# kamwoh/concepthash

Hardware: AMD Instinct MI355X
Metric: images/s encode (ViT+hash) + Hamming top-10 retrieval, CUB-200 64-bit (higher is better)
Workload: dtype bf16; 1 GPU; CUB-200 64-bit concept_hash, vit_b16 bf16 (CLIP-structured, Q=4 concept tokens, adapters b=384), batch=256/GPU, top-10 Hamming vs 5994-row gallery shard/GPU; per_gpu_batch=256, global_batch=256, gallery_rows_per_gpu=5994, hip_streams=2, parallelism=single GPU

## Files before the change

### concepthash_amd/_lib.py

```python
from __future__ import annotations

import ctypes
import os
from ctypes import (POINTER, Structure, c_char_p, c_double, c_float, c_int, c_int32, c_int64, c_size_t, c_uint32,
                    c_uint64, c_ulonglong, c_void_p)

_HERE = os.path.dirname(os.path.abspath(__file__))
LIB_PATH = os.path.join(_HERE, "libconcepthash_hip.so")
ABI_VERSION = 3


class ModelConfig(Structure):
    _fields_ = [(n, c_int32) for n in ("image_size", "patch", "dim", "layers", "heads", "ffn", "adapter_dim", "ncontext",
                                       "nbit", "nclass", "proj_dim", "center_dim", "upt_heads", "act", "max_batch")] + \
               [("ln_eps", c_float), ("bn_eps", c_float)]


class TextConfig(Structure):
    _fields_ = [(n, c_int32) for n in ("vocab", "max_positions", "dim", "layers", "heads", "ffn", "act", "max_batch")] + [("ln_eps", c_float)]


class ImageDesc(Structure):
    _fields_ = [("src_offset", c_int64), ("tmp_offset", c_int64)] + \
               [(n, c_int32) for n in ("h", "w", "nh", "nw", "top", "left", "row0", "nrows", "stride", "flip")]


class AugmentDesc(Structure):
    _fields_ = [("src_offset", c_int64), ("tmp_offset", c_int64), ("img_offset", c_int64)] + \
               [(n, c_int32) for n in ("h", "w", "nh", "nw", "top", "left", "row0", "nrows", "flip", "op", "iparam", "reserved")] + \
               [("fparam", c_double), ("m", c_double * 6)]


class JpegDesc(Structure):
    _fields_ = [("coef_offset", c_int64), ("pix_offset", c_int64), ("plane_offset", c_int64)] + \
               [(n, c_int32) for n in ("width", "height", "ncomp", "hs", "vs", "mcu_w", "mcu_h", "status", "nblocks", "reserved")] + \
               [("quant", (ctypes.c_uint16 * 64) * 3)]


class Tensor(Structure):
    _fields_ = [("name", c_char_p), ("data", POINTER(c_float)), ("numel", c_int64)]


SIGNATURES = {
    "ch_abi_version": (c_int, []),
    "ch_last_error": (c_char_p, []),
    "ch_model_create": (c_int, [POINTER(ModelConfig), POINTER(Tensor), c_int32, POINTER(c_void_p)]),
    "ch_model_destroy": (None, [c_void_p]),
    "ch_model_device_bytes": (c_size_t, [c_void_p]),
    "ch_model_flops_per_image": (c_double, [c_void_p]),
    "ch_model_set_option": (c_int, [c_void_p, c_char_p, c_int64]),
    "ch_model_get_option": (c_int, [c_void_p, c_char_p, POINTER(c_int64)]),
    "ch_model_profile_begin": (c_int, [c_void_p, c_int32]),
    "ch_model_profile_end": (c_int, [c_void_p, c_int32, POINTER(c_double), POINTER(c_int64), POINTER(c_double)]),
    "ch_debug_gemm": (c_int, [c_int32, c_void_p, c_int64, c_void_p, c_void_p, c_int32, c_int32, c_int32, c_int32, c_void_p,
                              c_int32, c_void_p, c_int32, c_void_p, c_void_p, c_void_p]),
    "ch_debug_gemm_ln": (c_int, [c_int32, c_void_p, c_int64, c_void_p, c_void_p, c_int32, c_int32, c_int32, c_int32, c_void_p,
                                 c_int32, c_void_p, c_int32, c_void_p, c_void_p, c_void_p, c_void_p, c_float, c_void_p, c_void_p,
                                 c_void_p]),
    "ch_debug_gemm_train": (c_int, [c_int32, c_void_p, c_int64, c_void_p, c_void_p, c_int32, c_int32, c_int32, c_int32, c_void_p,
                                    c_int32, c_void_p, c_void_p, c_void_p, c_void_p, c_float, c_void_p, c_int32, c_void_p]),
    "ch_debug_gemm_patch": (c_int, [c_int32, c_void_p, c_int64, c_void_p, c_int32, c_int32, c_int32, c_void_p, c_int32, c_void_p,
                                    c_int32, c_int32, c_void_p]),
    "ch_debug_gemm_dispatch_count": (c_int64, [c_int32]),
    "ch_debug_experiments_built": (c_int32, []),
    "ch_debug_set_gemm_splitk": (None, [c_int32]),
    "ch_debug_copy_buffer": (c_int, [c_void_p, c_int32, c_void_p, c_int64, c_void_p]),
    "ch_debug_adapter": (c_int, [c_void_p] * 2 + [c_int32] * 3 + [c_void_p] * 10 + [c_int32, c_void_p]),
    "ch_debug_attention": (c_int, [c_void_p, c_int32, c_int32, c_int32, c_void_p, c_void_p]),
    "ch_debug_attention_ex": (c_int, [c_void_p, c_int32, c_int32, c_int32, c_void_p, c_void_p, c_int32, c_int32, c_int32, c_void_p]),
    "ch_debug_attention_causal": (c_int, [c_void_p, c_int32, c_int32, c_int32, c_void_p, c_void_p]),
    "ch_debug_attention_dispatch_count": (c_int64, [c_int32]),
    "ch_encode": (c_int, [c_void_p, c_void_p, c_int32, c_int32, c_void_p, c_void_p, c_void_p, c_void_p, c_void_p,
                          c_void_p, c_void_p, c_void_p, c_int32, c_void_p]),
    "ch_encode_hidden": (c_int, [c_void_p, c_void_p, c_int32, c_int32, c_int32, c_void_p, c_void_p]),
    "ch_preprocess": (c_int, [c_void_p, c_void_p, c_int32, c_int32, c_int32, c_int32, POINTER(c_float), POINTER(c_float), c_void_p,
                              c_int32, c_void_p, c_void_p]),
    "ch_preprocess_max_taps": (c_int32, []),
    "ch_augment_workspace": (c_int64, [c_int32, c_int64]),
    "ch_preprocess_augment": (c_int, [c_void_p, c_void_p, c_int32, c_int32, c_int32, c_int32, c_int32, POINTER(c_float), POINTER(c_float),
                                      c_void_p, c_int32, c_void_p, c_void_p]),
    "ch_jpeg_plan": (c_int, [c_void_p, c_void_p, c_int32, c_void_p, POINTER(c_int64), POINTER(c_int64), POINTER(c_int64)]),
    "ch_jpeg_entropy_decode": (c_int, [c_void_p, c_void_p, c_int32, c_void_p, c_void_p, c_int32]),
    "ch_jpeg_plan_packed": (c_int, [c_void_p, c_void_p, c_int32, c_void_p, POINTER(c_int64), POINTER(c_int64), POINTER(c_int64)]),
    "ch_jpeg_entropy_decode_packed": (c_int, [c_void_p, c_void_p, c_int32, c_void_p, c_void_p, c_int32]),
    "ch_io_file_sizes": (c_int, [c_void_p, c_int32, c_void_p]),
    "ch_io_read_files": (c_int, [c_void_p, c_int32, c_void_p, c_void_p, c_void_p, c_int32]),
    "ch_jpeg_reconstruct": (c_int, [c_void_p, c_void_p, c_void_p, c_int32, c_void_p, c_void_p, c_void_p]),
    "ch_pack_sign": (c_int, [c_void_p, c_int64, c_int32, c_float, c_void_p, c_void_p]),
    "ch_hamming_dist": (c_int, [c_void_p, c_int64, c_void_p, c_int64, c_int32, c_void_p, c_void_p]),
    "ch_hamming_topk_workspace": (c_size_t, [c_int64, c_int64, c_int32, c_int32]),
    "ch_hamming_topk": (c_int, [c_void_p, c_int64, c_void_p, c_int64, c_int32, c_int32, c_int64, c_void_p, c_void_p,
                                c_void_p, c_size_t, c_void_p]),
    "ch_topk_merge": (c_int, [c_void_p, c_void_p, c_int32, c_int64, c_int32, c_void_p, c_void_p, c_void_p]),
    "ch_hamming_hist": (c_int, [c_void_p, c_int64, c_void_p, c_int64, c_int32, c_void_p, c_void_p, c_int32, c_int32,
                                c_void_p, c_void_p]),
    "ch_hamming_ap": (c_int, [c_void_p, c_int64, c_void_p, c_int64, c_int32, c_void_p, c_void_p, c_int32, c_int32,
                              c_void_p, c_int64, c_void_p, c_void_p, c_void_p, c_void_p]),
    "ch_hamming_ap_multi": (c_int, [c_void_p, c_int64, c_void_p, c_int64, c_int32, c_void_p, c_void_p, c_int32, c_int32,
                                    c_void_p, POINTER(c_int64), c_int32, c_void_p, c_void_p, c_void_p, c_void_p]),
    "ch_hamming_rec_workgroups": (c_size_t, [c_int64, c_int64, c_int32, c_int32]),
    "ch_hamming_rec_block": (c_int32, [c_int32]),
    "ch_hamming_hist_rec": (c_int, [c_void_p, c_int64, c_void_p, c_int64, c_int32, c_void_p, c_void_p, c_int32, c_int32,
                                    c_void_p, c_void_p, c_int32, c_void_p, c_void_p, c_void_p]),
    "ch_hamming_ap_rec": (c_int, [c_void_p, c_int64, c_void_p, c_int64, c_int32, c_void_p, c_void_p, c_int32, c_int32,
                                  c_void_p, c_void_p, c_int32, c_void_p, c_void_p, POINTER(c_int64), c_int32, c_void_p, c_void_p,
                                  c_void_p, c_void_p]),
    "ch_adapter_arena_numel": (c_int64, [c_void_p]),
    "ch_trainer_create": (c_int, [c_void_p, c_int32, c_void_p, c_void_p, POINTER(c_void_p)]),
    "ch_backbone_arena_numel": (c_int64, [POINTER(ModelConfig)]),
    "ch_backbone_arena_offset": (c_int64, [POINTER(ModelConfig), c_char_p, POINTER(c_int64)]),
    "ch_trainer_create_ex": (c_int, [c_void_p, c_int32, c_void_p, c_void_p, c_void_p, c_void_p, POINTER(c_void_p)]),
    "ch_trainer_destroy": (None, [c_void_p]),
    "ch_trainer_bytes": (c_int64, [c_void_p]),
    "ch_trainer_refresh": (c_int, [c_void_p, c_void_p]),
    "ch_train_forward": (c_int, [c_void_p, c_void_p, c_int32, c_int32, c_void_p, c_void_p, c_void_p, c_void_p, c_int32, c_void_p]),
    "ch_train_backward": (c_int, [c_void_p, c_void_p, c_void_p, c_void_p, c_void_p]),
    "ch_sgd_step": (c_int, [c_void_p, c_void_p, c_void_p, c_int64, c_float, c_float, c_float, c_float, c_int32, c_int32, c_void_p]),
    "ch_adam_step": (c_int, [c_void_p, c_void_p, c_void_p, c_void_p, c_int64, c_double, c_double, c_double, c_double, c_double, c_int32, c_int64,
                             c_void_p]),
    "ch_debug_attention_bwd": (c_int, [c_void_p, c_void_p, c_int32, c_int32, c_int32, c_void_p, c_void_p, c_int32, c_void_p]),
    "ch_debug_attention_bwd_ex": (c_int, [c_void_p, c_void_p, c_int32, c_int32, c_int32, c_void_p, c_void_p, c_int32, c_int32, c_void_p]),
    "ch_debug_wgrad": (c_int, [c_void_p, c_int32, c_void_p, c_int32, c_int64, c_int64, c_int32, c_int32, c_void_p, c_void_p]),
    "ch_debug_ln_bwd": (c_int, [c_void_p, c_void_p, c_int64, c_int32, c_float, c_void_p, c_void_p, c_void_p, c_void_p, c_void_p]),
    "ch_debug_act": (c_int, [c_void_p, c_void_p, c_int64, c_int32, c_void_p, c_int32, c_void_p, c_void_p]),
    "ch_hamming_hist_prefix": (c_int, [c_void_p, c_int32, c_int64, c_int32, c_void_p, c_void_p, c_void_p]),
    "ch_debug_set_hamming_scalar_loads": (None, [c_int32]),
    "ch_hamming_tie_bracket": (c_int, [c_void_p, c_int64, c_int32, POINTER(c_int64), c_int32, c_int32, c_void_p, c_void_p, c_void_p,
                                       c_void_p, c_void_p]),
    "ch_text_create": (c_int, [POINTER(TextConfig), POINTER(Tensor), c_int32, POINTER(c_void_p)]),
    "ch_text_destroy": (None, [c_void_p]),
    "ch_text_device_bytes": (c_size_t, [c_void_p]),
    "ch_text_encode": (c_int, [c_void_p, POINTER(c_int32), POINTER(c_int32), c_int32, c_int32, c_void_p, c_void_p, c_void_p]),
}

OPTION_KEYS = ("streams", "chain_auto", "ln_fold", "prune_last", "pp_min_k", "attn_stream", "small_kernel", "serpentine", "pp_sched", "fused_adapter", "resid_nt",
               "nt_out", "group_n", "splitk", "gemm_rows", "wide_kernel", "graph_max_batch", "train_chains", "train_chain_min_rows", "train_prune_last",
               "train_batched_grads")
_ENV_OVERRIDES = {
    "CH_STREAMS": ("streams", int), "CH_LN_FOLD": ("ln_fold", int), "CH_PRUNE_LAST": ("prune_last", int),
    "CH_GEMM_PP_MIN_K": ("pp_min_k", int), "CH_GEMM_SMALL": ("small_kernel", int), "CH_SERPENTINE": ("serpentine", int),
    "CH_GEMM_PP_SCHED": ("pp_sched", int), "CH_FUSED_ADAPTER": ("fused_adapter", int),
    "CH_RESID_NT": ("resid_nt", lambda v: 1 if int(v) else -1), "CH_NT_OUT": ("nt_out", lambda v: 1 if int(v) else -1),
    "CH_GEMM_GROUP_N": ("group_n", int), "CH_GEMM_SPLITK": ("splitk", int), "CH_GEMM_ROWS": ("gemm_rows", int), "CH_GEMM_WIDE": ("wide_kernel", int), "CH_GRAPH_MAX_BATCH": ("graph_max_batch", int),
    "CH_CHAIN_AUTO": ("chain_auto", int), "CH_TRAIN_STREAMS": ("train_chains", int), "CH_TRAIN_CHAIN_MIN_ROWS": ("train_chain_min_rows", int),
    "CH_TRAIN_PRUNE_LAST": ("train_prune_last", int),
}


def env_option_overrides() -> dict:
    out = {}
    for env, (key, conv) in _ENV_OVERRIDES.items():
        if env in os.environ:
            out[key] = conv(os.environ[env])
    return out

CATEGORIES = ("im2col", "gemm_patch", "rowops", "gemm_qkv", "attention", "gemm_out", "gemm_down", "gemm_up", "gemm_fc1",
              "gemm_fc2", "head", "adapter_fused", "attention_pruned", "gemm_out_pruned", "gemm_down_pruned", "gemm_up_pruned",
              "gemm_fc1_pruned", "gemm_fc2_pruned", "end")

_lib = None


def load() -> ctypes.CDLL:
    global _lib
    if _lib is not None:
        return _lib
    if not os.path.exists(LIB_PATH):
        raise RuntimeError(
            f"{LIB_PATH} is missing: the ConceptHash MI355X path needs the HIP extension. "
            "Build it with `python -m concepthash_amd.build` (hipcc, --offload-arch=gfx950). There is no CPU fallback.")
    try:
        lib = ctypes.CDLL(LIB_PATH)
    except OSError as e:
        raise RuntimeError(f"cannot load {LIB_PATH}: {e}") from e
    for name, (res, args) in SIGNATURES.items():
        try:
            fn = getattr(lib, name)
        except AttributeError as e:
            raise RuntimeError(f"{LIB_PATH} does not export {name}; rebuild it") from e
        fn.restype = res
        fn.argtypes = args
    if lib.ch_abi_version() != ABI_VERSION:
        raise RuntimeError(f"ABI mismatch: library {lib.ch_abi_version()} vs binding {ABI_VERSION}; rebuild")
    _lib = lib
    return lib


def check(status: int, what: str) -> None:
    if status != 0:
        msg = load().ch_last_error()
        raise RuntimeError(f"{what} failed (status {status}): {msg.decode() if msg else 'unknown error'}")


def stream_ptr(stream=None) -> c_void_p:
    import torch
    s = stream if stream is not None else torch.cuda.current_stream()
    return c_void_p(s.cuda_stream)


def ptr(t) -> c_void_p:
    return c_void_p(t.data_ptr()) if t is not None else c_void_p(0)
```

### concepthash_amd/csrc/attention.hip

```cpp
#include "ch_common.h"
#include "kernels.h"

namespace {

constexpr int HD = 64;
constexpr int QKV_AUX = 0;
#define LDQ(p) (*(const bf16x8 *)(p))
constexpr int NW = 8;
typedef __attribute__((address_space(3))) void lds_void_t;
typedef __attribute__((address_space(1))) const void gbl_void_t;
typedef short v4s __attribute__((ext_vector_type(4)));
typedef __attribute__((address_space(3))) v4s lds_v4s;

template <int KB, bool TAP, bool COMPACT, bool CAUSAL = false>
__global__ __launch_bounds__(NW * 64, 4) void attention_kernel(const bf16_t *__restrict__ qkv, int ntok, int heads, float scale_log2e,
                                                        bf16_t *__restrict__ out, float *__restrict__ cattn, int ncon, int rev) {
    extern __shared__ __attribute__((aligned(16))) char smem[];
    constexpr int KT = KB * 2;
    constexpr int KP = KB * 32;
    char *Ks = smem;
    char *Vs = smem + KP * 128;

    const int tid = threadIdx.x, lane = tid & 63;
    const int wid = __builtin_amdgcn_readfirstlane(tid >> 6);
    const int bid = rev ? (int)gridDim.x - 1 - (int)blockIdx.x : (int)blockIdx.x;
    const int b = bid / heads, h = bid - b * heads;
    const int D = heads * HD;
    const size_t ld = (size_t)3 * D;
    const bf16_t *base = qkv + (size_t)b * ntok * ld + h * HD;

    {
        const int lrow = lane >> 3;
        const int src_chunk = (lane & 7) ^ lrow;
        for (int i = wid; i < KP / 8; i += NW) {
            int row = i * 8 + lrow;
            row = row < ntok ? row : ntok - 1;
            const bf16_t *src = base + (size_t)row * ld + src_chunk * 8;
            __builtin_amdgcn_global_load_lds((gbl_void_t *)(src + D), (lds_void_t *)(Ks + i * 1024), 16, 0, QKV_AUX);
            __builtin_amdgcn_global_load_lds((gbl_void_t *)(src + 2 * D), (lds_void_t *)(Vs + i * 1024), 16, 0, QKV_AUX);
        }
    }
    const int fr = lane & 15, fq = lane >> 4;
    const int nqc = 1 + ncon;
    const int QT = COMPACT ? (nqc + 15) >> 4 : (ntok + 15) >> 4;
    auto query_of = [&](int j, bool &valid) {
        if constexpr (COMPACT) {
            valid = j < nqc;
            return !valid ? ntok - 1 : (j == 0 ? 0 : ntok - ncon + j - 1);
        } else {
            valid = j < ntok;
            return valid ? j : ntok - 1;
        }
    };
    bool qvalid;
    int qslot = wid * 16 + fr;
    int q = query_of(qslot, qvalid);
    bf16x8 qf0 = LDQ(base + (size_t)q * ld + fq * 8);
    bf16x8 qf1 = LDQ(base + (size_t)q * ld + fq * 8 + 32);
    asm volatile("s_waitcnt vmcnt(0)" ::: "memory");
    __syncthreads();

    const int tq = fr >> 2, tp = fr & 3;
    const int trow7 = ((fq & 1) << 2) | tq;
    int voff[4];
#pragma unroll
    for (int dt = 0; dt < 4; ++dt)
        voff[dt] = (fq * 4 + tq) * 128 + (((dt * 2 + (tp >> 1)) ^ trow7) << 4) + (tp & 1) * 8;
    const int koff0 = fr * 128 + ((fq ^ (fr & 7)) << 4), koff1 = fr * 128 + (((4 + fq) ^ (fr & 7)) << 4);

    for (int qt = wid; qt < QT; qt += NW) {
        f32x4 st[KT];
        bf16x8 kf[2][4];
#pragma unroll
        for (int t = 0; t < 2; ++t) {
            kf[0][2 * t] = *(const bf16x8 *)(Ks + t * 2048 + koff0);
            kf[0][2 * t + 1] = *(const bf16x8 *)(Ks + t * 2048 + koff1);
        }
#pragma unroll
        for (int c = 0; c < KB; ++c) {
            if (c + 1 < KB) {
#pragma unroll
                for (int t = 0; t < 2; ++t) {
                    kf[(c + 1) & 1][2 * t] = *(const bf16x8 *)(Ks + (2 * c + 2 + t) * 2048 + koff0);
                    kf[(c + 1) & 1][2 * t + 1] = *(const bf16x8 *)(Ks + (2 * c + 2 + t) * 2048 + koff1);
                }
            }
#pragma unroll
            for (int t = 0; t < 2; ++t) {
                f32x4 a = {0.f, 0.f, 0.f, 0.f};
                a = __builtin_amdgcn_mfma_f32_16x16x32_bf16(kf[c & 1][2 * t], qf0, a, 0, 0, 0);
                a = __builtin_amdgcn_mfma_f32_16x16x32_bf16(kf[c & 1][2 * t + 1], qf1, a, 0, 0, 0);
                st[2 * c + t] = a;
            }
            __builtin_amdgcn_sched_barrier(0);
        }
        const bool cur_valid = qvalid;
        const int cur_q = q, cur_slot = qslot;
        if (qt + NW < QT) {
            qslot = (qt + NW) * 16 + fr;
            q = query_of(qslot, qvalid);
            qf0 = LDQ(base + (size_t)q * ld + fq * 8);
            qf1 = LDQ(base + (size_t)q * ld + fq * 8 + 32);
        }
#pragma unroll
        for (int kt = KT - 2; kt < KT; ++kt)
            if (kt >= 0 && kt * 16 + 16 > ntok) {
#pragma unroll
                for (int r = 0; r < 4; ++r)
                    if (kt * 16 + fq * 4 + r >= ntok) st[kt][r] = -1e30f;
            }
        if constexpr (CAUSAL) {
            const int lim = cur_q - fq * 4;
#pragma unroll
            for (int kt = 0; kt < KT; ++kt)
#pragma unroll
                for (int r = 0; r < 4; ++r) st[kt][r] = kt * 16 + r > lim ? -1e30f : st[kt][r];
        }
        float mx = -1e30f;
#pragma unroll
        for (int kt = 0; kt < KT; ++kt)
#pragma unroll
            for (int r = 0; r < 4; ++r) mx = fmaxf(mx, st[kt][r]);
        mx = fmaxf(mx, __shfl_xor(mx, 16, 64));
        mx = fmaxf(mx, __shfl_xor(mx, 32, 64));
        const float mxs = mx * scale_log2e;
        float sum = 0.f;
#pragma unroll
        for (int kt = 0; kt < KT; ++kt)
#pragma unroll
            for (int r = 0; r < 4; ++r) {
                const float e = __builtin_amdgcn_exp2f(st[kt][r] * scale_log2e - mxs);
                st[kt][r] = e;
                sum += e;
            }
        sum += __shfl_xor(sum, 16, 64);
        sum += __shfl_xor(sum, 32, 64);
        const float inv = 1.0f / sum;
        if (TAP && cur_valid && cur_q >= ntok - ncon) {
            const int np = ntok - ncon - 1;
            float *dst = cattn + (((size_t)b * heads + h) * ncon + (cur_q - (ntok - ncon))) * np;
#pragma unroll
            for (int kt = 0; kt < KT; ++kt)
#pragma unroll
                for (int r = 0; r < 4; ++r) {
                    const int key = kt * 16 + fq * 4 + r;
                    if (key >= 1 && key <= np) dst[key - 1] = st[kt][r] * inv;
                }
        }

        f32x4 o[4];
#pragma unroll
        for (int dt = 0; dt < 4; ++dt) o[dt] = f32x4{0.f, 0.f, 0.f, 0.f};
        union VF {
            bf16x8 v;
            v4s h[2];
        };
        VF vf[2][4];
#pragma unroll
        for (int dt = 0; dt < 4; ++dt) {
            vf[0][dt].h[0] = __builtin_amdgcn_ds_read_tr16_b64_v4i16((lds_v4s *)(Vs + voff[dt]));
            vf[0][dt].h[1] = __builtin_amdgcn_ds_read_tr16_b64_v4i16((lds_v4s *)(Vs + 2048 + voff[dt]));
        }
#pragma unroll
        for (int kb = 0; kb < KB; ++kb) {
            if (kb + 1 < KB) {
#pragma unroll
                for (int dt = 0; dt < 4; ++dt) {
                    vf[(kb + 1) & 1][dt].h[0] = __builtin_amdgcn_ds_read_tr16_b64_v4i16((lds_v4s *)(Vs + (kb + 1) * 4096 + voff[dt]));
                    vf[(kb + 1) & 1][dt].h[1] =
                        __builtin_amdgcn_ds_read_tr16_b64_v4i16((lds_v4s *)(Vs + (kb + 1) * 4096 + 2048 + voff[dt]));
                }
            }
            union {
                bf16x8 v;
                uint32_t u[4];
            } pf;
            pf.u[0] = pack_bf16x2(st[2 * kb][0], st[2 * kb][1]);
            pf.u[1] = pack_bf16x2(st[2 * kb][2], st[2 * kb][3]);
            pf.u[2] = pack_bf16x2(st[2 * kb + 1][0], st[2 * kb + 1][1]);
            pf.u[3] = pack_bf16x2(st[2 * kb + 1][2], st[2 * kb + 1][3]);
#pragma unroll
            for (int dt = 0; dt < 4; ++dt) o[dt] = __builtin_amdgcn_mfma_f32_16x16x32_bf16(vf[kb & 1][dt].v, pf.v, o[dt], 0, 0, 0);
            __builtin_amdgcn_sched_barrier(0);
        }
        if (cur_valid) {
            bf16_t *op = out + (COMPACT ? (size_t)b * nqc + cur_slot : (size_t)b * ntok + cur_q) * D + h * HD + fq * 4;
#pragma unroll
            for (int dt = 0; dt < 4; ++dt) {
                uint2 w;
                w.x = pack_bf16x2(o[dt][0] * inv, o[dt][1] * inv);
                w.y = pack_bf16x2(o[dt][2] * inv, o[dt][3] * inv);
                *(uint2 *)(op + dt * 16) = w;
            }
        }
    }
}

template <int KB, bool TAP, bool COMPACT, bool CAUSAL = false>
int launch_attn_inst(const bf16_t *qkv, int B, int ntok, int heads, bf16_t *out, float *cattn, int ncon, int rev, hipStream_t s) {
    const int KP = KB * 32;
    const size_t lds = (size_t)KP * 128 * 2;
    CH_REQUIRE(lds <= 160 * 1024, "attention: sequence too long for the LDS-resident K/V kernel");
    static ch_once_per_device lds_once;
    if (int e = ch_func_max_lds((const void *)attention_kernel<KB, TAP, COMPACT, CAUSAL>, (int)lds, lds_once)) return e;
    const float scale_log2e = 0.125f * 1.4426950408889634f;
    CH_LAUNCH((attention_kernel<KB, TAP, COMPACT, CAUSAL>), dim3(B * heads), dim3(NW * 64), lds, s, qkv, ntok, heads, scale_log2e,
                       out, cattn, ncon, rev);
    CH_LAUNCH_CHECK();
    return 0;
}
template <int KB>
int launch_attn(const bf16_t *qkv, int B, int ntok, int heads, bf16_t *out, float *cattn, int ncon, bool compact, int rev, hipStream_t s) {
    if (compact)
        return cattn ? launch_attn_inst<KB, true, true>(qkv, B, ntok, heads, out, cattn, ncon, rev, s)
                     : launch_attn_inst<KB, false, true>(qkv, B, ntok, heads, out, cattn, ncon, rev, s);
    return cattn ? launch_attn_inst<KB, true, false>(qkv, B, ntok, heads, out, cattn, ncon, rev, s)
                 : launch_attn_inst<KB, false, false>(qkv, B, ntok, heads, out, cattn, ncon, rev, s);
}

}

int ch_attention(const bf16_t *qkv, int B, int ntok, int heads, bf16_t *out, hipStream_t s, float *cattn, int ncon, bool compact,
                 bool rev, int kernel) {
    CH_REQUIRE(B > 0 && ntok > 0 && heads > 0, "attention: empty problem");
    CH_REQUIRE(!compact || (ncon >= 1 && ncon < ntok), "attention: compact mode needs 1 <= ncon < ntok");
    CH_REQUIRE(kernel >= 0 && kernel <= 2, "attention: kernel must be 0 (by length), 1 (resident) or 2 (streaming)");
    if (kernel == 2 || (kernel == 0 && ntok > CH_ATTN_RESIDENT_MAX_TOKENS)) {
        ch_attention_count_launch(1);
        return ch_attention_stream(qkv, B, ntok, heads, out, s, cattn, ncon, compact, rev);
    }
    if (ntok <= CH_ATTN_RESIDENT_MAX_TOKENS) ch_attention_count_launch(0);
    const int KB = (ntok + 31) / 32;
    switch (KB) {
        case 1: return launch_attn<1>(qkv, B, ntok, heads, out, cattn, ncon, compact, rev ? 1 : 0, s);
        case 2: return launch_attn<2>(qkv, B, ntok, heads, out, cattn, ncon, compact, rev ? 1 : 0, s);
        case 3: return launch_attn<3>(qkv, B, ntok, heads, out, cattn, ncon, compact, rev ? 1 : 0, s);
        case 4: return launch_attn<4>(qkv, B, ntok, heads, out, cattn, ncon, compact, rev ? 1 : 0, s);
        case 5: return launch_attn<5>(qkv, B, ntok, heads, out, cattn, ncon, compact, rev ? 1 : 0, s);
        case 6: return launch_attn<6>(qkv, B, ntok, heads, out, cattn, ncon, compact, rev ? 1 : 0, s);
        case 7: return launch_attn<7>(qkv, B, ntok, heads, out, cattn, ncon, compact, rev ? 1 : 0, s);
        case 8: return launch_attn<8>(qkv, B, ntok, heads, out, cattn, ncon, compact, rev ? 1 : 0, s);
        case 9: return launch_attn<9>(qkv, B, ntok, heads, out, cattn, ncon, compact, rev ? 1 : 0, s);
    }
    ch_set_error("attention: the LDS-resident kernel holds at most 288 tokens per image");
    return 2;
}

int ch_attention_causal(const bf16_t *qkv, int B, int ntok, int heads, bf16_t *out, hipStream_t s) {
    CH_REQUIRE(B > 0 && ntok > 0 && heads > 0, "causal attention: empty problem");
    CH_REQUIRE(ntok <= CH_ATTN_RESIDENT_MAX_TOKENS, "causal attention: the LDS-resident kernel holds at most 288 tokens per sequence");
    switch ((ntok + 31) / 32) {
        case 1: return launch_attn_inst<1, false, false, true>(qkv, B, ntok, heads, out, nullptr, 0, 0, s);
        case 2: return launch_attn_inst<2, false, false, true>(qkv, B, ntok, heads, out, nullptr, 0, 0, s);
        case 3: return launch_attn_inst<3, false, false, true>(qkv, B, ntok, heads, out, nullptr, 0, 0, s);
        case 4: return launch_attn_inst<4, false, false, true>(qkv, B, ntok, heads, out, nullptr, 0, 0, s);
        case 5: return launch_attn_inst<5, false, false, true>(qkv, B, ntok, heads, out, nullptr, 0, 0, s);
        case 6: return launch_attn_inst<6, false, false, true>(qkv, B, ntok, heads, out, nullptr, 0, 0, s);
        case 7: return launch_attn_inst<7, false, false, true>(qkv, B, ntok, heads, out, nullptr, 0, 0, s);
        case 8: return launch_attn_inst<8, false, false, true>(qkv, B, ntok, heads, out, nullptr, 0, 0, s);
        default: return launch_attn_inst<9, false, false, true>(qkv, B, ntok, heads, out, nullptr, 0, 0, s);
    }
}
```

### concepthash_amd/csrc/debug_taps.hip

```cpp
#include <algorithm>
#include <string>

#include "model_internal.h"
#include "../../include/concepthash_hip_debug.h"

static bool g_debug_splitk = false;
static float *g_debug_ws = nullptr;
static unsigned *g_debug_cnt = nullptr;
static int debug_attach_splitk(GemmParams &p) {
    if (!g_debug_splitk) return 0;
    if (!g_debug_ws) {
        CH_CHECK_HIP(hipMalloc((void **)&g_debug_ws, CH_SPLITK_WS_BYTES));
        CH_CHECK_HIP(hipMalloc((void **)&g_debug_cnt, CH_SPLITK_CNT_BYTES));
        CH_CHECK_HIP(hipMemset(g_debug_cnt, 0, CH_SPLITK_CNT_BYTES));
    }
    p.splitk_ws = g_debug_ws;
    p.splitk_cnt = g_debug_cnt;
    p.force_split = 1;
    return 0;
}
extern "C" void ch_debug_set_gemm_splitk(int32_t on) { g_debug_splitk = on != 0; }

static GemmParams debug_gemm_params(const void *X, int64_t X_rows_alloc, const void *W, const float *bias, int32_t M, int32_t N, int32_t K,
                                    void *out_bf16, int32_t ldo, const float *scale_ptr) {
    GemmParams p{};
    p.X = (const bf16_t *)X; p.W = (const bf16_t *)W; p.M = M; p.N = N; p.K = K; p.X_rows_alloc = X_rows_alloc;
    p.bias = bias; p.out_bf16 = (bf16_t *)out_bf16; p.ldo = ldo; p.scale_ptr = scale_ptr;
    return p;
}
static int debug_gemm_launch(GemmParams &p, int epi, void *stream, int variant, bool direct, bool splitk) {
    if (splitk)
        if (int e = debug_attach_splitk(p)) return e;
    return direct ? ch_gemm_launch_variant(variant, p, epi, (hipStream_t)stream) : ch_gemm_bf16(p, epi, (hipStream_t)stream, variant);
}
extern "C" int ch_debug_gemm(int32_t variant, const void *X, int64_t X_rows_alloc, const void *W, const float *bias,
                             int32_t M, int32_t N, int32_t K, int32_t epi, void *out_bf16, int32_t ldo, float *resid,
                             int32_t ldr, const float *scale_ptr, const void *addend, void *stream) {
    CH_REQUIRE(X && W, "debug_gemm: null operand");
    CH_REQUIRE(epi >= EPI_BIAS && epi <= EPI_SCALE_RESID, "debug_gemm: epilogue must be one of the non-patch modes");
    GemmParams p = debug_gemm_params(X, X_rows_alloc, W, bias, M, N, K, out_bf16, ldo, scale_ptr);
    p.resid = resid; p.ldr = ldr; p.addend = (const bf16_t *)addend; p.ld_addend = N;
    const bool direct = (variant >= 1 && variant <= 10) || (variant >= 21 && variant <= 29) || (variant >= 41 && variant <= 47);
    return debug_gemm_launch(p, epi, stream, direct ? variant : 0, direct, true);
}
extern "C" int ch_debug_gemm_ln(int32_t variant, const void *X, int64_t X_rows_alloc, const void *W, const float *bias,
                                int32_t M, int32_t N, int32_t K, int32_t epi, void *out_bf16, int32_t ldo, float *resid,
                                int32_t ldr, const float *scale_ptr, const void *addend, const float *stats_in,
                                const float *fold_c, float ln_eps, float *stats_out, void *hb_out, void *stream) {
    CH_REQUIRE(X && W, "debug_gemm_ln: null operand");
    CH_REQUIRE(epi >= EPI_BIAS_STATS && epi <= EPI_FOLD_GELU, "debug_gemm_ln: epilogue must be one of the LayerNorm-fold modes");
    GemmParams p = debug_gemm_params(X, X_rows_alloc, W, bias, M, N, K, out_bf16, ldo, scale_ptr);
    p.resid = resid; p.ldr = ldr; p.addend = (const bf16_t *)addend; p.ld_addend = N;
    p.stats_in = stats_in; p.fold_c = fold_c; p.ln_eps = ln_eps; p.stats_out = stats_out; p.hb_out = (bf16_t *)hb_out; p.ld_hb = N;
    const bool direct = variant >= 5 && variant <= 7;
    const bool forced = variant == 1 || variant == 2 || variant == 4 || variant == 8 || variant == 9 || variant == 10;
    return debug_gemm_launch(p, epi, stream, direct || forced ? variant : 0, direct, true);
}
static int debug_gemm_launch_checked(GemmParams &p, int epi, void *stream, int variant, const char *what) {
    if (variant != 0 && variant != 1 && variant != 2 && variant != 4 && variant != 7) {
        ch_set_error(std::string(what) + ": variant must be 0 (dispatcher), 1, 2, 4 or 7");
        return 2;
    }
    return debug_gemm_launch(p, epi, stream, variant, variant != 0, false);
}
extern "C" int ch_debug_gemm_train(int32_t variant, const void *X, int64_t X_rows_alloc, const void *W, const float *bias, int32_t M,
                                   int32_t N, int32_t K, int32_t epi, void *out_bf16, int32_t ldo, const void *aux, const float *scale_ptr,
                                   const float *stats_in, const float *fold_c, float ln_eps, void *hb_out, int32_t ld_hb, void *stream) {
    CH_REQUIRE(X && W && bias && out_bf16, "debug_gemm_train: null operand");
    CH_REQUIRE(epi >= EPI_BIAS_DACT_QUICK && epi <= EPI_FOLD_ACT2_GELU, "debug_gemm_train: epilogue must be one of the training modes (11 .. 14)");
    CH_REQUIRE(M > 0 && N > 0 && K > 0, "debug_gemm_train: empty problem");
    CH_REQUIRE(ldo >= N && ldo % 8 == 0, "debug_gemm_train: ldo must be >= N and a multiple of 8 (16-byte row chunks)");
    const bool dact = epi == EPI_BIAS_DACT_QUICK || epi == EPI_BIAS_DACT_GELU;
    if (dact) {
        CH_REQUIRE(aux != nullptr, "debug_gemm_train: the derivative epilogues need aux");
        const char *a0 = (const char *)aux, *o0 = (const char *)out_bf16;
        const size_t span = ((size_t)(M - 1) * ldo + N) * sizeof(bf16_t);
        CH_REQUIRE(a0 + span <= o0 || o0 + span <= a0, "debug_gemm_train: aux and out_bf16 must not overlap");
    } else {
        CH_REQUIRE(hb_out != nullptr && stats_in && fold_c, "debug_gemm_train: the two-output epilogues need hb_out, stats_in and fold_c");
        CH_REQUIRE(ld_hb >= N && ld_hb % 8 == 0, "debug_gemm_train: ld_hb must be >= N and a multiple of 8 (16-byte row chunks)");
        CH_REQUIRE(K % 128 == 0 && K <= 1280 && ln_eps > 0.f, "debug_gemm_train: LN-folded epilogue needs K % 128 == 0, K <= 1280, ln_eps > 0");
        CH_REQUIRE(hb_out != out_bf16, "debug_gemm_train: hb_out and out_bf16 must be distinct");
    }
    GemmParams p = debug_gemm_params(X, X_rows_alloc, W, bias, M, N, K, out_bf16, ldo, scale_ptr);
    p.aux = (const bf16_t *)aux;
    p.stats_in = stats_in; p.fold_c = fold_c; p.ln_eps = ln_eps; p.hb_out = (bf16_t *)hb_out; p.ld_hb = ld_hb;
    return debug_gemm_launch_checked(p, epi, stream, variant, "debug_gemm_train");
}
extern "C" int ch_debug_gemm_patch(int32_t variant, const void *X, int64_t X_rows_alloc, const void *W, int32_t M, int32_t N, int32_t K,
                                   float *resid, int32_t ldr, const float *pos, int32_t tokens_per_img, int32_t patches_per_img,
                                   void *stream) {
    CH_REQUIRE(X && W && resid && pos, "debug_gemm_patch: null operand");
    CH_REQUIRE(M > 0 && N > 0 && K > 0, "debug_gemm_patch: empty problem");
    CH_REQUIRE(ldr >= N && ldr % 4 == 0, "debug_gemm_patch: ldr must be >= N and a multiple of 4 (16-byte row chunks)");
    CH_REQUIRE(patches_per_img >= 1 && tokens_per_img >= 1 + patches_per_img, "debug_gemm_patch: tokens_per_img must be >= 1 + patches_per_img");
    CH_REQUIRE(M % patches_per_img == 0, "debug_gemm_patch: M must be a whole number of images");
    GemmParams p = debug_gemm_params(X, X_rows_alloc, W, nullptr, M, N, K, nullptr, 0, nullptr);
    p.resid = resid; p.ldr = ldr; p.pos = pos; p.tokens_per_img = tokens_per_img; p.patches_per_img = patches_per_img;
    return debug_gemm_launch_checked(p, EPI_PATCH, stream, variant, "debug_gemm_patch");
}
extern "C" int32_t ch_debug_experiments_built(void) {
#ifdef CH_EXPERIMENTS
    return 1;
#else
    return 0;
#endif
}

extern "C" int ch_debug_attention(const void *qkv, int32_t B, int32_t ntok, int32_t heads, void *out, void *stream) {
    CH_REQUIRE(qkv && out, "debug_attention: null pointer");
    return ch_attention((const bf16_t *)qkv, B, ntok, heads, (bf16_t *)out, (hipStream_t)stream);
}
extern "C" int ch_debug_attention_ex(const void *qkv, int32_t B, int32_t ntok, int32_t heads, void *out, float *cattn, int32_t ncon,
                                     int32_t compact, int32_t kernel, void *stream) {
    CH_REQUIRE(qkv && out, "debug_attention_ex: null pointer");
    return ch_attention((const bf16_t *)qkv, B, ntok, heads, (bf16_t *)out, (hipStream_t)stream, cattn, ncon, compact != 0, false, kernel);
}

extern "C" int ch_debug_attention_causal(const void *qkv, int32_t B, int32_t ntok, int32_t heads, void *out, void *stream) {
    CH_REQUIRE(qkv && out, "debug_attention_causal: null pointer");
    return ch_attention_causal((const bf16_t *)qkv, B, ntok, heads, (bf16_t *)out, (hipStream_t)stream);
}

extern "C" int ch_debug_adapter(const void *A, float *H, int32_t M, int32_t D, int32_t b, const float *Wd, const float *bd,
                                const float *gamma, const float *beta, const void *Wu_bf16_padded, const float *bu,
                                const float *scale, void *work_wdf, float *work_c, float *work_d, int32_t dbg, void *stream) {
    const int bpad = (int)round_up64(b, 128);
    hipStream_t s = (hipStream_t)stream;
    if (int e = ch_fold_ln(Wd, bd, gamma, beta, b, bpad, D, (bf16_t *)work_wdf, work_c, work_d, s)) return e;
    AdapterParams p{};
    p.A = (const bf16_t *)A; p.H = H; p.M = M; p.D = D; p.bpad = bpad; p.Wd = (const bf16_t *)work_wdf; p.c = work_c; p.d = work_d;
    p.Wu = (const bf16_t *)Wu_bf16_padded; p.bu = bu; p.scale = scale; p.eps = 1e-5f; p.dbg = dbg;
    return ch_adapter_fused(p, s);
}

extern "C" int ch_debug_copy_buffer(ch_model *m, int32_t which, void *out, int64_t nbytes, void *stream) {
    CH_REQUIRE(m != nullptr && out != nullptr && nbytes >= 0, "debug_copy_buffer: null pointer");
    const int64_t rows = m->rows_alloc, D = m->cfg.dim;
    const void *src = nullptr;
    int64_t size = 0;
    switch (which) {
        case 0: src = m->H; size = rows * D * 4; break;
        case 1: src = m->Xn; size = rows * D * 2; break;
        case 2: src = m->QKV; size = rows * 3 * D * 2; break;
        case 3: src = m->AO; size = rows * D * 2; break;
        case 4: src = m->A; size = rows * D * 2; break;
        case 5: src = m->AD; size = rows * std::max(m->bpad, 128) * 2; break;
        case 6: src = m->F1; size = rows * (int64_t)m->cfg.ffn * 2; break;
        default: CH_REQUIRE(false, "debug_copy_buffer: which must be 0..6 (H, Xn, QKV, AO, A, AD, F1)");
    }
    CH_REQUIRE(nbytes <= size, "debug_copy_buffer: more bytes requested than the buffer holds");
    CH_CHECK_HIP(hipMemcpyAsync(out, src, (size_t)nbytes, hipMemcpyDeviceToDevice, (hipStream_t)stream));
    return 0;
}

extern "C" int ch_debug_attention_bwd(const void *qkv, const void *dO, int32_t B, int32_t ntok, int32_t heads, void *dqkv, const float *dpext,
                                      int32_t ncon, void *stream) {
    CH_REQUIRE(qkv && dO && dqkv, "debug_attention_bwd: null argument");
    return ch_attention_bwd((const bf16_t *)qkv, (const bf16_t *)dO, B, ntok, heads, (bf16_t *)dqkv, (hipStream_t)stream, dpext, ncon);
}
extern "C" int ch_debug_attention_bwd_ex(const void *qkv, const void *dO, int32_t B, int32_t ntok, int32_t heads, void *dqkv, const float *dpext,
                                         int32_t ncon, int32_t kernel, void *stream) {
    CH_REQUIRE(qkv && dO && dqkv, "debug_attention_bwd_ex: null argument");
    return ch_attention_bwd((const bf16_t *)qkv, (const bf16_t *)dO, B, ntok, heads, (bf16_t *)dqkv, (hipStream_t)stream, dpext, ncon, kernel);
}
extern "C" int ch_debug_wgrad(const void *A, int32_t lda, const void *Bm, int32_t ldb, int64_t rows, int64_t rows_alloc, int32_t N,
                              int32_t K, float *out, void *stream) {
    CH_REQUIRE(A && Bm && out, "debug_wgrad: null argument");
    float *ws = nullptr;
    CH_CHECK_HIP(hipMalloc((void **)&ws, sizeof(float) * ch_wgrad_ws_floats(rows, N, K)));
    const int e = ch_wgrad_tn((bf16_t *)A, lda, (const bf16_t *)Bm, ldb, rows, rows_alloc, N, K, out, ws, (hipStream_t)stream);
    (void)hipStreamSynchronize((hipStream_t)stream);
    (void)hipFree(ws);
    return e;
}
extern "C" int ch_debug_ln_bwd(const void *dyg, const void *x, int64_t rows, int32_t D, float eps, const float *dres_in, float *dres_out,
                               void *out_b, void *xhat_out, void *stream) {
    CH_REQUIRE(dyg && x && dres_in, "debug_ln_bwd: null argument");
    hipStream_t s = (hipStream_t)stream;
    float *st = nullptr, *xf = nullptr;
    bf16_t *hb = nullptr;
    CH_CHECK_HIP(hipMalloc((void **)&st, sizeof(float) * rows * (D / 64) * 2));
    CH_CHECK_HIP(hipMalloc((void **)&xf, sizeof(float) * rows * D));
    CH_CHECK_HIP(hipMalloc((void **)&hb, sizeof(bf16_t) * rows * D));
    int e = 0;
    {
        CH_CHECK_HIP(hipMemsetAsync(xf, 0, sizeof(float) * rows * D, s));
        CH_CHECK_HIP(hipMemcpy2DAsync((char *)xf + 2, 4, x, 2, 2, (size_t)rows * D, hipMemcpyDeviceToDevice, s));
    }
    e = ch_hb_stats(xf, rows, D, hb, st, s);
    if (!e) e = ch_ln_bwd((const bf16_t *)dyg, (const bf16_t *)x, st, rows, D, eps, dres_in, dres_out, (bf16_t *)out_b, s);
    if (!e && xhat_out) e = ch_normalize_bf16((const bf16_t *)x, st, rows, D, eps, (bf16_t *)xhat_out, s);
    (void)hipStreamSynchronize(s);
    (void)hipFree(st);
    (void)hipFree(xf);
    (void)hipFree(hb);
    return e;
}
extern "C" int ch_debug_act(const void *g, const void *pre, int64_t n, int32_t act, const float *scale_ptr, int32_t backward, void *out,
                            void *stream) {
    CH_REQUIRE(pre && out, "debug_act: null argument");
    if (backward) return ch_act_bwd((const bf16_t *)g, (const bf16_t *)pre, n, act, scale_ptr, (bf16_t *)out, (hipStream_t)stream);
    return ch_act_fwd((const bf16_t *)pre, n, act, (bf16_t *)out, (hipStream_t)stream);
}
```

### concepthash_amd/csrc/gemm_bf16.hip

```cpp
#include <cstdlib>

#include "ch_common.h"
#include "kernels.h"
#include "gemm_epilogue.h"

namespace {

constexpr int BM = 128, BN = 128, BK = 64;
constexpr int STAGE_BYTES = (BM + BN) * BK * 2;
constexpr int NTHREADS = 256;

typedef __attribute__((address_space(3))) void lds_void_t;
typedef __attribute__((address_space(1))) const void gbl_void_t;


__device__ __forceinline__ int xcd_remap(int bid, int nwg) {
    const int q = nwg >> 3, r = nwg & 7, xcd = bid & 7, local = bid >> 3;
    const int base = xcd < r ? xcd * (q + 1) : r * (q + 1) + (xcd - r) * q;
    return base + local;
}

template <int EPI, bool NT = false>
__global__ __launch_bounds__(NTHREADS, 2) void gemm_bf16_kernel(GemmParams p) {
    extern __shared__ __attribute__((aligned(16))) char smem[];
    const int tid = threadIdx.x;
    const int lane = tid & 63;
    const int wid = __builtin_amdgcn_readfirstlane(tid >> 6);
    const int wm = wid & 1, wn = wid >> 1;

    const int tiles_n = p.N / BN;
    const int tiles_m = (p.M + BM - 1) / BM;
    const int wg = xcd_remap(blockIdx.x, tiles_m * tiles_n);
    const int per_group = tiles_m * p.group_n;
    const int g = wg / per_group, rem = wg - g * per_group;
    const int gn = min(p.group_n, tiles_n - g * p.group_n);
    const int tm_fwd = rem / gn, tn = g * p.group_n + (rem - tm_fwd * gn);
    const int tm = p.rev ? tiles_m - 1 - tm_fwd : tm_fwd;
    const int m0 = tm * BM, n0 = tn * BN;

    const int lrow = lane >> 3;
    const int src_chunk = (lane & 7) ^ lrow;
    const char *gsrc[8];
#pragma unroll
    for (int j = 0; j < 8; ++j) {
        const int row = (wid * 8 + j) * 8 + lrow;
        const bf16_t *base = row < BM ? p.X + (size_t)(m0 + row) * p.K : p.W + (size_t)(n0 + row - BM) * p.K;
        gsrc[j] = (const char *)(base + src_chunk * 8);
    }
    auto stage = [&](int buf, int kt) {
        char *dst = smem + buf * STAGE_BYTES + wid * 8 * 1024;
#pragma unroll
        for (int j = 0; j < 8; ++j)
            __builtin_amdgcn_global_load_lds((gbl_void_t *)(gsrc[j] + (size_t)kt * BK * 2), (lds_void_t *)(dst + j * 1024),
                                             16, 0, 0);
    };

    f32x4 acc[4][4];
#pragma unroll
    for (int a = 0; a < 4; ++a)
#pragma unroll
        for (int b = 0; b < 4; ++b) acc[a][b] = f32x4{0.f, 0.f, 0.f, 0.f};

    const int frow = lane & 15, fq = lane >> 4;
    const int nk = p.K / BK;

    f32x4 fold_v[5];
    if constexpr (ch_epi::traits<EPI>::fold) ch_epi::fold_stats_issue(p, m0, tid, fold_v);
    stage(0, 0);
    constexpr bool PREF = ch_epi::traits<EPI>::scale_resid;
    ch_epi::ResidPrefetch rp;
    if constexpr (PREF) ch_epi::resid_prefetch<EPI, NT>(p, m0 + wm * 64, n0 + wn * 64, lane, rp);
    asm volatile("s_waitcnt vmcnt(0)" ::: "memory");
    __builtin_amdgcn_sched_barrier(0);
    if constexpr (ch_epi::traits<EPI>::fold)
        ch_epi::fold_stats_finish(p, tid, fold_v, (float *)(smem + 2 * STAGE_BYTES));
    __syncthreads();

    int cur = 0;
    for (int kt = 0; kt < nk; ++kt) {
        if (kt + 1 < nk) stage(cur ^ 1, kt + 1);
        const char *xs = smem + cur * STAGE_BYTES;
        const char *ws = xs + BM * BK * 2;
#pragma unroll
        for (int kk = 0; kk < 2; ++kk) {
            bf16x8 wf[4], xf[4];
#pragma unroll
            for (int t = 0; t < 4; ++t) {
                const int wr = wn * 64 + t * 16 + frow;
                wf[t] = *(const bf16x8 *)(ws + wr * 128 + (((kk * 4 + fq) ^ (wr & 7)) << 4));
                const int xr = wm * 64 + t * 16 + frow;
                xf[t] = *(const bf16x8 *)(xs + xr * 128 + (((kk * 4 + fq) ^ (xr & 7)) << 4));
            }
#pragma unroll
            for (int nt = 0; nt < 4; ++nt)
#pragma unroll
                for (int mt = 0; mt < 4; ++mt)
                    acc[nt][mt] = __builtin_amdgcn_mfma_f32_16x16x32_bf16(wf[nt], xf[mt], acc[nt][mt], 0, 0, 0);
        }
        asm volatile("s_waitcnt vmcnt(0)" ::: "memory");
        __syncthreads();
        cur ^= 1;
    }

    ch_epi::store_tile<EPI, 4, PREF, NT>(p, acc, smem + wid * 16384, m0 + wm * 64, n0 + wn * 64, lane,
                                         (const float *)(smem + 2 * STAGE_BYTES) + 2 * (wm * 64), &rp);
}

template <int EPI>
int launch(const GemmParams &p0, hipStream_t s) {
    GemmParams p = p0;
    p.group_n = ch_gemm_group_n(p.M, p.N, p.K, BM, BN, p.group_n_opt);
    const int tiles = ((p.M + BM - 1) / BM) * (p.N / BN);
    constexpr int lds = 2 * STAGE_BYTES + (ch_epi::traits<EPI>::fold ? CH_FOLD_LDS_BYTES : 0);
    static ch_once_per_device lds_once;
    if (int e = ch_func_max_lds((const void *)gemm_bf16_kernel<EPI>, lds, lds_once)) return e;
    if constexpr (ch_epi::traits<EPI>::scale_resid) {
        if (p.nt_resid) {
            static ch_once_per_device lds_once_nt;
            if (int e = ch_func_max_lds((const void *)gemm_bf16_kernel<EPI, true>, lds, lds_once_nt)) return e;
            CH_LAUNCH((gemm_bf16_kernel<EPI, true>), dim3(tiles), dim3(NTHREADS), lds, s, p);
            CH_LAUNCH_CHECK();
            ch_gemm_count_nt_launch(0);
            return 0;
        }
    }
    CH_LAUNCH(gemm_bf16_kernel<EPI>, dim3(tiles), dim3(NTHREADS), lds, s, p);
    CH_LAUNCH_CHECK();
    return 0;
}

}

int ch_gemm_bf16_v1(const GemmParams &p, int epi, hipStream_t s) {
    CH_REQUIRE(p.M > 0 && p.N > 0 && p.K > 0, "gemm: empty problem");
    CH_REQUIRE(epi == EPI_PATCH || p.bias != nullptr, "gemm: bias is required");
    CH_REQUIRE(p.N % BN == 0, "gemm: N must be a multiple of 128");
    CH_REQUIRE(p.K % BK == 0, "gemm: K must be a multiple of 64");
    CH_REQUIRE(p.X_rows_alloc >= round_up64(p.M, BM), "gemm: X must be allocated for M rounded up to 128 rows");
    switch (epi) {
        case EPI_BIAS: return launch<EPI_BIAS>(p, s);
        case EPI_BIAS_QUICKGELU: return launch<EPI_BIAS_QUICKGELU>(p, s);
        case EPI_BIAS_GELU: return launch<EPI_BIAS_GELU>(p, s);
        case EPI_BIAS_RESID: return launch<EPI_BIAS_RESID>(p, s);
        case EPI_SCALE_RESID: return launch<EPI_SCALE_RESID>(p, s);
        case EPI_PATCH: return launch<EPI_PATCH>(p, s);
        case EPI_BIAS_STATS: return launch<EPI_BIAS_STATS>(p, s);
        case EPI_SCALE_RESID_STATS: return launch<EPI_SCALE_RESID_STATS>(p, s);
        case EPI_FOLD_BIAS: return launch<EPI_FOLD_BIAS>(p, s);
        case EPI_FOLD_QUICKGELU: return launch<EPI_FOLD_QUICKGELU>(p, s);
        case EPI_FOLD_GELU: return launch<EPI_FOLD_GELU>(p, s);
        case EPI_BIAS_DACT_QUICK: return launch<EPI_BIAS_DACT_QUICK>(p, s);
        case EPI_BIAS_DACT_GELU: return launch<EPI_BIAS_DACT_GELU>(p, s);
        case EPI_FOLD_ACT2_QUICK: return launch<EPI_FOLD_ACT2_QUICK>(p, s);
        case EPI_FOLD_ACT2_GELU: return launch<EPI_FOLD_ACT2_GELU>(p, s);
    }
    ch_set_error("gemm: unknown epilogue");
    return 2;
}

int ch_gemm_group_n(int M, int N, int K, int bm, int bn, int forced) {
    const int tiles_n = N / bn, tiles_m = (M + bm - 1) / bm;
    const double xbytes = 2.0 * M * K, wpanel = 2.0 * bn * K, wbytes = 2.0 * N * K;
    const double rounds = (double)tiles_m * tiles_n / 256.0 + 1.0;
    if (forced > 0) return forced < tiles_n ? forced : tiles_n;
    int best = tiles_n;
    double best_cost = 1e300;
    for (int gn = 1; gn <= tiles_n; ++gn) {
        const int ng = (tiles_n + gn - 1) / gn;
        const bool fits = gn * wpanel <= 2.0e6;
        const double cost = xbytes * ng + wbytes * 8.0 * (fits ? 1.0 : rounds);
        if (cost < best_cost - 1.0) {
            best_cost = cost;
            best = gn;
        }
    }
    return best;
}

static std::atomic<int64_t> g_dispatch_count[5];
void ch_gemm_count_nt_launch(int kind) { g_dispatch_count[2 + (kind != 0)].fetch_add(1, std::memory_order_relaxed); }
static int resid_nt_choice(const GemmParams &p, int epi) {
    if (epi != EPI_SCALE_RESID && epi != EPI_SCALE_RESID_STATS) return 0;
    if (p.nt_resid_opt) return p.nt_resid_opt > 0;
    return std::max<int64_t>(p.M, p.footprint_rows) * p.N * 4 >= (48ll << 20);
}
static int out_nt_choice(const GemmParams &p, int epi) {
    if (epi != EPI_BIAS && epi != EPI_FOLD_BIAS && epi != EPI_FOLD_QUICKGELU && epi != EPI_FOLD_GELU && epi != EPI_FOLD_ACT2_QUICK &&
        epi != EPI_FOLD_ACT2_GELU && epi != EPI_BIAS_DACT_QUICK && epi != EPI_BIAS_DACT_GELU)
        return 0;
    if (p.nt_out_opt) return p.nt_out_opt > 0;
    return std::max<int64_t>(p.M, p.footprint_rows) * p.N * 2 >= (128ll << 20);
}
int ch_gemm_launch_variant(int variant, const GemmParams &p, int epi, hipStream_t s) {
    switch (variant) {
        case 1: return ch_gemm_bf16_v1(p, epi, s);
        case 2: return ch_gemm_bf16_pp(p, epi, s);
        case 4:
        case 8: {
            GemmParams q = p;
            q.pp_sched = variant == 4 ? 1 : 2;
            return ch_gemm_bf16_pp(q, epi, s);
        }
        case 3: return ch_gemm_bf16_dp(p, epi, s);
        case 5: return ch_gemm_bf16_ppp(p, epi, s);
        case 6: return ch_gemm_bf16_pq(p, epi, s);
        case 7: return ch_gemm_bf16_r4(p, epi, s);
        case 9: return ch_gemm_bf16_rows(p, epi, s);
        case 10: return ch_gemm_bf16_wide(p, epi, s);
    }
    if (variant >= 21 && variant <= 29) return ch_gemm_bf16_pp_dbg(p, variant - 20, s);
    if (variant >= 41 && variant <= 47) return ch_gemm_bf16_wide_dbg(p, variant - 40, s);
    ch_set_error("gemm: variant must be 1 .. 10, 21 .. 29 (256x256 timing builds) or 41 .. 47 (256x384 timing builds)");
    return 2;
}
int ch_gemm_bf16(const GemmParams &p0, int epi, hipStream_t s, int variant) {
    GemmParams p = p0;
    p.nt_resid = resid_nt_choice(p, epi);
    p.nt_out = out_nt_choice(p, epi);
    if (epi == EPI_BIAS_DACT_QUICK || epi == EPI_BIAS_DACT_GELU) CH_REQUIRE(p.aux != nullptr, "gemm: derivative epilogue needs aux (the pre-activation)");
    if (epi == EPI_FOLD_ACT2_QUICK || epi == EPI_FOLD_ACT2_GELU) CH_REQUIRE(p.hb_out != nullptr, "gemm: two-output epilogue needs hb_out");
    if (epi == EPI_FOLD_BIAS || epi == EPI_FOLD_QUICKGELU || epi == EPI_FOLD_GELU || epi == EPI_FOLD_ACT2_QUICK || epi == EPI_FOLD_ACT2_GELU)
        CH_REQUIRE(p.stats_in && p.fold_c && p.K % 128 == 0 && p.K <= 1280 && p.ln_eps > 0.f,
                   "gemm: LN-folded epilogue needs stats_in, fold_c, ln_eps and K % 128 == 0, K <= 1280");
    if (epi == EPI_BIAS_STATS || epi == EPI_SCALE_RESID_STATS)
        CH_REQUIRE(p.stats_out && (epi == EPI_BIAS_STATS || p.hb_out), "gemm: statistics epilogue needs stats_out (and hb_out)");
    if (variant != 0 && variant != 7) return ch_gemm_launch_variant(variant, p, epi, s);
    const int min_k = p.pp_min_k > 0 ? p.pp_min_k : 512;
    const int64_t tiles_pp = ceil_div64(p.M, 256) * (p.N / 256);
    const bool pp = ch_gemm_pp_supported(p) && p.K >= min_k && (p.pp_min_k > 0 || tiles_pp >= 128);
    const bool wide = !pp && p.wide_opt > 0 && ch_gemm_wide_supported(p, epi);
    g_dispatch_count[pp ? 1 : wide ? 4 : 0].fetch_add(1, std::memory_order_relaxed);
    if (pp) return ch_gemm_bf16_pp(p, epi, s);
    if (wide) return ch_gemm_bf16_wide(p, epi, s);
    if (p.rows_opt && p.small_kernel == 0 && p.M >= 128 * 128 && ch_gemm_rows_supported(p, epi)) return ch_gemm_bf16_rows(p, epi, s);
    const bool ring = (p.small_kernel == 2 || variant == 7 || (p.small_kernel == 0 && variant == 0 && p.M <= CH_RING_MAX_ROWS && !p.nt_resid)) &&
                      ch_gemm_r4_supported(p, epi);
    return ring ? ch_gemm_bf16_r4(p, epi, s) : ch_gemm_bf16_v1(p, epi, s);
}
extern "C" int64_t ch_debug_gemm_dispatch_count(int32_t which) {
    return g_dispatch_count[which < 0 || which > 4 ? 0 : which].load(std::memory_order_relaxed);
}
```

### concepthash_amd/csrc/gemm_epilogue.h

```cpp
#pragma once
#include "ch_common.h"
#include "kernels.h"

namespace ch_epi {

typedef uint32_t u32x4_nt __attribute__((ext_vector_type(4)));
template <bool NT>
__device__ __forceinline__ f32x4 ld_resid(const float *ptr) {
    if constexpr (NT) return __builtin_nontemporal_load((const f32x4 *)ptr);
    else return *(const f32x4 *)ptr;
}
template <bool NT>
__device__ __forceinline__ void st_resid(float *ptr, f32x4 v) {
    if constexpr (NT) __builtin_nontemporal_store(v, (f32x4 *)ptr);
    else *(f32x4 *)ptr = v;
}

__device__ __forceinline__ float quick_gelu_f(float x) {
    return x * __builtin_amdgcn_rcpf(1.0f + __builtin_amdgcn_exp2f(-2.4554669595930157f * x));
}
__device__ __forceinline__ float gelu_erf_f(float x) {
    const float z = fabsf(x) * 0.70710678118654752f;
    const float t = __builtin_amdgcn_rcpf(1.0f + 0.3275911f * z);
    const float poly = t * (0.254829592f + t * (-0.284496736f + t * (1.421413741f + t * (-1.453152027f + t * 1.061405429f))));
    const float erf_abs = 1.0f - poly * __builtin_amdgcn_exp2f(-1.4426950408889634f * z * z);
    return 0.5f * x * (1.0f + copysignf(erf_abs, x));
}

__device__ __forceinline__ float dquick_gelu_f(float x) {
    const float s = __builtin_amdgcn_rcpf(1.0f + __builtin_amdgcn_exp2f(-2.4554669595930157f * x));
    return s * (1.0f + 1.702f * x * (1.0f - s));
}
__device__ __forceinline__ float dgelu_erf_f(float x) {
    const float z = fabsf(x) * 0.70710678118654752f;
    const float t = __builtin_amdgcn_rcpf(1.0f + 0.3275911f * z);
    const float poly = t * (0.254829592f + t * (-0.284496736f + t * (1.421413741f + t * (-1.453152027f + t * 1.061405429f))));
    const float e = __builtin_amdgcn_exp2f(-1.4426950408889634f * z * z);
    const float cdf = 0.5f * (1.0f + copysignf(1.0f - poly * e, x));
    return cdf + x * 0.3989422804014327f * e;
}

template <int EPI>
struct traits {
    static constexpr bool dact = (EPI == EPI_BIAS_DACT_QUICK || EPI == EPI_BIAS_DACT_GELU);
    static constexpr bool act2 = (EPI == EPI_FOLD_ACT2_QUICK || EPI == EPI_FOLD_ACT2_GELU);
    static constexpr bool fold = (EPI == EPI_FOLD_BIAS || EPI == EPI_FOLD_QUICKGELU || EPI == EPI_FOLD_GELU || act2);
    static constexpr bool quick = (EPI == EPI_BIAS_QUICKGELU || EPI == EPI_FOLD_QUICKGELU);
    static constexpr bool erf = (EPI == EPI_BIAS_GELU || EPI == EPI_FOLD_GELU);
    static constexpr bool bf16_only = (EPI == EPI_BIAS || EPI == EPI_BIAS_STATS || quick || erf || fold || dact);
    static constexpr bool scale_resid = (EPI == EPI_SCALE_RESID || EPI == EPI_SCALE_RESID_STATS);
    static constexpr bool stats = (EPI == EPI_BIAS_STATS || EPI == EPI_SCALE_RESID_STATS);
};

template <int EPI>
__device__ __forceinline__ f32x4 activate(f32x4 v) {
    if constexpr (traits<EPI>::quick) {
#pragma unroll
        for (int r = 0; r < 4; ++r) v[r] = quick_gelu_f(v[r]);
    }
    if constexpr (traits<EPI>::erf) {
#pragma unroll
        for (int r = 0; r < 4; ++r) v[r] = gelu_erf_f(v[r]);
    }
    return v;
}

template <int CTRL>
__device__ __forceinline__ float dpp_f(float v) {
    return __builtin_bit_cast(float, __builtin_amdgcn_update_dpp(0, __builtin_bit_cast(int, v), CTRL, 0xf, 0xf, true));
}
__device__ __forceinline__ float sum8(float v) {
    v += dpp_f<0xB1>(v);
    v += dpp_f<0x4E>(v);
    v += dpp_f<0x141>(v);
    return v;
}
__device__ __forceinline__ float sum16(float v) {
    v = sum8(v);
    v += dpp_f<0x140>(v);
    return v;
}

__device__ __forceinline__ void fold_stats_issue(const GemmParams &p, int m0, int tid, f32x4 (&v)[5]) {
    const int m = min(m0 + (tid >> 1), p.M - 1);
    const int n4 = p.K >> 7, H = (n4 + 1) >> 1;
    const f32x4 *st = (const f32x4 *)(p.stats_in + (size_t)m * (p.K >> 6) * 2);
#pragma unroll
    for (int i = 0; i < 5; ++i) {
        const f32x4 *src = st + min((tid & 1) * H + i, n4 - 1);
        asm volatile("global_load_dwordx4 %0, %1, off" : "=v"(v[i]) : "v"(src) : "memory");
    }
}
__device__ __forceinline__ void fold_stats_finish(const GemmParams &p, int tid, const f32x4 (&v)[5], float *row_ms) {
    const int n4 = p.K >> 7, H = (n4 + 1) >> 1, first = (tid & 1) * H;
    float sm = 0.f, sq = 0.f;
#pragma unroll
    for (int i = 0; i < 5; ++i) {
        const bool valid = i < H && first + i < n4;
        sm += valid ? v[i][0] + v[i][2] : 0.f;
        sq += valid ? v[i][1] + v[i][3] : 0.f;
    }
    sm += dpp_f<0xB1>(sm);
    sq += dpp_f<0xB1>(sq);
    const float inv = 1.0f / (float)p.K;
    const float mean = sm * inv;
    const float var = fmaxf(sq * inv - mean * mean, 0.f);
    if (!(tid & 1)) *(ch_f32x2_t *)(row_ms + (tid & ~1)) = ch_f32x2_t{rsqrtf(var + p.ln_eps), mean};
}

struct ResidPrefetch {
    f32x4 hv[8];
    uint2 av[8];
};
template <int EPI, bool NT = false>
__device__ __forceinline__ void resid_prefetch(const GemmParams &p, int m_base, int n_base, int lane, ResidPrefetch &r) {
    const int lrow = lane >> 4, pos = lane & 15;
#pragma unroll
    for (int j = 0; j < 8; ++j) {
        const int row = j * 4 + lrow;
        const int m = m_base + row;
        const int mc = m < p.M ? m : p.M - 1;
        const int n = n_base + (pos ^ (row & 15)) * 4;
        r.hv[j] = ld_resid<NT>(p.resid + (size_t)mc * p.ldr + n);
        r.av[j] = make_uint2(0u, 0u);
        if (p.addend) r.av[j] = *(const uint2 *)(p.addend + (size_t)mc * p.ld_addend + n);
    }
}

template <int EPI, int MT, bool PREF = false, bool NT = false, bool NTOUT = false>
__device__ __forceinline__ void store_tile(const GemmParams &p, f32x4 (&acc)[4][MT], char *wave_lds, int m_base, int n_base,
                                           int lane, const float *row_ms = nullptr, const ResidPrefetch *pf = nullptr) {
    static_assert(!PREF || (MT == 4 && traits<EPI>::scale_resid), "prefetched residual: 64-row wave tiles, scale+residual epilogues");
    const int fr = lane & 15, fq = lane >> 4;
    using T = traits<EPI>;
    constexpr bool BF16_ONLY = T::bf16_only;
    f32x4 bias[4];
#pragma unroll
    for (int nt = 0; nt < 4; ++nt) {
        if constexpr (EPI != EPI_PATCH)
            bias[nt] = *(const f32x4 *)(p.bias + n_base + nt * 16 + fq * 4);
        else
            bias[nt] = f32x4{0.f, 0.f, 0.f, 0.f};
    }

    if constexpr (BF16_ONLY) {
        uint4 ax[T::dact ? MT * 2 : 1];
        float dact_scale = 1.0f;
        if constexpr (T::dact) {
            const int lrow = lane >> 3, pos = lane & 7;
#pragma unroll
            for (int i = 0; i < MT * 2; ++i) {
                const int row = i * 8 + lrow;
                const int m = m_base + row;
                const int mc = m < p.M ? m : p.M - 1;
                ax[i] = *(const uint4 *)(p.aux + (size_t)mc * p.ldo + n_base + (pos ^ (row & 7)) * 8);
            }
            if (EPI == EPI_BIAS_DACT_GELU && p.scale_ptr) dact_scale = *p.scale_ptr;
        }
        f32x4 fc[4];
        if constexpr (T::fold) {
#pragma unroll
            for (int nt = 0; nt < 4; ++nt) fc[nt] = *(const f32x4 *)(p.fold_c + n_base + nt * 16 + fq * 4);
        }
#pragma unroll
        for (int mt = 0; mt < MT; ++mt) {
            const int row = mt * 16 + fr;
            float rs = 1.0f, nm = 0.f;
            if constexpr (T::fold) {
                const ch_f32x2_t ms = *(const ch_f32x2_t *)(row_ms + 2 * row);
                rs = ms[0];
                nm = -ms[1] * ms[0];
            }
#pragma unroll
            for (int nt = 0; nt < 4; ++nt) {
                f32x4 pre;
                if constexpr (T::fold)
                    pre = acc[nt][mt] * rs + (fc[nt] * nm + bias[nt]);
                else
                    pre = acc[nt][mt] + bias[nt];
                const f32x4 v = activate<EPI>(pre);
                uint2 o;
                o.x = pack_bf16x2(v[0], v[1]);
                o.y = pack_bf16x2(v[2], v[3]);
                *(uint2 *)(wave_lds + row * 128 + (((nt * 2 + (fq >> 1)) ^ (row & 7)) << 4) + (((fq & 1) ^ ((row >> 3) & 1)) << 3)) = o;
            }
        }
        asm volatile("s_waitcnt lgkmcnt(0)" ::: "memory");
        const int lrow = lane >> 3, pos = lane & 7;
#pragma unroll
        for (int i = 0; i < MT * 2; ++i) {
            const int row = i * 8 + lrow;
            const int chunk = pos ^ (row & 7);
            uint4 v = *(const uint4 *)(wave_lds + row * 128 + pos * 16);
            if (i & 1) v = make_uint4(v.z, v.w, v.x, v.y);
            const int m = m_base + row;
            if constexpr (T::dact) {
                const uint4 a = ax[i];
                const float sc = dact_scale;
                const uint32_t vw[4] = {v.x, v.y, v.z, v.w}, aw[4] = {a.x, a.y, a.z, a.w};
                uint32_t ow[4];
#pragma unroll
                for (int j = 0; j < 4; ++j) {
                    const float x0 = bf2f((bf16_t)(aw[j] & 0xffff)), x1 = bf2f((bf16_t)(aw[j] >> 16));
                    const float d0 = EPI == EPI_BIAS_DACT_QUICK ? dquick_gelu_f(x0) : dgelu_erf_f(x0);
                    const float d1 = EPI == EPI_BIAS_DACT_QUICK ? dquick_gelu_f(x1) : dgelu_erf_f(x1);
                    ow[j] = pack_bf16x2(sc * bf2f((bf16_t)(vw[j] & 0xffff)) * d0, sc * bf2f((bf16_t)(vw[j] >> 16)) * d1);
                }
                v = make_uint4(ow[0], ow[1], ow[2], ow[3]);
            }
            if (m < p.M) {
                uint4 *dst = (uint4 *)(p.out_bf16 + (size_t)m * p.ldo + n_base + chunk * 8);
                if constexpr (NTOUT) __builtin_nontemporal_store(__builtin_bit_cast(u32x4_nt, v), (u32x4_nt *)dst);
                else *dst = v;
            }
            if constexpr (T::act2) {
                const uint32_t vw[4] = {v.x, v.y, v.z, v.w};
                uint32_t ow[4];
#pragma unroll
                for (int j = 0; j < 4; ++j) {
                    const float x0 = bf2f((bf16_t)(vw[j] & 0xffff)), x1 = bf2f((bf16_t)(vw[j] >> 16));
                    ow[j] = EPI == EPI_FOLD_ACT2_QUICK ? pack_bf16x2(quick_gelu_f(x0), quick_gelu_f(x1))
                                                       : pack_bf16x2(gelu_erf_f(x0), gelu_erf_f(x1));
                }
                if (m < p.M) {
                    uint4 *dst2 = (uint4 *)(p.hb_out + (size_t)m * p.ld_hb + n_base + chunk * 8);
                    const uint4 w2 = make_uint4(ow[0], ow[1], ow[2], ow[3]);
                    if constexpr (NTOUT) __builtin_nontemporal_store(__builtin_bit_cast(u32x4_nt, w2), (u32x4_nt *)dst2);
                    else *dst2 = w2;
                }
            }
            if constexpr (T::stats) {
                const uint32_t w[4] = {v.x, v.y, v.z, v.w};
                float sm = 0.f, sq = 0.f;
#pragma unroll
                for (int j = 0; j < 4; ++j) {
                    const float a = bf2f((bf16_t)(w[j] & 0xffff)), b = bf2f((bf16_t)(w[j] >> 16));
                    sm += a + b;
                    sq += a * a + b * b;
                }
                sm = sum8(sm);
                sq = sum8(sq);
                if (pos == 0 && m < p.M)
                    *(ch_f32x2_t *)(p.stats_out + ((size_t)m * (p.N >> 6) + (n_base >> 6)) * 2) = ch_f32x2_t{sm, sq};
            }
        }
    } else {
        float scale = 1.0f;
        if constexpr (T::scale_resid) scale = *p.scale_ptr;
        const int lrow = lane >> 4, pos = lane & 15;
#pragma unroll
        for (int pass = 0; pass < MT / 4; ++pass) {
            if (pass) asm volatile("s_waitcnt lgkmcnt(0)" ::: "memory");
#pragma unroll
            for (int mt4 = 0; mt4 < 4; ++mt4) {
                const int row = mt4 * 16 + fr;
#pragma unroll
                for (int nt = 0; nt < 4; ++nt) {
                    const f32x4 v = acc[nt][pass * 4 + mt4] + bias[nt];
                    *(f32x4 *)(wave_lds + row * 256 + (((nt * 4 + fq) ^ (row & 15)) << 4)) = v;
                }
            }
            asm volatile("s_waitcnt lgkmcnt(0)" ::: "memory");
#pragma unroll
            for (int batch = 0; batch < 2; ++batch) {
                f32x4 hv[8], lv[8];
                uint2 av[8];
                size_t off[8];
                bool ok[8];
#pragma unroll
                for (int i = 0; i < 8; ++i) {
                    const int row = (batch * 8 + i) * 4 + lrow;
                    const int chunk = pos ^ (row & 15);
                    const int m = m_base + pass * 64 + row;
                    const int n = n_base + chunk * 4;
                    ok[i] = m < p.M;
                    const int mc = ok[i] ? m : p.M - 1;
                    lv[i] = *(const f32x4 *)(wave_lds + row * 256 + pos * 16);
                    if constexpr (EPI == EPI_PATCH) {
                        const int img = mc / p.patches_per_img, pp = mc - img * p.patches_per_img;
                        off[i] = ((size_t)img * p.tokens_per_img + 1 + pp) * p.ldr + n;
                        hv[i] = *(const f32x4 *)(p.pos + (size_t)(1 + pp) * p.N + n);
                    } else {
                        off[i] = (size_t)mc * p.ldr + n;
                        if (PREF && batch == 0)
                            hv[i] = pf->hv[i];
                        else
                            hv[i] = EPI == EPI_BIAS_RESID ? *(const f32x4 *)(p.resid + off[i]) : ld_resid<NT>(p.resid + off[i]);
                        if constexpr (T::scale_resid) {
                            if (PREF && batch == 0) {
                                av[i] = pf->av[i];
                            } else {
                                av[i] = make_uint2(0u, 0u);
                                if (p.addend) av[i] = *(const uint2 *)(p.addend + (size_t)mc * p.ld_addend + n);
                            }
                        }
                    }
                }
#pragma unroll
                for (int i = 0; i < 8; ++i) {
                    if (!ok[i]) continue;
                    const f32x4 v = lv[i];
                    if constexpr (EPI == EPI_PATCH) {
                        *(f32x4 *)(p.resid + off[i]) = v + hv[i];
                    } else if constexpr (EPI == EPI_BIAS_RESID) {
                        *(f32x4 *)(p.resid + off[i]) = hv[i] + v;
                        const int row = (batch * 8 + i) * 4 + lrow;
                        const int m = m_base + pass * 64 + row;
                        const int n = n_base + (pos ^ (row & 15)) * 4;
                        uint2 o;
                        o.x = pack_bf16x2(v[0], v[1]);
                        o.y = pack_bf16x2(v[2], v[3]);
                        *(uint2 *)(p.out_bf16 + (size_t)m * p.ldo + n) = o;
                    } else {
                        f32x4 h = hv[i] + v * scale;
                        h[0] += bf2f((bf16_t)(av[i].x & 0xffff));
                        h[1] += bf2f((bf16_t)(av[i].x >> 16));
                        h[2] += bf2f((bf16_t)(av[i].y & 0xffff));
                        h[3] += bf2f((bf16_t)(av[i].y >> 16));
                        st_resid<NT>(p.resid + off[i], h);
                        if constexpr (T::stats) {
                            const int row = (batch * 8 + i) * 4 + lrow;
                            const int m = m_base + pass * 64 + row;
                            const int n = n_base + (pos ^ (row & 15)) * 4;
                            uint2 o;
                            o.x = pack_bf16x2(h[0], h[1]);
                            o.y = pack_bf16x2(h[2], h[3]);
                            *(uint2 *)(p.hb_out + (size_t)m * p.ld_hb + n) = o;
                            const float a = bf2f((bf16_t)(o.x & 0xffff)), b = bf2f((bf16_t)(o.x >> 16));
                            const float c = bf2f((bf16_t)(o.y & 0xffff)), d = bf2f((bf16_t)(o.y >> 16));
                            const float sm = sum16((a + b) + (c + d));
                            const float sq = sum16((a * a + b * b) + (c * c + d * d));
                            if (pos == 0)
                                *(ch_f32x2_t *)(p.stats_out + ((size_t)m * (p.N >> 6) + (n_base >> 6)) * 2) = ch_f32x2_t{sm, sq};
                        }
                    }
                }
            }
        }
    }
}

}
```

### concepthash_amd/csrc/gemm_pp.hip

```cpp
#include <cstdlib>

#include "ch_common.h"
#include "kernels.h"
#include "gemm_epilogue.h"

namespace {

constexpr int BM = 256, BN = 256, BK = 64;
constexpr int HALF_BYTES = 128 * BK * 2;
constexpr int BUF_BYTES = 4 * HALF_BYTES;
constexpr int NTHREADS = 512;
constexpr int PP_LDS_BYTES = 2 * BUF_BYTES + CH_FOLD_LDS_BYTES + 16;

typedef __attribute__((address_space(3))) void lds_void_t;
typedef __attribute__((address_space(1))) const void gbl_void_t;


__device__ __forceinline__ int xcd_remap(int bid, int nwg) {
    const int q = nwg >> 3, r = nwg & 7, xcd = bid & 7, local = bid >> 3;
    const int base = xcd < r ? xcd * (q + 1) : r * (q + 1) + (xcd - r) * q;
    return base + local;
}

#define PP_BARRIER()                       \
// ... 177 lines not shown
            PP_BARRIER();
            PP_MFMA(Wa, 0, 0);
            PP_MFMA(Wbf, 1, 0);
            PP_BARRIER();
            read_x(1, 1);
            if (kt + 3 < nkt) {
                issue(2, kt + 3);
                issue(3, kt + 3);
                issue(0, kt + 3);
                PP_WAIT_VM(8);
            }
            PP_WAIT_LGKM0();
            PP_BARRIER();
            PP_MFMA(Wbf, 1, 1);
            PP_MFMA(Wa, 0, 1);
            PP_BARRIER();
        }
        if (wr == 0) PP_BARRIER();
    } else {
        f32x4 fold_v[5];
        if constexpr (ch_epi::traits<EPI>::fold) ch_epi::fold_stats_issue(p, m0, tid, fold_v);
        issue(0, kb0);
        issue(2, kb0);
        issue(3, kb0);
        issue(1, kb0);
        issue(0, kb0 + 1);
        issue(2, kb0 + 1);
        issue(3, kb0 + 1);
        PP_WAIT_VM(6);
        if constexpr (ch_epi::traits<EPI>::fold) {
            ch_epi::fold_stats_finish(p, tid, fold_v, (float *)(smem + 2 * BUF_BYTES));
            asm volatile("s_waitcnt lgkmcnt(0)" ::: "memory");
        }
        PP_BARRIER();
        if constexpr (DBG & 8) stamp[2] = __builtin_amdgcn_s_memtime();
        if (wr == 1) PP_BARRIER();

        for (int jj = 0; jj < J; ++jj) {
            const bool more = (jj + 1 < J);
            const int ke = 2 * (j0 + jj), ko = ke + 1;
            read_w(Wa, 0, 0);
            read_x(0, 0);
            issue(1, ko);
            PP_WAIT_LGKM0();
            PP_BARRIER();
            PP_MFMA(Wa, 0, 0);
            PP_BARRIER();
            read_w(Wbf, 0, 1);
            if (more) issue(0, ke + 2);
            PP_WAIT_LGKM0();
            PP_BARRIER();
            PP_MFMA(Wbf, 1, 0);
            PP_BARRIER();
            read_x(0, 1);
            if (more) issue(2, ke + 2);
            PP_WAIT_LGKM0();
            PP_BARRIER();
            PP_MFMA(Wbf, 1, 1);
            PP_BARRIER();
            if (more) {
                issue(3, ke + 2);
                PP_WAIT_VM(6);
            } else {
                PP_WAIT_VM(0);
            }
            PP_BARRIER();
            PP_MFMA(Wa, 0, 1);
            PP_BARRIER();
            if (free_tail && !more && wr == 0) PP_BARRIER();
            read_w(Wa, 1, 0);
            read_x(1, 0);
            if (more) issue(1, ke + 2);
            PP_WAIT_LGKM0();
            PP_BARRIER_T();
            PP_MFMA(Wa, 0, 0);
            PP_BARRIER_T();
            read_w(Wbf, 1, 1);
            if (more) issue(0, ko + 2);
            PP_WAIT_LGKM0();
            PP_BARRIER_T();
            PP_MFMA(Wbf, 1, 0);
            PP_BARRIER_T();
            read_x(1, 1);
            if (more) issue(2, ko + 2);
            PP_WAIT_LGKM0();
            PP_BARRIER_T();
            PP_MFMA(Wbf, 1, 1);
            PP_BARRIER_T();
            if (more) {
                issue(3, ko + 2);
                PP_WAIT_VM(6);
            }
            PP_BARRIER_T();
            PP_MFMA(Wa, 0, 1);
            PP_BARRIER_T();
        }
        if (!free_tail && wr == 0) PP_BARRIER();
    }

    if (split) {
        typedef unsigned v4u __attribute__((ext_vector_type(4)));
        constexpr unsigned SLAB_BYTES = BM * BN * 4;
        const auto rsrc = __builtin_amdgcn_make_buffer_rsrc(p.splitk_ws, 0, (int)CH_SPLITK_WS_BYTES, 0x00020000);
        const unsigned tile_off = (unsigned)(split_tile * p.split_s) * SLAB_BYTES;
        const unsigned lane_off = (unsigned)tid * 16;
        {
            const unsigned base = tile_off + (unsigned)slice * SLAB_BYTES + lane_off;
#pragma unroll
            for (int i = 0; i < 32; ++i)
                __builtin_amdgcn_raw_buffer_store_b128(__builtin_bit_cast(v4u, acc[i >> 3][i & 7]), rsrc, base + i * (NTHREADS * 16), 0, 16);
        }
        asm volatile("s_waitcnt vmcnt(0)" ::: "memory");
        __syncthreads();
        unsigned *ticket_lds = (unsigned *)(smem + 2 * BUF_BYTES + CH_FOLD_LDS_BYTES);
        if (tid == 0)
            *ticket_lds = __hip_atomic_fetch_add(p.splitk_cnt + split_tile, 1u, __ATOMIC_RELAXED, __HIP_MEMORY_SCOPE_AGENT);
        __syncthreads();
        const unsigned ticket = *ticket_lds;
        if (ticket != (unsigned)(p.split_s - 1)) return;
        if (tid == 0)
            __hip_atomic_store(p.splitk_cnt + split_tile, 0u, __ATOMIC_RELAXED, __HIP_MEMORY_SCOPE_AGENT);
        __builtin_amdgcn_fence(__ATOMIC_ACQUIRE, "wavefront");
#pragma unroll
        for (int a = 0; a < 4; ++a)
#pragma unroll
            for (int b = 0; b < 8; ++b) acc[a][b] = f32x4{0.f, 0.f, 0.f, 0.f};
        for (int sl = 0; sl < p.split_s; ++sl) {
            const unsigned base = tile_off + (unsigned)sl * SLAB_BYTES + lane_off;
#pragma unroll
            for (int i = 0; i < 32; ++i)
                acc[i >> 3][i & 7] += __builtin_bit_cast(f32x4, __builtin_amdgcn_raw_buffer_load_b128(rsrc, base + i * (NTHREADS * 16), 0, 16));
        }
    }

    if constexpr (DBG & 4) {
        f32x4 t = acc[0][0];
#pragma unroll
        for (int a = 0; a < 4; ++a)
#pragma unroll
            for (int b = 0; b < 8; ++b) t += acc[a][b];
        if (t[0] == 12345.678f) p.out_bf16[tid] = (bf16_t)1;
        return;
    }
    if constexpr (DBG & 8) stamp[3] = __builtin_amdgcn_s_memtime();
    if constexpr (SCHED == 2 && ch_epi::traits<EPI>::bf16_only) {
        if (free_tail) {
#pragma unroll
            for (int pass = 0; pass < 2; ++pass) {
                f32x4 half[4][4];
#pragma unroll
                for (int nt = 0; nt < 4; ++nt)
#pragma unroll
                    for (int mt = 0; mt < 4; ++mt) half[nt][mt] = acc[nt][pass * 4 + mt];
                ch_epi::store_tile<EPI, 4, false, false, TAG == 2>(p, half, smem + wid * 8192, m0 + wr * 128 + pass * 64, n0 + wc * 64, lane,
                                           (const float *)(smem + 2 * BUF_BYTES) + 2 * (wr * 128 + pass * 64));
                asm volatile("s_waitcnt lgkmcnt(0)" ::: "memory");
            }
            return;
        }
    }
    ch_epi::store_tile<EPI, 8, false, false, TAG == 2>(p, acc, smem + wid * 16384, m0 + wr * 128, n0 + wc * 64, lane,
                               (const float *)(smem + 2 * BUF_BYTES) + 2 * (wr * 128));
    if constexpr (DBG & 8) {
        stamp[4] = __builtin_amdgcn_s_memtime();
        asm volatile("s_waitcnt vmcnt(0)" ::: "memory");
        stamp[5] = __builtin_amdgcn_s_memtime();
        if (tid == 0) {
            unsigned long long *st = (unsigned long long *)p.resid + (size_t)blockIdx.x * 8;
            st[0] = stamp[0];
            st[1] = stamp[1];
            st[2] = stamp[2];
            st[3] = stamp[3];
            st[4] = stamp[4];
            st[5] = stamp[5];
            st[6] = (unsigned long long)__builtin_amdgcn_s_getreg(0xF804) | ((unsigned long long)__builtin_amdgcn_s_getreg(0xF814) << 32);
            st[7] = __builtin_amdgcn_s_memrealtime();
        }
    }
}

void ch_pp_choose_split(GemmParams &p, int tiles) {
    static const int ncu = [] {
        int dev = 0, n = 256;
        if (hipGetDevice(&dev) == hipSuccess) (void)hipDeviceGetAttribute(&n, hipDeviceAttributeMultiprocessorCount, dev);
        return n > 0 ? n : 256;
    }();
    p.split_full = tiles;
    p.split_s = 1;
    if (!(p.splitk_opt || p.force_split) || !p.splitk_ws || !p.splitk_cnt) return;
    const int R = tiles % ncu, J = p.K / (2 * BK);
    if (R == 0) return;
    int S = 1;
    for (int c = 2; c <= 8; ++c)
        if (J % c == 0 && R * c <= ncu && R * c <= 256) S = c;
    if (S < 2 || J / S < 1) return;
    p.split_full = tiles - R;
    p.split_s = S;
}

template <int EPI, int SCHED>
int launch_pp_sched(GemmParams &p, int tiles, hipStream_t s) {
    constexpr int lds = PP_LDS_BYTES;
    const dim3 grid(p.split_full + (tiles - p.split_full) * p.split_s);
    if constexpr (EPI == EPI_BIAS_STATS && SCHED == 0) {
        if (p.tag == 1) {
            static ch_once_per_device lds_once_t;
            if (int e = ch_func_max_lds((const void *)gemm_pp_kernel<EPI, 0, SCHED, 1>, lds, lds_once_t)) return e;
            CH_LAUNCH((gemm_pp_kernel<EPI, 0, SCHED, 1>), grid, dim3(NTHREADS), lds, s, p);
            CH_LAUNCH_CHECK();
            return 0;
        }
    }
    if constexpr ((EPI == EPI_BIAS || EPI == EPI_FOLD_BIAS || EPI == EPI_FOLD_QUICKGELU || EPI == EPI_FOLD_GELU || EPI == EPI_FOLD_ACT2_QUICK ||
                   EPI == EPI_FOLD_ACT2_GELU || EPI == EPI_BIAS_DACT_QUICK || EPI == EPI_BIAS_DACT_GELU) && SCHED == 0) {
        if (p.nt_out) {
            static ch_once_per_device lds_once_n;
            if (int e = ch_func_max_lds((const void *)gemm_pp_kernel<EPI, 0, SCHED, 2>, lds, lds_once_n)) return e;
            CH_LAUNCH((gemm_pp_kernel<EPI, 0, SCHED, 2>), grid, dim3(NTHREADS), lds, s, p);
            CH_LAUNCH_CHECK();
            ch_gemm_count_nt_launch(1);
            return 0;
        }
    }
    static ch_once_per_device lds_once;
    if (int e = ch_func_max_lds((const void *)gemm_pp_kernel<EPI, 0, SCHED>, lds, lds_once)) return e;
    CH_LAUNCH((gemm_pp_kernel<EPI, 0, SCHED>), grid, dim3(NTHREADS), lds, s, p);
    CH_LAUNCH_CHECK();
    return 0;
}

template <int EPI>
int launch_pp(const GemmParams &p0, hipStream_t s) {
    GemmParams p = p0;
    p.group_n = ch_gemm_group_n(p.M, p.N, p.K, BM, BN, p.group_n_opt);
    const int tiles = ((p.M + BM - 1) / BM) * (p.N / BN);
    if (p.pp_sched == 1) {
#ifdef CH_EXPERIMENTS
        p.split_full = tiles;
        p.split_s = 1;
        return launch_pp_sched<EPI, 1>(p, tiles, s);
#else
        return ch_experiments_not_built();
#endif
    }
    if (p.pp_sched == 2) {
#ifdef CH_EXPERIMENTS
        ch_pp_choose_split(p, tiles);
        return launch_pp_sched<EPI, 2>(p, tiles, s);
#else
        return ch_experiments_not_built();
#endif
    }
    ch_pp_choose_split(p, tiles);
    return launch_pp_sched<EPI, 0>(p, tiles, s);
}

}

bool ch_gemm_pp_supported(const GemmParams &p) {
    return p.N % BN == 0 && p.K % (2 * BK) == 0 && p.X_rows_alloc >= round_up64(p.M, BM) &&
           (size_t)round_up64(p.M, BM) * p.K * 2 < (1ull << 32) && (size_t)p.N * p.K * 2 < (1ull << 32);
}

int ch_gemm_bf16_pp_dbg(const GemmParams &p0, int dbg, hipStream_t s) {
    GemmParams p = p0;
    p.group_n = ch_gemm_group_n(p.M, p.N, p.K, BM, BN);
    const int tiles = ((p.M + BM - 1) / BM) * (p.N / BN);
    if (!ch_gemm_pp_supported(p)) return 2;
    p.split_full = tiles;
    p.split_s = 1;
#define PP_DBG_CASE(D)                                                                                                   \
    case D:                                                                                                              \
        (void)hipFuncSetAttribute((const void *)gemm_pp_kernel<EPI_BIAS, D>, hipFuncAttributeMaxDynamicSharedMemorySize,   \
                                  2 * BUF_BYTES);                                                                        \
        hipLaunchKernelGGL((gemm_pp_kernel<EPI_BIAS, D>), dim3(tiles), dim3(NTHREADS), 2 * BUF_BYTES, s, p);             \
        break;
    switch (dbg) {
        PP_DBG_CASE(1)
        PP_DBG_CASE(2)
        PP_DBG_CASE(3)
        PP_DBG_CASE(4)
        PP_DBG_CASE(5)
        PP_DBG_CASE(6)
        PP_DBG_CASE(7)
        case 8:
        case 9: {
            if (!p.resid) return 2;
            constexpr int lds = PP_LDS_BYTES;
            if (dbg == 8) {
                (void)hipFuncSetAttribute((const void *)gemm_pp_kernel<EPI_BIAS, 8>, hipFuncAttributeMaxDynamicSharedMemorySize, lds);
                hipLaunchKernelGGL((gemm_pp_kernel<EPI_BIAS, 8>), dim3(tiles), dim3(NTHREADS), lds, s, p);
            } else {
                (void)hipFuncSetAttribute((const void *)gemm_pp_kernel<EPI_BIAS_QUICKGELU, 8>, hipFuncAttributeMaxDynamicSharedMemorySize,
                                          lds);
                hipLaunchKernelGGL((gemm_pp_kernel<EPI_BIAS_QUICKGELU, 8>), dim3(tiles), dim3(NTHREADS), lds, s, p);
            }
            break;
        }
        default: return 2;
    }
    CH_LAUNCH_CHECK();
    return 0;
}

int ch_gemm_bf16_pp(const GemmParams &p, int epi, hipStream_t s) {
    CH_REQUIRE(p.M > 0 && p.N > 0 && p.K > 0, "gemm: empty problem");
    CH_REQUIRE(epi == EPI_PATCH || p.bias != nullptr, "gemm: bias is required");
    CH_REQUIRE(ch_gemm_pp_supported(p), "gemm_pp: needs N % 256 == 0, K % 128 == 0, X padded to 256 rows, operands < 4 GiB");
    switch (epi) {
        case EPI_BIAS: return launch_pp<EPI_BIAS>(p, s);
        case EPI_BIAS_QUICKGELU: return launch_pp<EPI_BIAS_QUICKGELU>(p, s);
        case EPI_BIAS_GELU: return launch_pp<EPI_BIAS_GELU>(p, s);
        case EPI_BIAS_RESID: return launch_pp<EPI_BIAS_RESID>(p, s);
        case EPI_SCALE_RESID: return launch_pp<EPI_SCALE_RESID>(p, s);
        case EPI_PATCH: return launch_pp<EPI_PATCH>(p, s);
        case EPI_BIAS_STATS: return launch_pp<EPI_BIAS_STATS>(p, s);
        case EPI_SCALE_RESID_STATS: return launch_pp<EPI_SCALE_RESID_STATS>(p, s);
        case EPI_FOLD_BIAS: return launch_pp<EPI_FOLD_BIAS>(p, s);
        case EPI_FOLD_QUICKGELU: return launch_pp<EPI_FOLD_QUICKGELU>(p, s);
        case EPI_FOLD_GELU: return launch_pp<EPI_FOLD_GELU>(p, s);
        case EPI_BIAS_DACT_QUICK: return launch_pp<EPI_BIAS_DACT_QUICK>(p, s);
        case EPI_BIAS_DACT_GELU: return launch_pp<EPI_BIAS_DACT_GELU>(p, s);
        case EPI_FOLD_ACT2_QUICK: return launch_pp<EPI_FOLD_ACT2_QUICK>(p, s);
        case EPI_FOLD_ACT2_GELU: return launch_pp<EPI_FOLD_ACT2_GELU>(p, s);
    }
    ch_set_error("gemm: unknown epilogue");
    return 2;
}
```

### concepthash_amd/csrc/gemm_r4.hip

```cpp
#include "ch_common.h"
#include "kernels.h"
#include "gemm_epilogue.h"

namespace {

constexpr int BM = 128, BN = 128, BK = 32;
constexpr int STAGE_BYTES = (BM + BN) * BK * 2;
constexpr int NTHREADS = 256;

typedef __attribute__((address_space(3))) void lds_void_t;
typedef __attribute__((address_space(1))) const void gbl_void_t;

__device__ __forceinline__ int xcd_remap(int bid, int nwg) {
    const int q = nwg >> 3, r = nwg & 7, xcd = bid & 7, local = bid >> 3;
    const int base = xcd < r ? xcd * (q + 1) : r * (q + 1) + (xcd - r) * q;
    return base + local;
}

template <int EPI, int NSTAGE>
__global__ __launch_bounds__(NTHREADS, NSTAGE == 2 ? 4 : 2) void gemm_r4_kernel(GemmParams p) {
    extern __shared__ __attribute__((aligned(16))) char smem[];
    const int tid = threadIdx.x;
    const int lane = tid & 63;
    const int wid = __builtin_amdgcn_readfirstlane(tid >> 6);
    const int wm = wid & 1, wn = wid >> 1;

    const int tiles_n = p.N / BN;
    const int tiles_m = (p.M + BM - 1) / BM;
    const int wg = xcd_remap(blockIdx.x, tiles_m * tiles_n);
    const int per_group = tiles_m * p.group_n;
    const int g = wg / per_group, rem = wg - g * per_group;
    const int gn = min(p.group_n, tiles_n - g * p.group_n);
    const int tm_fwd = rem / gn, tn = g * p.group_n + (rem - tm_fwd * gn);
    const int tm = p.rev ? tiles_m - 1 - tm_fwd : tm_fwd;
    const int m0 = tm * BM, n0 = tn * BN;

    const int src_chunk = (lane & 3) ^ (((lane >> 5) & 1) << 1);
    const char *gsrc[4];
#pragma unroll
    for (int j = 0; j < 4; ++j) {
        const int row = (wid * 4 + j) * 16 + (lane >> 2);
        const bf16_t *base = row < BM ? p.X + (size_t)(m0 + row) * p.K : p.W + (size_t)(n0 + row - BM) * p.K;
        gsrc[j] = (const char *)(base + src_chunk * 8);
    }
    auto stage = [&](int buf, int kt) {
        char *dst = smem + buf * STAGE_BYTES + wid * 4 * 1024;
#pragma unroll
        for (int j = 0; j < 4; ++j)
            __builtin_amdgcn_global_load_lds((gbl_void_t *)(gsrc[j] + (size_t)kt * BK * 2), (lds_void_t *)(dst + j * 1024), 16, 0, 0);
    };

    f32x4 acc[4][4];
#pragma unroll
    for (int a = 0; a < 4; ++a)
#pragma unroll
        for (int b = 0; b < 4; ++b) acc[a][b] = f32x4{0.f, 0.f, 0.f, 0.f};

    const int fr = lane & 15, fq = lane >> 4;
    const int fsw = (fq ^ (((fr >> 3) & 1) << 1)) << 4;
    const int xoff = (wm * 64 + fr) * 64 + fsw;
    const int woff = BM * 64 + (wn * 64 + fr) * 64 + fsw;
    const int nk = p.K / BK;

    f32x4 fold_v[5];
    if constexpr (ch_epi::traits<EPI>::fold) ch_epi::fold_stats_issue(p, m0, tid, fold_v);
    constexpr bool PREF = ch_epi::traits<EPI>::scale_resid;
    ch_epi::ResidPrefetch rp;
    if constexpr (PREF) ch_epi::resid_prefetch<EPI>(p, m0 + wm * 64, n0 + wn * 64, lane, rp);
    stage(0, 0);
    if (NSTAGE > 2 && nk > 1) stage(1, 1);
    if (NSTAGE > 2 && nk > 2) stage(2, 2);
    if constexpr (ch_epi::traits<EPI>::fold) {
        if (NSTAGE > 2 && nk > 2)
            asm volatile("s_waitcnt vmcnt(12)" ::: "memory");
        else if (NSTAGE == 2)
            asm volatile("s_waitcnt vmcnt(4)" ::: "memory");
        else
            asm volatile("s_waitcnt vmcnt(0)" ::: "memory");
        __builtin_amdgcn_sched_barrier(0);
        ch_epi::fold_stats_finish(p, tid, fold_v, (float *)(smem + NSTAGE * STAGE_BYTES));
    }

    int buf = 0;
    for (int kt = 0; kt < nk; ++kt) {
        const int ahead = nk - 1 - kt;
        if (NSTAGE > 2 && ahead >= 2)
            asm volatile("s_waitcnt vmcnt(8)" ::: "memory");
        else if (NSTAGE > 2 && ahead == 1)
            asm volatile("s_waitcnt vmcnt(4)" ::: "memory");
        else
            asm volatile("s_waitcnt vmcnt(0)" ::: "memory");
        __builtin_amdgcn_sched_barrier(0);
        __builtin_amdgcn_s_barrier();
        __builtin_amdgcn_sched_barrier(0);
        if (kt + NSTAGE - 1 < nk) stage((buf + NSTAGE - 1) & (NSTAGE - 1), kt + NSTAGE - 1);
        const char *sb = smem + buf * STAGE_BYTES;
        bf16x8 wf[4], xf[4];
#pragma unroll
        for (int t = 0; t < 4; ++t) {
            wf[t] = *(const bf16x8 *)(sb + woff + t * 1024);
            xf[t] = *(const bf16x8 *)(sb + xoff + t * 1024);
        }
#pragma unroll
        for (int nt = 0; nt < 4; ++nt)
#pragma unroll
            for (int mt = 0; mt < 4; ++mt)
                acc[nt][mt] = __builtin_amdgcn_mfma_f32_16x16x32_bf16(wf[nt], xf[mt], acc[nt][mt], 0, 0, 0);
        buf = (buf + 1) & (NSTAGE - 1);
    }
    __builtin_amdgcn_sched_barrier(0);
    asm volatile("s_waitcnt lgkmcnt(0)" ::: "memory");
    __builtin_amdgcn_s_barrier();
    __builtin_amdgcn_sched_barrier(0);
    ch_epi::store_tile<EPI, 4, PREF>(p, acc, smem + wid * (NSTAGE == 2 ? 8192 : 16384), m0 + wm * 64, n0 + wn * 64, lane,
                                     (const float *)(smem + NSTAGE * STAGE_BYTES) + 2 * (wm * 64), &rp);
}

template <int EPI, int NSTAGE = 4>
int launch_r4(const GemmParams &p0, hipStream_t s) {
    GemmParams p = p0;
    p.group_n = ch_gemm_group_n(p.M, p.N, p.K, BM, BN);
    const int tiles = ((p.M + BM - 1) / BM) * (p.N / BN);
    constexpr int lds = NSTAGE * STAGE_BYTES + (ch_epi::traits<EPI>::fold ? CH_FOLD_LDS_BYTES : 0);
    static ch_once_per_device lds_once;
    if (int e = ch_func_max_lds((const void *)gemm_r4_kernel<EPI, NSTAGE>, lds, lds_once)) return e;
    hipLaunchKernelGGL((gemm_r4_kernel<EPI, NSTAGE>), dim3(tiles), dim3(NTHREADS), lds, s, p);
    CH_LAUNCH_CHECK();
    return 0;
}

}

bool ch_gemm_r4_supported(const GemmParams &p, int epi) {
    return epi >= EPI_BIAS && epi <= EPI_FOLD_GELU && p.N % BN == 0 && p.K % BK == 0 && p.K >= 3 * BK && p.X_rows_alloc >= round_up64(p.M, BM);
}

int ch_gemm_bf16_r4(const GemmParams &p, int epi, hipStream_t s) {
    CH_REQUIRE(p.M > 0 && p.N > 0 && p.K > 0, "gemm: empty problem");
    CH_REQUIRE(epi == EPI_PATCH || p.bias != nullptr, "gemm: bias is required");
    CH_REQUIRE(ch_gemm_r4_supported(p, epi), "gemm_r4: needs a forward epilogue, N % 128 == 0, K % 32 == 0, K >= 96, X padded to 128 rows");
    switch (epi) {
        case EPI_BIAS: return launch_r4<EPI_BIAS>(p, s);
        case EPI_BIAS_QUICKGELU: return launch_r4<EPI_BIAS_QUICKGELU>(p, s);
        case EPI_BIAS_GELU: return launch_r4<EPI_BIAS_GELU>(p, s);
        case EPI_BIAS_RESID: return launch_r4<EPI_BIAS_RESID>(p, s);
        case EPI_SCALE_RESID: return launch_r4<EPI_SCALE_RESID>(p, s);
        case EPI_PATCH: return launch_r4<EPI_PATCH>(p, s);
        case EPI_BIAS_STATS: return launch_r4<EPI_BIAS_STATS>(p, s);
        case EPI_SCALE_RESID_STATS: return launch_r4<EPI_SCALE_RESID_STATS>(p, s);
        case EPI_FOLD_BIAS: return launch_r4<EPI_FOLD_BIAS>(p, s);
        case EPI_FOLD_QUICKGELU: return launch_r4<EPI_FOLD_QUICKGELU>(p, s);
        case EPI_FOLD_GELU: return launch_r4<EPI_FOLD_GELU>(p, s);
    }
    ch_set_error("gemm: unknown epilogue");
    return 2;
}
```

### concepthash_amd/csrc/kernels.h

```cpp
#pragma once
#include "ch_common.h"

enum GemmEpilogue {
    EPI_BIAS = 0,
    EPI_BIAS_QUICKGELU = 1,
    EPI_BIAS_GELU = 2,
    EPI_BIAS_RESID = 3,
    EPI_SCALE_RESID = 4,
    EPI_PATCH = 5,
    EPI_BIAS_STATS = 6,
    EPI_SCALE_RESID_STATS = 7,
    EPI_FOLD_BIAS = 8,
    EPI_FOLD_QUICKGELU = 9,
    EPI_FOLD_GELU = 10,
    EPI_BIAS_DACT_QUICK = 11,
    EPI_BIAS_DACT_GELU = 12,
    EPI_FOLD_ACT2_QUICK = 13,
    EPI_FOLD_ACT2_GELU = 14,
    EPI_COUNT = 15,
};

struct GemmParams {
    const bf16_t *X;
    const bf16_t *W;
    int M, N, K;
    int64_t X_rows_alloc;
    const float *bias;
    bf16_t *out_bf16;
    int ldo;
    float *resid;
    int ldr;
    const float *scale_ptr;
    const bf16_t *addend;
    int ld_addend;
    int group_n;
    const float *pos;
    int tokens_per_img;
    int patches_per_img;
    float *stats_out;
    bf16_t *hb_out;
    int ld_hb;
    const float *stats_in;
    const float *fold_c;
    float ln_eps;
    const bf16_t *aux;
    float *splitk_ws;
    unsigned *splitk_cnt;
    int split_full, split_s;
    int force_split;
    int rev;
    int pp_sched;
    int pp_min_k;
    int64_t footprint_rows;
    int nt_resid;
    int nt_out;
    int tag;
    int small_kernel;
    int nt_resid_opt;
    int nt_out_opt;
    int group_n_opt;
    int splitk_opt;
    int rows_opt;
    int wide_opt;
};
constexpr size_t CH_SPLITK_WS_BYTES = (size_t)256 * 256 * 256 * 4;
constexpr size_t CH_SPLITK_CNT_BYTES = 256 * sizeof(unsigned);
constexpr int CH_FOLD_LDS_BYTES = 2048;
int ch_gemm_bf16(const GemmParams &p, int epi, hipStream_t s, int variant = 0);
int ch_gemm_launch_variant(int variant, const GemmParams &p, int epi, hipStream_t s);
int ch_gemm_bf16_v1(const GemmParams &p, int epi, hipStream_t s);
int ch_gemm_bf16_pp(const GemmParams &p, int epi, hipStream_t s);
bool ch_gemm_pp_supported(const GemmParams &p);
int ch_gemm_bf16_r4(const GemmParams &p, int epi, hipStream_t s);
bool ch_gemm_r4_supported(const GemmParams &p, int epi);
constexpr int64_t CH_RING_MAX_ROWS = 8192;

#ifdef CH_EXPERIMENTS
int ch_gemm_bf16_pq(const GemmParams &p, int epi, hipStream_t s);
bool ch_gemm_pq_supported(const GemmParams &p);
int ch_gemm_bf16_ppp(const GemmParams &p, int epi, hipStream_t s);
bool ch_gemm_ppp_supported(const GemmParams &p, int epi);
int ch_gemm_bf16_dp(const GemmParams &p, int epi, hipStream_t s);
bool ch_gemm_dp_supported(const GemmParams &p);
int ch_gemm_bf16_rows(const GemmParams &p, int epi, hipStream_t s);
bool ch_gemm_rows_supported(const GemmParams &p, int epi);
int ch_gemm_bf16_wide(const GemmParams &p, int epi, hipStream_t s);
bool ch_gemm_wide_supported(const GemmParams &p, int epi);
int ch_gemm_bf16_wide_dbg(const GemmParams &p, int dbg, hipStream_t s);
#else
static inline int ch_experiments_not_built() {
    ch_set_error("experiment kernels are not part of this build (rebuild with CH_BUILD_EXPERIMENTS=1)");
    return 2;
}
static inline int ch_gemm_bf16_pq(const GemmParams &, int, hipStream_t) { return ch_experiments_not_built(); }
static inline int ch_gemm_bf16_ppp(const GemmParams &, int, hipStream_t) { return ch_experiments_not_built(); }
static inline int ch_gemm_bf16_dp(const GemmParams &, int, hipStream_t) { return ch_experiments_not_built(); }
static inline int ch_gemm_bf16_rows(const GemmParams &, int, hipStream_t) { return ch_experiments_not_built(); }
static inline bool ch_gemm_rows_supported(const GemmParams &, int) { return false; }
static inline int ch_gemm_bf16_wide(const GemmParams &, int, hipStream_t) { return ch_experiments_not_built(); }
static inline bool ch_gemm_wide_supported(const GemmParams &, int) { return false; }
static inline int ch_gemm_bf16_wide_dbg(const GemmParams &, int, hipStream_t) { return ch_experiments_not_built(); }
#endif
int ch_gemm_bf16_pp_dbg(const GemmParams &p, int dbg, hipStream_t s);
void ch_gemm_count_nt_launch(int kind);
int ch_gemm_group_n(int M, int N, int K, int bm, int bn, int forced = 0);

struct AdapterParams {
    const bf16_t *A;
    float *H;
    int M, D, bpad;
    const bf16_t *Wd;
    const float *c, *d;
    const bf16_t *Wu;
    const float *bu;
    const float *scale;
    float eps;
    int dbg;
};
#ifdef CH_EXPERIMENTS
bool ch_adapter_fused_supported(int D, int bpad);
int ch_adapter_fused(const AdapterParams &p, hipStream_t s);
#else
static inline bool ch_adapter_fused_supported(int, int) { return false; }
static inline int ch_adapter_fused(const AdapterParams &, hipStream_t) { return ch_experiments_not_built(); }
#endif
int ch_fold_ln(const float *Wd, const float *bd, const float *gamma, const float *beta, int b, int bpad, int D, bf16_t *Wdf,
               float *c, float *d, hipStream_t s);

int ch_im2col(const void *images, int image_dtype, int B, int image, int patch, int Kp, bf16_t *out, hipStream_t s);
int ch_assemble_preln(float *H, int B, int ntok, int np, int D, const float *cls_pos0, const float *ctx,
                      const float *pre_w, const float *pre_b, const float *ln_w, const float *ln_b, float eps,
                      bf16_t *xn, hipStream_t s);
int ch_layernorm_f32(const float *x, int64_t rows, int D, const float *w, const float *b, float eps, bf16_t *out,
                     hipStream_t s);
int ch_layernorm_bf16(const bf16_t *x, int64_t rows, int D, const float *w, const float *b, float eps, bf16_t *out,
                      hipStream_t s);

int ch_gather_head_rows(const float *H, int B, int ntok, int ncon, int D, float *out, hipStream_t s);

int ch_attention(const bf16_t *qkv, int B, int ntok, int heads, bf16_t *out, hipStream_t s, float *cattn = nullptr,
                 int ncon = 0, bool compact = false, bool rev = false, int kernel = 0);
int ch_attention_causal(const bf16_t *qkv, int B, int ntok, int heads, bf16_t *out, hipStream_t s);

constexpr int CH_ATTN_RESIDENT_MAX_TOKENS = 288;
constexpr int CH_ATTN_MAX_TOKENS = 1 + 32 * 32 + 64;
int ch_attention_stream(const bf16_t *qkv, int B, int ntok, int heads, bf16_t *out, hipStream_t s, float *cattn, int ncon, bool compact,
                        bool rev);
int ch_attention_bwd_stream(const bf16_t *qkv, const bf16_t *dO, int B, int ntok, int heads, bf16_t *dqkv, hipStream_t s, const float *dpext,
                            int ncon);
void ch_attention_count_launch(int which);

struct HeadParams {
    const float *H;
    int B, ntok, D, Q, nbit, C, P;
    const float *hash_pe;
    const float *hash_fc;
    const float *bn_scale;
    const float *bn_shift;
    const float *center_l2;
    const float *center_bin;
    const float *concept_pe;
    const float *concept_cent_l2;
    const float *post_w, *post_b;
    const float *vis_proj;
    float ln_eps;
    float *out_codes;
    uint64_t *out_packed;
    float *out_logits_cont;
    float *out_logits_bin;
    float *out_logits_concept;
    float *out_hash_features;
    float *out_image_features;
    float *ws_xn;
    float *ws_cls;
};
int ch_head(const HeadParams &p, hipStream_t s);
int ch_pack_sign_launch(const float *codes, int64_t rows, int nbit, float thr, uint64_t *out, hipStream_t s);

int ch_small_linear(const float *x, int rows, int in_f, const float *W, const float *b, int out_f, int act, float *y,
                    hipStream_t s);
int ch_small_layernorm(const float *x, int rows, int D, const float *w, const float *b, float eps, float *y,
                       hipStream_t s);
int ch_small_add(const float *a, const float *b, int64_t n, float *y, hipStream_t s);
int ch_small_mha(const float *qkv, int T, int P, int heads, float *out, hipStream_t s);
int ch_small_l2norm(const float *x, int rows, int cols, float *out_l2, float *out_bin, hipStream_t s);
int ch_convert_bf16(const float *x, int64_t rows, int cols, int cols_pad, bf16_t *out, hipStream_t s);
int ch_bn_fold(const float *w, const float *b, const float *mean, const float *var, int n, float eps, float *scale,
               float *shift, hipStream_t s);

int ch_hb_stats(const float *H, int64_t rows, int D, bf16_t *hb, float *stats, hipStream_t s);
int ch_act_fwd(const bf16_t *pre, int64_t n, int act, bf16_t *out, hipStream_t s);
int ch_act_bwd(const bf16_t *g, const bf16_t *pre, int64_t n, int act, const float *scale_ptr, bf16_t *out, hipStream_t s);
int ch_normalize_bf16(const bf16_t *x, const float *stats, int64_t rows, int D, float eps, bf16_t *out, hipStream_t s);
int ch_ln_bwd(const bf16_t *dyg, const bf16_t *x, const float *stats, int64_t rows, int D, float eps, const float *dres_in,
              float *dres_out, bf16_t *out_b, hipStream_t s, bf16_t *xhat_out = nullptr);
int ch_wgrad_tn(bf16_t *A, int lda, const bf16_t *B, int ldb, int64_t rows, int64_t rows_alloc, int N, int K, float *out,
                float *ws, hipStream_t s, int *chunks_out = nullptr);
struct ChReduceJob {
    const float *partial;
    float *out;
    int nchunks;
    int n4;
};
int ch_reduce_partials_multi(const ChReduceJob *jobs, int njobs, hipStream_t s);
size_t ch_wgrad_ws_floats(int64_t rows, int N, int K);
int ch_colsum(const void *A, int is_f32, int lda, int64_t rows, int N, float *out, float *ws, hipStream_t s, int *chunks_out = nullptr);
size_t ch_colsum_ws_floats(int N);
int ch_transpose_f32_to_bf16(const float *src, int R, int C, int ld_src, const float *colscale, bf16_t *dst, int ld_dst, hipStream_t s);
int ch_transpose_bf16(const bf16_t *src, int R, int C, int ld_src, bf16_t *dst, int ld_dst, hipStream_t s);
int ch_adapter_grads(const float *G, const float *cu, const float *T, const float *cd, const float *params, int D, int b, int bpad,
                     float *grads, float *ws , hipStream_t s, int nad = 1, int64_t stride = 0);
int ch_adapter_refresh(const float *params, int64_t stride, int nad, int D, int b, int bpad, bf16_t *down_wf, float *fold_c, float *fold_d,
                       bf16_t *up_w, bf16_t *up_wT, bf16_t *down_wgT, hipStream_t s);
int ch_sgd_step_launch(float *p, const float *g, float *buf, int64_t n, float lr, float momentum, float wd, float dampening, int nesterov,
                       int first, hipStream_t s);
int ch_adam_step_launch(float *p, const float *g, float *m, float *v, int64_t n, double lr, double beta1, double beta2, double eps, double wd,
                        int decoupled, int64_t step, hipStream_t s);
struct ChFoldGradParts {
    const float *W[3];
    float *dW[3], *db[3];
    int nparts, rows_each;
};
int ch_fold_grads(const float *T, const float *c, const float *gamma, const float *beta, int D, const ChFoldGradParts &parts, float *dgamma,
                  float *dbeta, hipStream_t s);
int ch_embed_bwd(float *X, float *dY, int B, int ntok, int np, int D, const float *cls_pos0, const float *ctx, const float *gamma, float eps,
                 bf16_t *dx_patch, hipStream_t s);
int ch_token_rows_sum(const float *dX, int B, int ntok, int nrows, int D, float *out, hipStream_t s);
int ch_concept_rows_sum(const float *dH, int B, int ntok, int Q, int D, float *out, hipStream_t s);
int ch_scatter_concept_rows(const float *dhf, int B, int ntok, int Q, int D, float *dH, bf16_t *dHb, hipStream_t s);
int ch_expand_head_rows(const void *src, int is_f32, int B, int ntok, int Q, int D, void *dst, hipStream_t s);
int ch_small_ln_bwd(const float *dy, const float *x, const float *gamma, int rows, int D, float eps, float *dx, hipStream_t s);
int ch_gather_concept_rows(const float *H, int B, int ntok, int Q, int D, float *out, hipStream_t s);
int ch_attention_bwd(const bf16_t *qkv, const bf16_t *dO, int B, int ntok, int heads, bf16_t *dqkv, hipStream_t s,
                     const float *dpext = nullptr, int ncon = 0, int kernel = 0);
```

### concepthash_amd/csrc/model.hip

```cpp
#include <algorithm>
#include <cstdlib>
#include <map>
#include <string>
#include <vector>

#include "../../include/concepthash_hip.h"
#include "ch_common.h"
#include "kernels.h"

thread_local ch_prof_pair g_ch_prof_pair;
extern "C" int ch_abi_version(void) { return CH_ABI_VERSION; }

#include "model_internal.h"
#include "weight_builder.h"

namespace {

struct Builder : ChWeightBuilder {
    bool fold(const std::string *wnames, const std::string *bnames, int nparts, int rows_each, int n_pad, int D,
              const float *gamma, const float *beta, const bf16_t **wf, const float **cc, const float **dd) {
        const int n_true = nparts * rows_each;
        float *w32 = nullptr, *b32 = nullptr;
        if (hipMalloc((void **)&w32, sizeof(float) * (size_t)n_true * D) != hipSuccess ||
            hipMalloc((void **)&b32, sizeof(float) * n_true) != hipSuccess) {
// ... 101 lines not shown
            aw.up_w = uw;
            aw.up_b = B.f32(ap + "up_proj.bias", D);
            if (B.ok) {
                const std::string dwn = ap + "down_proj.weight", dbn = ap + "down_proj.bias";
                B.fold(&dwn, &dbn, 1, b, m->bpad, D, aw.ln_w, aw.ln_b, &aw.down_wf, &aw.fold_c, &aw.fold_d);
            }
        }
    }
    if (!B.ok) return 4;

    {
        const float *hq = B.f32("hash_queries", (int64_t)Q * P);
        const float *inw = B.f32("hash_attention.sa.in_proj_weight", (int64_t)3 * P * P);
        const float *inb = B.f32("hash_attention.sa.in_proj_bias", 3 * P);
        const float *ow = B.f32("hash_attention.sa.out_proj.weight", (int64_t)P * P);
        const float *ob = B.f32("hash_attention.sa.out_proj.bias", P);
        const float *f0w = B.f32("hash_attention.ffn.0.weight", (int64_t)P * P);
        const float *f0b = B.f32("hash_attention.ffn.0.bias", P);
        const float *f3w = B.f32("hash_attention.ffn.3.weight", (int64_t)P * P);
        const float *f3b = B.f32("hash_attention.ffn.3.bias", P);
        const float *n1w = B.f32("hash_attention.norm1.weight", P);
        const float *n1b = B.f32("hash_attention.norm1.bias", P);
        const float *n2w = B.f32("hash_attention.norm2.weight", P);
        const float *n2b = B.f32("hash_attention.norm2.bias", P);
        const float *f2w = B.f32("hash_attention.ffn2.weight", (int64_t)D * P);
        const float *f2b = B.f32("hash_attention.ffn2.bias", D);
        float *qkv = (float *)B.alloc(sizeof(float) * Q * 3 * P);
        float *t0 = (float *)B.alloc(sizeof(float) * Q * P);
        float *t1 = (float *)B.alloc(sizeof(float) * Q * P);
        float *t2 = (float *)B.alloc(sizeof(float) * Q * P);
        float *ctx = (float *)B.alloc(sizeof(float) * Q * D);
        if (!B.ok) return 4;
        int e = 0;
        e |= ch_small_linear(hq, Q, P, inw, inb, 3 * P, 0, qkv, s);
        e |= ch_small_mha(qkv, Q, P, c.upt_heads, t0, s);
        e |= ch_small_linear(t0, Q, P, ow, ob, P, 0, t1, s);
        e |= ch_small_layernorm(hq, Q, P, n1w, n1b, 1e-5f, t0, s);
        e |= ch_small_add(t0, t1, (int64_t)Q * P, t2, s);
        e |= ch_small_linear(t2, Q, P, f0w, f0b, P, 1, t0, s);
        e |= ch_small_linear(t0, Q, P, f3w, f3b, P, 0, t1, s);
        e |= ch_small_layernorm(t2, Q, P, n2w, n2b, 1e-5f, t0, s);
        e |= ch_small_add(t0, t1, (int64_t)Q * P, t2, s);
        e |= ch_small_linear(t2, Q, P, f2w, f2b, D, 0, ctx, s);
        if (e) return 4;
        m->ctx = ctx;
    }

    m->hash_pe = B.has("hash_pe") ? B.f32("hash_pe", (int64_t)Q * D) : B.f32_zeros((int64_t)Q * D);
    m->hash_fc = B.f32("hash_fc.weight", (int64_t)(c.nbit / Q) * D);
    {
        float *sc = (float *)B.alloc(sizeof(float) * c.nbit), *sh = (float *)B.alloc(sizeof(float) * c.nbit);
        if (!B.ok) return 4;
        if (B.has("hash_bn.running_mean")) {
            const float *w = B.f32("hash_bn.weight", c.nbit), *bb = B.f32("hash_bn.bias", c.nbit);
            const float *mu = B.f32("hash_bn.running_mean", c.nbit), *var = B.f32("hash_bn.running_var", c.nbit);
            if (!B.ok) return 4;
            if (ch_bn_fold(w, bb, mu, var, c.nbit, c.bn_eps, sc, sh, s)) return 4;
        } else {
            std::vector<float> ones(c.nbit, 1.0f);
            if (hipMemcpy(sc, ones.data(), sizeof(float) * c.nbit, hipMemcpyHostToDevice) != hipSuccess) return 4;
            if (hipMemset(sh, 0, sizeof(float) * c.nbit) != hipSuccess) return 4;
        }
        m->bn_scale = sc;
        m->bn_shift = sh;
    }
    {
        const int cd = c.center_dim;
        const float *cen = B.f32("center", (int64_t)C * cd);
        float *proj = (float *)B.alloc(sizeof(float) * C * c.nbit);
        if (B.has("text_projection.0.weight")) {
            const float *w0 = B.f32("text_projection.0.weight", (int64_t)cd * cd), *b0 = B.f32("text_projection.0.bias", cd);
            const float *w2 = B.f32("text_projection.2.weight", (int64_t)c.nbit * cd),
                        *b2 = B.f32("text_projection.2.bias", c.nbit);
            float *t = (float *)B.alloc(sizeof(float) * C * cd);
            if (!B.ok) return 4;
            if (ch_small_linear(cen, C, cd, w0, b0, cd, 1, t, s)) return 4;
            if (ch_small_linear(t, C, cd, w2, b2, c.nbit, 0, proj, s)) return 4;
        } else {
            const float *w = B.f32("text_projection.weight", (int64_t)c.nbit * cd), *bb = B.f32("text_projection.bias", c.nbit);
            if (!B.ok) return 4;
            if (ch_small_linear(cen, C, cd, w, bb, c.nbit, 0, proj, s)) return 4;
        }
        float *l2 = (float *)B.alloc(sizeof(float) * C * c.nbit), *bin = (float *)B.alloc(sizeof(float) * C * c.nbit);
        if (!B.ok) return 4;
        if (ch_small_l2norm(proj, C, c.nbit, l2, bin, s)) return 4;
        m->center_l2 = l2;
        m->center_bin = bin;
    }
    if (B.has("concept_ce.centroids")) {
        m->concept_pe = B.f32("concept_pe", (int64_t)Q * D);
        const float *cc = B.f32("concept_ce.centroids", (int64_t)C * D);
        float *l2 = (float *)B.alloc(sizeof(float) * C * D);
        if (!B.ok) return 4;
        if (ch_small_l2norm(cc, C, D, l2, nullptr, s)) return 4;
        m->concept_cent_l2 = l2;
    }
    if (B.has(VM + "post_layernorm.weight") && B.has("backbone.visual_projection.weight")) {
        m->post_w = B.f32(VM + "post_layernorm.weight", D);
        m->post_b = B.f32(VM + "post_layernorm.bias", D);
        m->vis_proj = B.f32("backbone.visual_projection.weight", (int64_t)P * D);
    }
    if (!B.ok) return 4;

    const int64_t rows = round_up64((int64_t)c.max_batch * m->ntok, 256) + 256;
    const int64_t prows = round_up64((int64_t)c.max_batch * np, 256) + 256;
    m->rows_alloc = rows;
    m->prow_alloc = prows;
    m->H = (float *)B.alloc(sizeof(float) * rows * D);
    m->Xn = (bf16_t *)B.alloc(sizeof(bf16_t) * rows * D);
    m->Hc = (float *)B.alloc(sizeof(float) * ((size_t)c.max_batch * (1 + c.ncontext) + 512) * D);
    m->head_xn = (float *)B.alloc(sizeof(float) * ((size_t)c.max_batch * c.ncontext + 16) * D);
    m->head_cls = (float *)B.alloc(sizeof(float) * ((size_t)c.max_batch + 16) * D);
    m->statsA = (float *)B.alloc(sizeof(float) * rows * (D / 64) * 2);
    m->statsH = (float *)B.alloc(sizeof(float) * rows * (D / 64) * 2);
    m->QKV = (bf16_t *)B.alloc(sizeof(bf16_t) * rows * 3 * D);
    m->AO = (bf16_t *)B.alloc(sizeof(bf16_t) * rows * D);
    m->A = (bf16_t *)B.alloc(sizeof(bf16_t) * rows * D);
    m->AD = (bf16_t *)B.alloc(sizeof(bf16_t) * rows * std::max(m->bpad, 128));
    m->F1 = (bf16_t *)B.alloc(sizeof(bf16_t) * rows * M);
    m->PATCH = (bf16_t *)B.alloc(sizeof(bf16_t) * prows * Kp);
    if (!B.ok) return 4;
    CH_CHECK_HIP(hipMemset(m->H, 0, sizeof(float) * rows * D));
    CH_CHECK_HIP(hipMemset(m->Xn, 0, sizeof(bf16_t) * rows * D));
    CH_CHECK_HIP(hipMemset(m->Hc, 0, sizeof(float) * ((size_t)c.max_batch * (1 + c.ncontext) + 512) * D));
    CH_CHECK_HIP(hipMemset(m->statsA, 0, sizeof(float) * rows * (D / 64) * 2));
    CH_CHECK_HIP(hipMemset(m->statsH, 0, sizeof(float) * rows * (D / 64) * 2));
    CH_CHECK_HIP(hipMemset(m->QKV, 0, sizeof(bf16_t) * rows * 3 * D));
    CH_CHECK_HIP(hipMemset(m->AO, 0, sizeof(bf16_t) * rows * D));
    CH_CHECK_HIP(hipMemset(m->A, 0, sizeof(bf16_t) * rows * D));
    CH_CHECK_HIP(hipMemset(m->AD, 0, sizeof(bf16_t) * rows * std::max(m->bpad, 128)));
    CH_CHECK_HIP(hipMemset(m->F1, 0, sizeof(bf16_t) * rows * M));
    CH_CHECK_HIP(hipMemset(m->PATCH, 0, sizeof(bf16_t) * prows * Kp));
    CH_CHECK_HIP(hipDeviceSynchronize());
    return 0;
}

inline void mark(ch_model *m, int pi, int cat, double flops, hipStream_t s) {
    ch_model::Prof &P = m->prof[pi];
    g_ch_prof_pair = ch_prof_pair();
    if (!m->prof_on || P.n + 1 >= P.ev.size()) return;
    (void)hipEventRecord(P.ev[P.n], s);
    P.cat[P.n] = cat;
    P.flops[P.n] = flops;
    P.exact[P.n] = 0;
    if (cat != CH_CAT_END) {
        g_ch_prof_pair.start = P.kstart[P.n];
        g_ch_prof_pair.stop = P.kstop[P.n];
        g_ch_prof_pair.used = (bool *)&P.exact[P.n];
    }
    P.n++;
}

int run_chain(ch_model *mm, int pi, const void *images_all, int image_dtype, int img0, int B, int nlayers, hipStream_t s,
              float *concept_attn, bool attn_all_layers, bool prune, int Btot) {
    const ch_model_config &c = mm->cfg;
    const int D = c.dim, M = c.ffn, ntok = mm->ntok, np = mm->np;
    const int rows = B * ntok;
    const int act_epi = c.act == 0 ? EPI_BIAS_QUICKGELU : EPI_BIAS_GELU;
    const size_t row0 = (size_t)img0 * ntok, prow0 = (size_t)img0 * np;
    struct View {
        float *H, *statsA, *statsH;
        bf16_t *Xn, *QKV, *AO, *A, *AD, *F1, *PATCH;
        int64_t rows_alloc, prow_alloc;
    } v{mm->H + row0 * D, mm->statsA + row0 * (D / 64) * 2, mm->statsH + row0 * (D / 64) * 2, mm->Xn + row0 * D, mm->QKV + row0 * 3 * D, mm->AO + row0 * D, mm->A + row0 * D,
        mm->AD + row0 * std::max(mm->bpad, 128), mm->F1 + row0 * M, mm->PATCH + prow0 * mm->Kp,
        mm->rows_alloc - (int64_t)row0, mm->prow_alloc - (int64_t)prow0};
    View *m = &v;
    const size_t img_elems = (size_t)3 * c.image_size * c.image_size;
    const void *images = (const char *)images_all + (size_t)img0 * img_elems * (image_dtype == 0 ? 4 : 2);
    if (concept_attn) concept_attn += (size_t)img0 * c.heads * c.ncontext * np;

    mark(mm, pi, CH_CAT_IM2COL, 0.0, s);
    if (int e = ch_im2col(images, image_dtype, B, c.image_size, c.patch, mm->Kp, m->PATCH, s)) return e;
    mark(mm, pi, CH_CAT_GEMM_PATCH, 2.0 * B * np * (double)D * 3.0 * c.patch * c.patch, s);
    {
        GemmParams p{};
        p.X = m->PATCH; p.W = mm->patch_w; p.M = B * np; p.N = D; p.K = mm->Kp; p.X_rows_alloc = m->prow_alloc;
        p.bias = nullptr; p.resid = m->H; p.ldr = D; p.pos = mm->pos; p.tokens_per_img = ntok; p.patches_per_img = np;
        p.pp_min_k = mm->pp_min_k; p.pp_sched = mm->pp_sched; p.small_kernel = mm->small_kernel; p.group_n_opt = mm->group_n;
        if (int e = ch_gemm_bf16(p, EPI_PATCH, s)) return e;
    }
    const LayerW &w0 = mm->layers[0];
    mark(mm, pi, CH_CAT_ROWOPS, 0.0, s);
    if (int e = ch_assemble_preln(m->H, B, ntok, np, D, mm->cls_pos0, mm->ctx, mm->pre_w, mm->pre_b, w0.ln1_w, w0.ln1_b,
                                  c.ln_eps, m->Xn, s))
        return e;

    struct Fold {
        const float *stats_in = nullptr, *fold_c = nullptr;
        float eps = 0.f;
        float *stats_out = nullptr;
        bf16_t *hb_out = nullptr;
    };
    const bool fold = mm->ln_fold && c.adapter_dim > 0 && !mm->use_fused_adapter;
    int dir = 0;
    auto next_dir = [&]() { return mm->serpentine ? (dir ^= 1) : 0; };
    int cur_rows = rows;
    float *cur_H = m->H;
    auto pruned_cat = [](int cat) {
        switch (cat) {
            case CH_CAT_GEMM_OUT: return (int)CH_CAT_GEMM_OUT_PRUNED;
            case CH_CAT_GEMM_DOWN: return (int)CH_CAT_GEMM_DOWN_PRUNED;
            case CH_CAT_GEMM_UP: return (int)CH_CAT_GEMM_UP_PRUNED;
            case CH_CAT_GEMM_FC1: return (int)CH_CAT_GEMM_FC1_PRUNED;
            case CH_CAT_GEMM_FC2: return (int)CH_CAT_GEMM_FC2_PRUNED;
        }
        return cat;
    };
    auto gemm = [&](int cat, int n_true, int k_true, const bf16_t *X, const bf16_t *W, int N, int K, const float *bias,
                    int epi, bf16_t *out, int ldo, const float *scale, const bf16_t *addend = nullptr, const Fold &f = Fold()) {
        mark(mm, pi, cur_rows != rows ? pruned_cat(cat) : cat, 2.0 * cur_rows * (double)n_true * k_true, s);
        GemmParams p{};
        p.tag = cat == CH_CAT_GEMM_FC2 ? 1 : 0;
        p.splitk_ws = mm->splitk_ws[pi]; p.splitk_cnt = mm->splitk_cnt[pi]; p.pp_min_k = mm->pp_min_k; p.pp_sched = mm->pp_sched; p.small_kernel = mm->small_kernel; p.rev = next_dir();
        p.nt_resid_opt = mm->resid_nt; p.nt_out_opt = mm->nt_out; p.group_n_opt = mm->group_n; p.splitk_opt = mm->splitk; p.rows_opt = mm->gemm_rows; p.wide_opt = mm->wide_kernel;
        p.footprint_rows = (int64_t)cur_rows * Btot / B;
        p.stats_in = f.stats_in; p.fold_c = f.fold_c; p.ln_eps = f.eps; p.stats_out = f.stats_out; p.hb_out = f.hb_out; p.ld_hb = D;
        p.addend = addend; p.ld_addend = D;
        p.X = X; p.W = W; p.M = cur_rows; p.N = N; p.K = K; p.X_rows_alloc = m->rows_alloc; p.bias = bias;
        p.out_bf16 = out; p.ldo = ldo; p.resid = cur_H; p.ldr = D; p.scale_ptr = scale;
        return ch_gemm_bf16(p, epi, s);
    };
    auto adapter = [&](const AdapterW &aw, bool emit_h) -> int {
        if (!aw.down_w) return 0;
        if (fold) {
            Fold fd;
            fd.stats_in = m->statsA; fd.fold_c = aw.fold_c; fd.eps = 1e-5f;
            if (int e = gemm(CH_CAT_GEMM_DOWN, c.adapter_dim, D, m->A, aw.down_wf, mm->bpad, D, aw.fold_d, EPI_FOLD_GELU, m->AD,
                             mm->bpad, nullptr, nullptr, fd))
                return e;
            Fold fu;
            if (emit_h) { fu.stats_out = m->statsH; fu.hb_out = m->Xn; }
            return gemm(CH_CAT_GEMM_UP, D, c.adapter_dim, m->AD, aw.up_w, D, mm->bpad, aw.up_b,
                        emit_h ? EPI_SCALE_RESID_STATS : EPI_SCALE_RESID, nullptr, 0, aw.scale, m->A, fu);
        }
        if (aw.down_wf && mm->use_fused_adapter && ch_adapter_fused_supported(D, mm->bpad)) {
            mark(mm, pi, CH_CAT_ADAPTER, 4.0 * rows * (double)D * c.adapter_dim, s);
            AdapterParams ap{};
            ap.A = m->A; ap.H = m->H; ap.M = rows; ap.D = D; ap.bpad = mm->bpad; ap.Wd = aw.down_wf; ap.c = aw.fold_c;
            ap.d = aw.fold_d; ap.Wu = aw.up_w; ap.bu = aw.up_b; ap.scale = aw.scale; ap.eps = 1e-5f;
            return ch_adapter_fused(ap, s);
        }
        mark(mm, pi, CH_CAT_ROWOPS, 0.0, s);
        if (int e = ch_layernorm_bf16(m->A, rows, D, aw.ln_w, aw.ln_b, 1e-5f, m->Xn, s)) return e;
        if (int e = gemm(CH_CAT_GEMM_DOWN, c.adapter_dim, D, m->Xn, aw.down_w, mm->bpad, D, aw.down_b, EPI_BIAS_GELU, m->AD,
                         mm->bpad, nullptr))
            return e;
        return gemm(CH_CAT_GEMM_UP, D, c.adapter_dim, m->AD, aw.up_w, D, mm->bpad, aw.up_b, EPI_SCALE_RESID, nullptr, 0,
                    aw.scale, m->A);
    };

    Fold stats_a;
    if (fold) stats_a.stats_out = m->statsA;
    for (int i = 0; i < nlayers; ++i) {
        const LayerW &w = mm->layers[i];
        if (i > 0 && fold) {
            Fold fq;
            fq.stats_in = m->statsH; fq.fold_c = w.qkv_c; fq.eps = c.ln_eps;
            if (int e = gemm(CH_CAT_GEMM_QKV, 3 * D, D, m->Xn, w.qkv_wf, 3 * D, D, w.qkv_d, EPI_FOLD_BIAS, m->QKV, 3 * D, nullptr,
                             nullptr, fq))
                return e;
        } else {
            if (i > 0) {
                mark(mm, pi, CH_CAT_ROWOPS, 0.0, s);
                if (int e = ch_layernorm_f32(m->H, rows, D, w.ln1_w, w.ln1_b, c.ln_eps, m->Xn, s)) return e;
            }
            if (int e = gemm(CH_CAT_GEMM_QKV, 3 * D, D, m->Xn, w.qkv_w, 3 * D, D, w.qkv_b, EPI_BIAS, m->QKV, 3 * D, nullptr)) return e;
        }
        const bool pruned = prune && fold && mm->prune_last && i == nlayers - 1 && nlayers == c.layers;
        const int nq = 1 + c.ncontext;
        mark(mm, pi, pruned ? CH_CAT_ATTENTION_PRUNED : CH_CAT_ATTENTION, 4.0 * B * (double)(pruned ? nq : ntok) * ntok * D, s);
        float *cattn = !concept_attn ? nullptr
                       : attn_all_layers ? concept_attn + (size_t)i * Btot * c.heads * c.ncontext * np
                       : i == nlayers - 1 ? concept_attn : nullptr;
        if (int e = ch_attention(m->QKV, B, ntok, c.heads, m->AO, s, cattn, c.ncontext, pruned, next_dir() != 0, mm->attn_stream ? 2 : 0))
            return e;
        if (pruned) {
            cur_rows = B * nq;
            cur_H = mm->Hc + (size_t)img0 * nq * D;
            mark(mm, pi, CH_CAT_ROWOPS, 0.0, s);
            if (int e = ch_gather_head_rows(m->H, B, ntok, c.ncontext, D, cur_H, s)) return e;
        }
        const int sub_epi = fold ? EPI_BIAS_STATS : (w.ad[0].down_w ? EPI_BIAS : EPI_BIAS_RESID);
        if (int e = gemm(CH_CAT_GEMM_OUT, D, D, m->AO, w.out_w, D, D, w.out_b, sub_epi, m->A, D, nullptr, nullptr, stats_a)) return e;
        if (int e = adapter(w.ad[0], true)) return e;
        if (fold) {
            Fold f1;
            f1.stats_in = m->statsH; f1.fold_c = w.fc1_c; f1.eps = c.ln_eps;
            if (int e = gemm(CH_CAT_GEMM_FC1, M, D, m->Xn, w.fc1_wf, M, D, w.fc1_d,
                             c.act == 0 ? EPI_FOLD_QUICKGELU : EPI_FOLD_GELU, m->F1, M, nullptr, nullptr, f1))
                return e;
        } else {
            mark(mm, pi, CH_CAT_ROWOPS, 0.0, s);
            if (int e = ch_layernorm_f32(m->H, rows, D, w.ln2_w, w.ln2_b, c.ln_eps, m->Xn, s)) return e;
            if (int e = gemm(CH_CAT_GEMM_FC1, M, D, m->Xn, w.fc1_w, M, D, w.fc1_b, act_epi, m->F1, M, nullptr)) return e;
        }
        if (int e = gemm(CH_CAT_GEMM_FC2, D, M, m->F1, w.fc2_w, D, M, w.fc2_b, sub_epi, m->A, D, nullptr, nullptr, stats_a)) return e;
        if (int e = adapter(w.ad[1], i + 1 < nlayers)) return e;
    }
    return 0;
}

int run_encoder(ch_model *m, const void *images, int image_dtype, int B, int nlayers, hipStream_t s,
                float *concept_attn = nullptr, bool attn_all_layers = false, bool prune = false) {
    int ns = std::min(m->nstreams, B);
    if (ns == 2 && m->chain_auto) {
        const int64_t rows = (int64_t)B * m->ntok;
        if (rows < 5600) ns = 1;
    }
    m->last_chains = ns;
    if (ns < 2) return run_chain(m, 0, images, image_dtype, 0, B, nlayers, s, concept_attn, attn_all_layers, prune, B);
    CH_CHECK_HIP(hipEventRecord(m->ev_fork, s));
    for (int i = 0; i < ns; ++i) {
        const int b0 = (int)((int64_t)B * i / ns), b1 = (int)((int64_t)B * (i + 1) / ns);
        hipStream_t si = i == 0 ? s : m->aux_stream[i - 1];
        if (i > 0) CH_CHECK_HIP(hipStreamWaitEvent(si, m->ev_fork, 0));
        if (int e = run_chain(m, i, images, image_dtype, b0, b1 - b0, nlayers, si, concept_attn, attn_all_layers, prune, B)) return e;
        if (i > 0) {
            CH_CHECK_HIP(hipEventRecord(m->ev_join[i - 1], si));
            CH_CHECK_HIP(hipStreamWaitEvent(s, m->ev_join[i - 1], 0));
        }
    }
    return 0;
}

void drop_graphs(ch_model *m) {
    if (!m->graphs.empty()) (void)hipDeviceSynchronize();
    for (auto &kv : m->graphs) {
        if (kv.second.exec) (void)hipGraphExecDestroy(kv.second.exec);
        if (kv.second.graph) (void)hipGraphDestroy(kv.second.graph);
    }
    m->graphs.clear();
}

int validate(const ch_model_config *c) {
    CH_REQUIRE(c != nullptr, "null config");
    CH_REQUIRE(c->dim > 0 && c->dim % 128 == 0 && c->dim <= 1280, "dim must be a multiple of 128 and <= 1280");
    CH_REQUIRE(c->heads > 0 && c->dim == c->heads * 64, "head_dim must be 64 (dim == heads * 64)");
    CH_REQUIRE(c->ffn > 0 && c->ffn % 128 == 0, "ffn must be a multiple of 128");
    CH_REQUIRE(c->layers >= 1, "layers must be >= 1");
    CH_REQUIRE(c->patch > 0 && c->image_size > 0 && c->image_size % c->patch == 0, "image_size must be divisible by patch");
    CH_REQUIRE(c->ncontext >= 1 && c->ncontext <= 64, "ncontext must be in [1, 64]");
    CH_REQUIRE(c->nbit > 0 && c->nbit % c->ncontext == 0, "nbit must be divisible by ncontext");
    CH_REQUIRE(c->nclass > 0 && c->proj_dim > 0 && c->center_dim > 0, "nclass / proj_dim / center_dim must be positive");
    CH_REQUIRE(c->upt_heads > 0 && c->proj_dim % c->upt_heads == 0, "proj_dim must be divisible by upt_heads");
    CH_REQUIRE(c->adapter_dim >= 0, "adapter_dim must be >= 0");
    CH_REQUIRE(c->max_batch >= 1, "max_batch must be >= 1");
    CH_REQUIRE(c->act == 0 || c->act == 1, "act must be 0 (quick_gelu) or 1 (gelu)");
    const int grid = c->image_size / c->patch;
    CH_REQUIRE(grid <= 32, "more than a 32 x 32 patch grid (1,024 patch tokens per image) is not supported");
    static_assert(1 + 32 * 32 + 64 <= CH_ATTN_MAX_TOKENS, "the streaming attention kernels cover every admissible model");
    return 0;
}

}

extern "C" int ch_model_create(const ch_model_config *cfg, const ch_tensor *tensors, int32_t ntensors, ch_model **out) {
    CH_REQUIRE(out != nullptr, "null out pointer");
    *out = nullptr;
    if (int e = validate(cfg)) return e;
    CH_REQUIRE(tensors != nullptr && ntensors > 0, "no tensors");
    ch_model *m = new ch_model();
    m->cfg = *cfg;
    if (m->cfg.ln_eps <= 0.f) m->cfg.ln_eps = 1e-5f;
    if (m->cfg.bn_eps <= 0.f) m->cfg.bn_eps = 1e-5f;
    const int grid = cfg->image_size / cfg->patch;
    m->np = grid * grid;
    m->ntok = 1 + m->np + cfg->ncontext;
    m->Kp = (int)round_up64(3 * cfg->patch * cfg->patch, 64);
    bool aux_ok = hipEventCreateWithFlags(&m->ev_fork, hipEventDisableTiming) == hipSuccess;
    for (int i = 0; aux_ok && i < CH_MAX_STREAMS - 1; ++i)
        aux_ok = hipStreamCreateWithFlags(&m->aux_stream[i], hipStreamNonBlocking) == hipSuccess &&
                 hipEventCreateWithFlags(&m->ev_join[i], hipEventDisableTiming) == hipSuccess;
    if (!aux_ok) {
        ch_set_error("cannot create the auxiliary streams / events");
        ch_model_destroy(m);
        return 4;
    }
    m->bpad = (int)round_up64(cfg->adapter_dim, 128);
    int e = build_model(m, tensors, ntensors);
    if (e == 0 && hipDeviceSynchronize() != hipSuccess) {
        ch_set_error("device error while folding weights");
        e = 4;
    }
    if (e) {
        ch_model_destroy(m);
        return e;
    }
    *out = m;
    return 0;
}

extern "C" void ch_model_destroy(ch_model *m) {
    if (!m) return;
    drop_graphs(m);
    if (m->cap_stream) (void)hipStreamDestroy(m->cap_stream);
    for (auto &P : m->prof) {
        for (hipEvent_t e : P.ev) (void)hipEventDestroy(e);
        for (hipEvent_t e : P.kstart) (void)hipEventDestroy(e);
        for (hipEvent_t e : P.kstop) (void)hipEventDestroy(e);
    }
    for (hipStream_t a : m->aux_stream)
        if (a) (void)hipStreamDestroy(a);
    if (m->ev_fork) (void)hipEventDestroy(m->ev_fork);
    for (hipEvent_t e : m->ev_join)
        if (e) (void)hipEventDestroy(e);
    for (void *p : m->allocs)
        if (p) (void)hipFree(p);
    delete m;
}

extern "C" size_t ch_model_device_bytes(const ch_model *m) { return m ? m->bytes : 0; }

namespace {
struct OptionRef {
    const char *key;
    int kind;
    void *(*field)(ch_model *);
    int64_t lo, hi;
};
#define CH_OPT_FIELD(name) [](ch_model *m) -> void * { return &m->name; }
const OptionRef g_options[] = {
    {"streams", 0, CH_OPT_FIELD(nstreams), 1, CH_MAX_STREAMS},
    {"chain_auto", 1, CH_OPT_FIELD(chain_auto), 0, 1},
    {"ln_fold", 1, CH_OPT_FIELD(ln_fold), 0, 1},
    {"prune_last", 1, CH_OPT_FIELD(prune_last), 0, 1},
    {"pp_min_k", 0, CH_OPT_FIELD(pp_min_k), 0, 1 << 20},
    {"attn_stream", 0, CH_OPT_FIELD(attn_stream), 0, 1},
    {"small_kernel", 0, CH_OPT_FIELD(small_kernel), 0, 2},
    {"serpentine", 1, CH_OPT_FIELD(serpentine), 0, 1},
    {"pp_sched", 0, CH_OPT_FIELD(pp_sched), 0, 2},
    {"fused_adapter", 1, CH_OPT_FIELD(use_fused_adapter), 0, 1},
    {"resid_nt", 0, CH_OPT_FIELD(resid_nt), -1, 1},
    {"nt_out", 0, CH_OPT_FIELD(nt_out), -1, 1},
    {"group_n", 0, CH_OPT_FIELD(group_n), 0, 64},
    {"splitk", 0, CH_OPT_FIELD(splitk), 0, 1},
    {"gemm_rows", 0, CH_OPT_FIELD(gemm_rows), 0, 1},
    {"wide_kernel", 0, CH_OPT_FIELD(wide_kernel), 0, 1},
    {"graph_max_batch", 0, CH_OPT_FIELD(graph_max_batch), 0, 1 << 16},
    {"train_chains", 0, CH_OPT_FIELD(train_chains), 1, 2},
    {"train_chain_min_rows", 2, CH_OPT_FIELD(train_chain_min_rows), 0, (int64_t)1 << 40},
    {"train_prune_last", 1, CH_OPT_FIELD(train_prune_last), 0, 1},
    {"train_batched_grads", 1, CH_OPT_FIELD(train_batched_grads), 0, 1},
};
#undef CH_OPT_FIELD
const OptionRef *find_option(const char *key) {
    if (!key) return nullptr;
    for (const OptionRef &o : g_options)
        if (std::string(o.key) == key) return &o;
    return nullptr;
}
}

extern "C" int ch_model_set_option(ch_model *m, const char *key, int64_t value) {
    CH_REQUIRE(m != nullptr, "set_option: null model");
    const OptionRef *o = find_option(key);
    if (!o) {
        ch_set_error(std::string("invalid argument: set_option: unknown key '") + (key ? key : "(null)") + "'");
        return 2;
    }
    if (value < o->lo || value > o->hi) {
        ch_set_error(std::string("invalid argument: set_option: '") + key + "' must be in [" + std::to_string(o->lo) + ", " +
                     std::to_string(o->hi) + "], got " + std::to_string(value));
        return 2;
    }
#ifndef CH_EXPERIMENTS
    const std::string k = key;
    if (value != 0 && (k == "fused_adapter" || k == "pp_sched" || k == "gemm_rows" || k == "wide_kernel")) {
        ch_set_error("set_option: '" + k + "' selects an experiment kernel that is not part of this build (CH_BUILD_EXPERIMENTS=1)");
        return 2;
    }
#endif
    if (std::string(key) == "splitk" && value != 0) {
        for (int i = 0; i < CH_MAX_STREAMS; ++i) {
            if (m->splitk_ws[i]) continue;
            CH_CHECK_HIP(hipMalloc((void **)&m->splitk_ws[i], CH_SPLITK_WS_BYTES));
            m->allocs.push_back(m->splitk_ws[i]);
            CH_CHECK_HIP(hipMalloc((void **)&m->splitk_cnt[i], CH_SPLITK_CNT_BYTES));
            m->allocs.push_back(m->splitk_cnt[i]);
            CH_CHECK_HIP(hipMemset(m->splitk_cnt[i], 0, CH_SPLITK_CNT_BYTES));
            m->bytes += CH_SPLITK_WS_BYTES + CH_SPLITK_CNT_BYTES;
        }
    }
    void *f = o->field(m);
    if (o->kind == 0) *(int *)f = (int)value;
    else if (o->kind == 1) *(bool *)f = value != 0;
    else *(int64_t *)f = value;
    if (std::string(key) == "graph_max_batch") m->graph_max_batch = std::min(m->graph_max_batch, m->cfg.max_batch);
    drop_graphs(m);
    return 0;
}

extern "C" int ch_model_get_option(ch_model *m, const char *key, int64_t *value) {
    CH_REQUIRE(m != nullptr && value != nullptr, "get_option: null model / value");
    if (key && std::string(key) == "graph_replays") { *value = m->graph_replays; return 0; }
    if (key && std::string(key) == "last_chains") { *value = m->last_chains; return 0; }
    if (key && std::string(key) == "graph_captures") { *value = m->graph_captures; return 0; }
    const OptionRef *o = find_option(key);
    if (!o) {
        ch_set_error(std::string("invalid argument: get_option: unknown key '") + (key ? key : "(null)") + "'");
        return 2;
    }
    void *f = o->field(m);
    *value = o->kind == 0 ? (int64_t) * (int *)f : o->kind == 1 ? (int64_t) * (bool *)f : *(int64_t *)f;
    return 0;
}

extern "C" double ch_model_flops_per_image(const ch_model *m) {
    if (!m) return 0.0;
    const ch_model_config &c = m->cfg;
    const double N = m->ntok, D = c.dim, M = c.ffn, b = c.adapter_dim, L = c.layers;
    const double patch = 2.0 * m->np * D * 3.0 * c.patch * c.patch;
    const double layer = 8.0 * N * D * D + 4.0 * N * D * M + 4.0 * N * N * D + 8.0 * N * D * b;
    double total = patch + L * layer + 2.0 * D * c.nbit;
    if (m->prune_last && m->ln_fold && c.adapter_dim > 0 && !m->use_fused_adapter) {
        const double nq = 1 + c.ncontext;
        total += -layer + 6.0 * N * D * D + 4.0 * nq * N * D + 2.0 * nq * D * D + 4.0 * nq * D * M + 8.0 * nq * D * b;
    }
    return total;
}

namespace {

int encode_impl(ch_model *m, const void *images, int image_dtype, int B, float *out_codes, uint64_t *out_packed, float *out_logits_cont,
                float *out_logits_bin, float *out_logits_concept, float *out_hash_features, float *out_image_features,
                float *out_concept_attn, bool all_layers, hipStream_t s) {
    if (int e = run_encoder(m, images, image_dtype, B, m->cfg.layers, s, out_concept_attn, all_layers, true)) return e;
    const ch_model_config &c = m->cfg;
    const bool pruned = m->prune_last && m->ln_fold && c.adapter_dim > 0 && !m->use_fused_adapter;
    HeadParams p{};
    p.H = pruned ? m->Hc : m->H; p.B = B; p.ntok = pruned ? 1 + c.ncontext : m->ntok; p.D = c.dim; p.Q = c.ncontext; p.nbit = c.nbit; p.C = c.nclass; p.P = c.proj_dim;
    p.hash_pe = m->hash_pe; p.hash_fc = m->hash_fc; p.bn_scale = m->bn_scale; p.bn_shift = m->bn_shift;
    p.center_l2 = m->center_l2; p.center_bin = m->center_bin; p.concept_pe = m->concept_pe;
    p.concept_cent_l2 = m->concept_cent_l2; p.post_w = m->post_w; p.post_b = m->post_b; p.vis_proj = m->vis_proj;
    p.ln_eps = c.ln_eps;
    p.out_codes = out_codes; p.out_packed = out_packed; p.out_logits_cont = out_logits_cont;
    p.out_logits_bin = out_logits_bin; p.out_logits_concept = out_logits_concept;
    p.out_hash_features = out_hash_features; p.out_image_features = out_image_features;
    p.ws_xn = m->head_xn; p.ws_cls = m->head_cls;
    mark(m, 0, CH_CAT_HEAD, 2.0 * B * (double)c.dim * c.nbit, s);
    if (int e = ch_head(p, s)) return e;
    mark(m, 0, CH_CAT_END, 0.0, s);
    return 0;
}

int ensure_bytes(ch_model *m, void **buf, size_t *have, size_t need) {
    if (*have >= need) return 0;
    drop_graphs(m);
    if (*buf) {
        CH_CHECK_HIP(hipDeviceSynchronize());
        for (void *&p : m->allocs)
            if (p == *buf) p = nullptr;
        CH_CHECK_HIP(hipFree(*buf));
        m->bytes -= *have;
    }
    CH_CHECK_HIP(hipMalloc(buf, need));
    m->allocs.push_back(*buf);
    m->bytes += need;
    *have = need;
    return 0;
}

int encode_graph(ch_model *m, const void *images, int image_dtype, int B, void *const outs[8], bool all_layers, hipStream_t s) {
    const ch_model_config &c = m->cfg;
    const size_t img_bytes = (size_t)B * 3 * c.image_size * c.image_size * (image_dtype == 0 ? 4 : 2);
    const size_t np = (size_t)m->np;
    const size_t out_bytes[8] = {sizeof(float) * B * c.nbit, sizeof(uint64_t) * B * ((c.nbit + 63) / 64), sizeof(float) * B * c.nclass,
                                 sizeof(float) * B * c.nclass, sizeof(float) * c.ncontext * B * c.nclass, sizeof(float) * B * c.ncontext * c.dim,
                                 sizeof(float) * B * c.proj_dim,
                                 sizeof(float) * (all_layers ? c.layers : 1) * B * c.heads * c.ncontext * np};
    int mask = 0;
    for (int i = 0; i < 8; ++i)
        if (outs[i]) mask |= 1 << i;
    const size_t cap = (size_t)m->graph_max_batch;
    if (int e = ensure_bytes(m, &m->g_in, &m->g_in_bytes, cap * 3 * c.image_size * c.image_size * 4)) return e;
    for (int i = 0; i < 8; ++i)
        if (outs[i])
            if (int e = ensure_bytes(m, &m->g_out[i], &m->g_out_bytes[i], out_bytes[i] / B * cap)) return e;
    CH_CHECK_HIP(hipMemcpyAsync(m->g_in, images, img_bytes, hipMemcpyDeviceToDevice, s));
    auto staged = [&](int i) { return outs[i] ? m->g_out[i] : nullptr; };
    auto chain = [&](hipStream_t st) {
        return encode_impl(m, m->g_in, image_dtype, B, (float *)staged(0), (uint64_t *)staged(1), (float *)staged(2), (float *)staged(3),
                           (float *)staged(4), (float *)staged(5), (float *)staged(6), (float *)staged(7), all_layers, st);
    };
    const auto key = std::make_tuple(B, image_dtype, mask, all_layers ? 1 : 0);
    auto it = m->graphs.find(key);
    if (it == m->graphs.end()) {
        if (int e = chain(s)) return e;
        if (!m->cap_stream) CH_CHECK_HIP(hipStreamCreateWithFlags(&m->cap_stream, hipStreamNonBlocking));
        ch_model::GraphEntry ge;
        CH_CHECK_HIP(hipStreamBeginCapture(m->cap_stream, hipStreamCaptureModeThreadLocal));
        const int e = chain(m->cap_stream);
        const hipError_t he = hipStreamEndCapture(m->cap_stream, &ge.graph);
        if (e) {
            if (ge.graph) (void)hipGraphDestroy(ge.graph);
            return e;
        }
        CH_CHECK_HIP(he);
        CH_CHECK_HIP(hipGraphInstantiate(&ge.exec, ge.graph, nullptr, nullptr, 0));
        m->graphs[key] = ge;
        m->graph_captures++;
    } else {
        CH_CHECK_HIP(hipGraphLaunch(it->second.exec, s));
        m->graph_replays++;
    }
    for (int i = 0; i < 8; ++i)
        if (outs[i]) CH_CHECK_HIP(hipMemcpyAsync(outs[i], m->g_out[i], out_bytes[i], hipMemcpyDeviceToDevice, s));
    return 0;
}

}

extern "C" int ch_encode(ch_model *m, const void *images, int32_t image_dtype, int32_t B, float *out_codes,
                         uint64_t *out_packed, float *out_logits_cont, float *out_logits_bin, float *out_logits_concept,
                         float *out_hash_features, float *out_image_features, float *out_concept_attn,
                         int32_t concept_attn_all_layers, void *stream) {
    CH_REQUIRE(m != nullptr && images != nullptr && out_codes != nullptr, "null model / images / out_codes");
    CH_REQUIRE(image_dtype == 0 || image_dtype == 1, "image_dtype must be 0 (fp32) or 1 (bf16)");
    CH_REQUIRE(B >= 1 && B <= m->cfg.max_batch, "batch outside [1, max_batch]");
    CH_REQUIRE(!out_logits_concept || m->concept_cent_l2, "model has no concept classifier (concept_ce.centroids)");
    CH_REQUIRE(!out_image_features || m->vis_proj, "model has no post_layernorm / visual_projection");
    hipStream_t s = (hipStream_t)stream;
    if (m->graph_max_batch > 0 && B <= m->graph_max_batch && !m->prof_on) {
        void *const outs[8] = {out_codes, out_packed, out_logits_cont, out_logits_bin, out_logits_concept, out_hash_features,
                               out_image_features, out_concept_attn};
        return encode_graph(m, images, image_dtype, B, outs, concept_attn_all_layers != 0, s);
    }
    return encode_impl(m, images, image_dtype, B, out_codes, out_packed, out_logits_cont, out_logits_bin, out_logits_concept,
                       out_hash_features, out_image_features, out_concept_attn, concept_attn_all_layers != 0, s);
}

extern "C" int ch_encode_hidden(ch_model *m, const void *images, int32_t image_dtype, int32_t B, int32_t layer,
                                float *out_hidden, void *stream) {
    CH_REQUIRE(m != nullptr && images != nullptr && out_hidden != nullptr, "null model / images / out_hidden");
    CH_REQUIRE(B >= 1 && B <= m->cfg.max_batch, "batch outside [1, max_batch]");
    CH_REQUIRE(layer >= 0 && layer <= m->cfg.layers, "layer outside [0, layers]");
    hipStream_t s = (hipStream_t)stream;
    if (int e = run_encoder(m, images, image_dtype, B, layer, s)) return e;
    CH_CHECK_HIP(hipMemcpyAsync(out_hidden, m->H, sizeof(float) * (size_t)B * m->ntok * m->cfg.dim,
                                hipMemcpyDeviceToDevice, s));
    return 0;
}

extern "C" int ch_pack_sign(const float *codes, int64_t rows, int32_t nbit, float threshold, uint64_t *out_packed,
                            void *stream) {
    CH_REQUIRE(rows >= 0 && nbit > 0, "pack_sign: rows must be >= 0 and nbit > 0");
    CH_REQUIRE(rows == 0 || (codes && out_packed), "pack_sign: null pointer");
    return ch_pack_sign_launch(codes, rows, nbit, threshold, out_packed, (hipStream_t)stream);
}

extern "C" int ch_model_profile_begin(ch_model *m, int32_t max_launches) {
    CH_REQUIRE(m != nullptr && max_launches > 0, "profile_begin: null model or non-positive capacity");
    for (auto &P : m->prof) {
        while (P.ev.size() < (size_t)max_launches + 1) {
            hipEvent_t e, a, b;
            CH_CHECK_HIP(hipEventCreate(&e));
            CH_CHECK_HIP(hipEventCreate(&a));
            CH_CHECK_HIP(hipEventCreate(&b));
            P.ev.push_back(e);
            P.kstart.push_back(a);
            P.kstop.push_back(b);
        }
        P.cat.assign(P.ev.size(), CH_CAT_END);
        P.flops.assign(P.ev.size(), 0.0);
        P.exact.assign(P.ev.size(), 0);
        P.n = 0;
    }
    m->prof_on = true;
    return 0;
}

extern "C" int ch_model_profile_end(ch_model *m, int32_t ncat, double *ms_per_cat, int64_t *launches_per_cat, double *flops_per_cat) {
    CH_REQUIRE(m != nullptr && ms_per_cat && launches_per_cat && flops_per_cat, "profile_end: null pointer");
    CH_REQUIRE(ncat >= CH_NCAT, "profile_end: the caller's arrays hold fewer than CH_NCAT entries (built against an older header?)");
    m->prof_on = false;
    for (int i = 0; i < CH_NCAT; ++i) {
        ms_per_cat[i] = 0.0;
        launches_per_cat[i] = 0;
        flops_per_cat[i] = 0.0;
    }
// ... 23 lines not shown
```

### concepthash_amd/csrc/model_internal.h

```cpp
#pragma once
#include <map>
#include <string>
#include <tuple>
#include <vector>

#include "../../include/concepthash_hip.h"
#include "ch_common.h"
#include "kernels.h"

constexpr int CH_MAX_STREAMS = 4;

struct AdapterW {
    const float *ln_w = nullptr, *ln_b = nullptr, *down_b = nullptr, *up_b = nullptr, *scale = nullptr;
    const bf16_t *down_w = nullptr, *up_w = nullptr;
    const bf16_t *down_wf = nullptr;
    const float *fold_c = nullptr, *fold_d = nullptr;
};
struct LayerW {
    const float *ln1_w, *ln1_b, *ln2_w, *ln2_b, *qkv_b, *out_b, *fc1_b, *fc2_b;
    const bf16_t *qkv_w, *out_w, *fc1_w, *fc2_w;
    const bf16_t *qkv_wf = nullptr, *fc1_wf = nullptr;
    const float *qkv_c = nullptr, *qkv_d = nullptr, *fc1_c = nullptr, *fc1_d = nullptr;
    AdapterW ad[2];
};

struct ch_model {
    ch_model_config cfg;
    int np = 0, ntok = 0, Kp = 0, bpad = 0;
    std::vector<void *> allocs;
    size_t bytes = 0;
    const bf16_t *patch_w = nullptr;
    const float *pos = nullptr, *cls_pos0 = nullptr, *ctx = nullptr, *pre_w = nullptr, *pre_b = nullptr;
    const float *zero_bias = nullptr;
    std::vector<LayerW> layers;
    const float *hash_pe = nullptr, *hash_fc = nullptr, *bn_scale = nullptr, *bn_shift = nullptr;
    const float *center_l2 = nullptr, *center_bin = nullptr, *concept_pe = nullptr, *concept_cent_l2 = nullptr;
    const float *post_w = nullptr, *post_b = nullptr, *vis_proj = nullptr;
    bool use_fused_adapter = false;
    bool ln_fold = true;
    bool prof_on = false;
    struct Prof {
        std::vector<hipEvent_t> ev;
        std::vector<hipEvent_t> kstart, kstop;
        std::vector<char> exact;
        std::vector<int> cat;
        std::vector<double> flops;
        size_t n = 0;
    } prof[CH_MAX_STREAMS];
    int nstreams = 2;
    hipStream_t aux_stream[CH_MAX_STREAMS - 1] = {};
    hipEvent_t ev_fork = nullptr, ev_join[CH_MAX_STREAMS - 1] = {};
    int64_t rows_alloc = 0, prow_alloc = 0;
    float *H = nullptr;
    float *splitk_ws[CH_MAX_STREAMS] = {};
    unsigned *splitk_cnt[CH_MAX_STREAMS] = {};
    bool prune_last = true;
    bool serpentine = false;
    int pp_sched = 0;
    int small_kernel = 0;
    int pp_min_k = 0;
    int attn_stream = 0;
    int resid_nt = 0, nt_out = 0;
    int group_n = 0;
    int splitk = 0;
    int gemm_rows = 0;
    int wide_kernel = 0;
    int graph_max_batch = 0;
    hipStream_t cap_stream = nullptr;
    struct GraphEntry {
        hipGraph_t graph = nullptr;
        hipGraphExec_t exec = nullptr;
    };
    std::map<std::tuple<int, int, int, int>, GraphEntry> graphs;
    void *g_in = nullptr;
    size_t g_in_bytes = 0;
    void *g_out[8] = {};
    size_t g_out_bytes[8] = {};
    int64_t graph_replays = 0, graph_captures = 0;
    int train_chains = 2;
    int last_chains = 0;
    bool chain_auto = true;
    int64_t train_chain_min_rows = 0;
    bool train_prune_last = true;
    bool train_batched_grads = true;
    float *Hc = nullptr;
    float *head_xn = nullptr, *head_cls = nullptr;
    float *statsA = nullptr, *statsH = nullptr;
    bf16_t *Xn = nullptr, *QKV = nullptr, *AO = nullptr, *A = nullptr, *AD = nullptr, *F1 = nullptr, *PATCH = nullptr;
};
```

### include/concepthash_hip_debug.h

```cpp
#ifndef CONCEPTHASH_HIP_DEBUG_H
#define CONCEPTHASH_HIP_DEBUG_H

#include "concepthash_hip.h"

#ifdef __cplusplus
extern "C" {
#endif

int ch_debug_gemm(int32_t variant, const void *X, int64_t X_rows_alloc, const void *W, const float *bias, int32_t M,
                  int32_t N, int32_t K, int32_t epi, void *out_bf16, int32_t ldo, float *resid, int32_t ldr,
                  const float *scale_ptr, const void *addend, void *stream);
int ch_debug_gemm_ln(int32_t variant, const void *X, int64_t X_rows_alloc, const void *W, const float *bias, int32_t M,
                     int32_t N, int32_t K, int32_t epi, void *out_bf16, int32_t ldo, float *resid, int32_t ldr,
                     const float *scale_ptr, const void *addend, const float *stats_in, const float *fold_c, float ln_eps,
                     float *stats_out, void *hb_out, void *stream);
int ch_debug_gemm_train(int32_t variant, const void *X, int64_t X_rows_alloc, const void *W, const float *bias, int32_t M, int32_t N,
                        int32_t K, int32_t epi, void *out_bf16, int32_t ldo, const void *aux, const float *scale_ptr,
                        const float *stats_in, const float *fold_c, float ln_eps, void *hb_out, int32_t ld_hb, void *stream);
int ch_debug_gemm_patch(int32_t variant, const void *X, int64_t X_rows_alloc, const void *W, int32_t M, int32_t N, int32_t K, float *resid,
                        int32_t ldr, const float *pos, int32_t tokens_per_img, int32_t patches_per_img, void *stream);
int32_t ch_debug_experiments_built(void);
int64_t ch_debug_gemm_dispatch_count(int32_t which);
int ch_debug_copy_buffer(ch_model *m, int32_t which, void *out, int64_t nbytes, void *stream);
void ch_debug_set_gemm_splitk(int32_t on);
int ch_debug_adapter(const void *A, float *H, int32_t M, int32_t D, int32_t b, const float *Wd, const float *bd,
                     const float *gamma, const float *beta, const void *Wu_bf16_padded, const float *bu, const float *scale,
                     void *work_wdf, float *work_c, float *work_d, int32_t dbg, void *stream);
int ch_debug_attention(const void *qkv, int32_t B, int32_t ntok, int32_t heads, void *out, void *stream);
int ch_debug_attention_ex(const void *qkv, int32_t B, int32_t ntok, int32_t heads, void *out, float *cattn, int32_t ncon, int32_t compact,
                          int32_t kernel, void *stream);
int ch_debug_attention_causal(const void *qkv, int32_t B, int32_t ntok, int32_t heads, void *out, void *stream);
int64_t ch_debug_attention_dispatch_count(int32_t which);

void ch_debug_set_hamming_scalar_loads(int32_t on);

int ch_debug_attention_bwd(const void *qkv, const void *dO, int32_t B, int32_t ntok, int32_t heads, void *dqkv, const float *dpext,
                           int32_t ncon, void *stream);
int ch_debug_attention_bwd_ex(const void *qkv, const void *dO, int32_t B, int32_t ntok, int32_t heads, void *dqkv, const float *dpext,
                              int32_t ncon, int32_t kernel, void *stream);
int ch_debug_wgrad(const void *A, int32_t lda, const void *Bm, int32_t ldb, int64_t rows, int64_t rows_alloc, int32_t N, int32_t K,
                   float *out, void *stream);
int ch_debug_ln_bwd(const void *dyg, const void *x, int64_t rows, int32_t D, float eps, const float *dres_in, float *dres_out,
                    void *out_b, void *xhat_out, void *stream);
int ch_debug_act(const void *g, const void *pre, int64_t n, int32_t act, const float *scale_ptr, int32_t backward, void *out,
                 void *stream);

#ifdef __cplusplus
}
#endif
#endif
```

Measured before the change: 21320 images/s.

## Emit QKV GEMM output in head-major layout for contiguous attention loads

```diff
diff --git a/concepthash_amd/_lib.py b/concepthash_amd/_lib.py
--- a/concepthash_amd/_lib.py
+++ b/concepthash_amd/_lib.py
@@ -59,6 +59,8 @@
                                  c_void_p]),
     "ch_debug_gemm_train": (c_int, [c_int32, c_void_p, c_int64, c_void_p, c_void_p, c_int32, c_int32, c_int32, c_int32, c_void_p,
                                     c_int32, c_void_p, c_void_p, c_void_p, c_void_p, c_float, c_void_p, c_int32, c_void_p]),
+    "ch_debug_gemm_head_major": (c_int, [c_int32, c_void_p, c_int64, c_void_p, c_void_p, c_int32, c_int32, c_int32, c_void_p, c_int32, c_int32,
+                                         c_int32, c_int32, c_void_p]),
     "ch_debug_gemm_patch": (c_int, [c_int32, c_void_p, c_int64, c_void_p, c_int32, c_int32, c_int32, c_void_p, c_int32, c_void_p,
                                     c_int32, c_int32, c_void_p]),
     "ch_debug_gemm_dispatch_count": (c_int64, [c_int32]),
@@ -70,6 +72,7 @@
     "ch_debug_attention_ex": (c_int, [c_void_p, c_int32, c_int32, c_int32, c_void_p, c_void_p, c_int32, c_int32, c_int32, c_void_p]),
     "ch_debug_attention_causal": (c_int, [c_void_p, c_int32, c_int32, c_int32, c_void_p, c_void_p]),
     "ch_debug_attention_dispatch_count": (c_int64, [c_int32]),
+    "ch_debug_attention_head_major_count": (c_int64, []),
     "ch_encode": (c_int, [c_void_p, c_void_p, c_int32, c_int32, c_void_p, c_void_p, c_void_p, c_void_p, c_void_p,
                           c_void_p, c_void_p, c_void_p, c_int32, c_void_p]),
     "ch_encode_hidden": (c_int, [c_void_p, c_void_p, c_int32, c_int32, c_int32, c_void_p, c_void_p]),
@@ -133,7 +136,7 @@
     "ch_text_encode": (c_int, [c_void_p, POINTER(c_int32), POINTER(c_int32), c_int32, c_int32, c_void_p, c_void_p, c_void_p]),
 }
 
-OPTION_KEYS = ("streams", "chain_auto", "ln_fold", "prune_last", "pp_min_k", "attn_stream", "small_kernel", "serpentine", "pp_sched", "fused_adapter", "resid_nt",
+OPTION_KEYS = ("streams", "chain_auto", "ln_fold", "prune_last", "pp_min_k", "attn_stream", "qkv_head_major", "small_kernel", "serpentine", "pp_sched", "fused_adapter", "resid_nt",
                "nt_out", "group_n", "splitk", "gemm_rows", "wide_kernel", "graph_max_batch", "train_chains", "train_chain_min_rows", "train_prune_last",
                "train_batched_grads")
 _ENV_OVERRIDES = {
@@ -143,7 +146,7 @@
     "CH_RESID_NT": ("resid_nt", lambda v: 1 if int(v) else -1), "CH_NT_OUT": ("nt_out", lambda v: 1 if int(v) else -1),
     "CH_GEMM_GROUP_N": ("group_n", int), "CH_GEMM_SPLITK": ("splitk", int), "CH_GEMM_ROWS": ("gemm_rows", int), "CH_GEMM_WIDE": ("wide_kernel", int), "CH_GRAPH_MAX_BATCH": ("graph_max_batch", int),
     "CH_CHAIN_AUTO": ("chain_auto", int), "CH_TRAIN_STREAMS": ("train_chains", int), "CH_TRAIN_CHAIN_MIN_ROWS": ("train_chain_min_rows", int),
-    "CH_TRAIN_PRUNE_LAST": ("train_prune_last", int),
+    "CH_TRAIN_PRUNE_LAST": ("train_prune_last", int), "CH_QKV_HEAD_MAJOR": ("qkv_head_major", int),
 }
 
 
diff --git a/concepthash_amd/csrc/attention.hip b/concepthash_amd/csrc/attention.hip
--- a/concepthash_amd/csrc/attention.hip
+++ b/concepthash_amd/csrc/attention.hip
@@ -1,3 +1,5 @@
+#include <atomic>
+
 #include "ch_common.h"
 #include "kernels.h"
 
@@ -12,7 +14,7 @@
 typedef short v4s __attribute__((ext_vector_type(4)));
 typedef __attribute__((address_space(3))) v4s lds_v4s;
 
-template <int KB, bool TAP, bool COMPACT, bool CAUSAL = false>
+template <int KB, bool TAP, bool COMPACT, bool CAUSAL = false, bool HM = false>
 __global__ __launch_bounds__(NW * 64, 4) void attention_kernel(const bf16_t *__restrict__ qkv, int ntok, int heads, float scale_log2e,
                                                         bf16_t *__restrict__ out, float *__restrict__ cattn, int ncon, int rev) {
     extern __shared__ __attribute__((aligned(16))) char smem[];
@@ -26,8 +28,9 @@
     const int bid = rev ? (int)gridDim.x - 1 - (int)blockIdx.x : (int)blockIdx.x;
     const int b = bid / heads, h = bid - b * heads;
     const int D = heads * HD;
-    const size_t ld = (size_t)3 * D;
-    const bf16_t *base = qkv + (size_t)b * ntok * ld + h * HD;
+    const size_t ld = HM ? (size_t)HD : (size_t)3 * D;
+    const bf16_t *base = HM ? qkv + (size_t)bid * ntok * HD : qkv + (size_t)b * ntok * ld + h * HD;
+    const size_t hm_which = (size_t)gridDim.x * ntok * HD;
 
     {
         const int lrow = lane >> 3;
@@ -36,8 +39,13 @@
             int row = i * 8 + lrow;
             row = row < ntok ? row : ntok - 1;
             const bf16_t *src = base + (size_t)row * ld + src_chunk * 8;
-            __builtin_amdgcn_global_load_lds((gbl_void_t *)(src + D), (lds_void_t *)(Ks + i * 1024), 16, 0, QKV_AUX);
-            __builtin_amdgcn_global_load_lds((gbl_void_t *)(src + 2 * D), (lds_void_t *)(Vs + i * 1024), 16, 0, QKV_AUX);
+            if constexpr (HM) {
+                __builtin_amdgcn_global_load_lds((gbl_void_t *)(src + hm_which), (lds_void_t *)(Ks + i * 1024), 16, 0, QKV_AUX);
+                __builtin_amdgcn_global_load_lds((gbl_void_t *)(src + 2 * hm_which), (lds_void_t *)(Vs + i * 1024), 16, 0, QKV_AUX);
+            } else {
+                __builtin_amdgcn_global_load_lds((gbl_void_t *)(src + D), (lds_void_t *)(Ks + i * 1024), 16, 0, QKV_AUX);
+                __builtin_amdgcn_global_load_lds((gbl_void_t *)(src + 2 * D), (lds_void_t *)(Vs + i * 1024), 16, 0, QKV_AUX);
+            }
         }
     }
     const int fr = lane & 15, fq = lane >> 4;
@@ -196,51 +204,63 @@
     }
 }
 
-template <int KB, bool TAP, bool COMPACT, bool CAUSAL = false>
+template <int KB, bool TAP, bool COMPACT, bool CAUSAL = false, bool HM = false>
 int launch_attn_inst(const bf16_t *qkv, int B, int ntok, int heads, bf16_t *out, float *cattn, int ncon, int rev, hipStream_t s) {
     const int KP = KB * 32;
     const size_t lds = (size_t)KP * 128 * 2;
     CH_REQUIRE(lds <= 160 * 1024, "attention: sequence too long for the LDS-resident K/V kernel");
     static ch_once_per_device lds_once;
-    if (int e = ch_func_max_lds((const void *)attention_kernel<KB, TAP, COMPACT, CAUSAL>, (int)lds, lds_once)) return e;
+    if (int e = ch_func_max_lds((const void *)attention_kernel<KB, TAP, COMPACT, CAUSAL, HM>, (int)lds, lds_once)) return e;
     const float scale_log2e = 0.125f * 1.4426950408889634f;
-    CH_LAUNCH((attention_kernel<KB, TAP, COMPACT, CAUSAL>), dim3(B * heads), dim3(NW * 64), lds, s, qkv, ntok, heads, scale_log2e,
+    CH_LAUNCH((attention_kernel<KB, TAP, COMPACT, CAUSAL, HM>), dim3(B * heads), dim3(NW * 64), lds, s, qkv, ntok, heads, scale_log2e,
                        out, cattn, ncon, rev);
     CH_LAUNCH_CHECK();
     return 0;
 }
+template <int KB, bool HM>
+int launch_attn_layout(const bf16_t *qkv, int B, int ntok, int heads, bf16_t *out, float *cattn, int ncon, bool compact, int rev, hipStream_t s) {
+    if (compact)
+        return cattn ? launch_attn_inst<KB, true, true, false, HM>(qkv, B, ntok, heads, out, cattn, ncon, rev, s)
+                     : launch_attn_inst<KB, false, true, false, HM>(qkv, B, ntok, heads, out, cattn, ncon, rev, s);
+    return cattn ? launch_attn_inst<KB, true, false, false, HM>(qkv, B, ntok, heads, out, cattn, ncon, rev, s)
+                 : launch_attn_inst<KB, false, false, false, HM>(qkv, B, ntok, heads, out, cattn, ncon, rev, s);
+}
 template <int KB>
-int launch_attn(const bf16_t *qkv, int B, int ntok, int heads, bf16_t *out, float *cattn, int ncon, bool compact, int rev, hipStream_t s) {
-    if (compact)
-        return cattn ? launch_attn_inst<KB, true, true>(qkv, B, ntok, heads, out, cattn, ncon, rev, s)
-                     : launch_attn_inst<KB, false, true>(qkv, B, ntok, heads, out, cattn, ncon, rev, s);
-    return cattn ? launch_attn_inst<KB, true, false>(qkv, B, ntok, heads, out, cattn, ncon, rev, s)
-                 : launch_attn_inst<KB, false, false>(qkv, B, ntok, heads, out, cattn, ncon, rev, s);
-}
-
-}
+int launch_attn(const bf16_t *qkv, int B, int ntok, int heads, bf16_t *out, float *cattn, int ncon, bool compact, int rev, bool head_major,
+                hipStream_t s) {
+    return head_major ? launch_attn_layout<KB, true>(qkv, B, ntok, heads, out, cattn, ncon, compact, rev, s)
+                      : launch_attn_layout<KB, false>(qkv, B, ntok, heads, out, cattn, ncon, compact, rev, s);
+}
+
+}
+
+static std::atomic<int64_t> g_head_major_launches;
+extern "C" int64_t ch_debug_attention_head_major_count(void) { return g_head_major_launches.load(std::memory_order_relaxed); }
 
 int ch_attention(const bf16_t *qkv, int B, int ntok, int heads, bf16_t *out, hipStream_t s, float *cattn, int ncon, bool compact,
-                 bool rev, int kernel) {
+                 bool rev, int kernel, bool head_major) {
     CH_REQUIRE(B > 0 && ntok > 0 && heads > 0, "attention: empty problem");
     CH_REQUIRE(!compact || (ncon >= 1 && ncon < ntok), "attention: compact mode needs 1 <= ncon < ntok");
     CH_REQUIRE(kernel >= 0 && kernel <= 2, "attention: kernel must be 0 (by length), 1 (resident) or 2 (streaming)");
-    if (kernel == 2 || (kernel == 0 && ntok > CH_ATTN_RESIDENT_MAX_TOKENS)) {
+    const bool streaming = kernel == 2 || (kernel == 0 && ntok > CH_ATTN_RESIDENT_MAX_TOKENS);
+    CH_REQUIRE(!head_major || (!streaming && ntok <= CH_ATTN_RESIDENT_MAX_TOKENS), "attention: only the LDS-resident kernel reads the head-major layout");
+    if (streaming) {
         ch_attention_count_launch(1);
         return ch_attention_stream(qkv, B, ntok, heads, out, s, cattn, ncon, compact, rev);
     }
     if (ntok <= CH_ATTN_RESIDENT_MAX_TOKENS) ch_attention_count_launch(0);
+    if (head_major) g_head_major_launches.fetch_add(1, std::memory_order_relaxed);
     const int KB = (ntok + 31) / 32;
     switch (KB) {
-        case 1: return launch_attn<1>(qkv, B, ntok, heads, out, cattn, ncon, compact, rev ? 1 : 0, s);
-        case 2: return launch_attn<2>(qkv, B, ntok, heads, out, cattn, ncon, compact, rev ? 1 : 0, s);
-        case 3: return launch_attn<3>(qkv, B, ntok, heads, out, cattn, ncon, compact, rev ? 1 : 0, s);
-        case 4: return launch_attn<4>(qkv, B, ntok, heads, out, cattn, ncon, compact, rev ? 1 : 0, s);
-        case 5: return launch_attn<5>(qkv, B, ntok, heads, out, cattn, ncon, compact, rev ? 1 : 0, s);
-        case 6: return launch_attn<6>(qkv, B, ntok, heads, out, cattn, ncon, compact, rev ? 1 : 0, s);
-        case 7: return launch_attn<7>(qkv, B, ntok, heads, out, cattn, ncon, compact, rev ? 1 : 0, s);
-        case 8: return launch_attn<8>(qkv, B, ntok, heads, out, cattn, ncon, compact, rev ? 1 : 0, s);
-        case 9: return launch_attn<9>(qkv, B, ntok, heads, out, cattn, ncon, compact, rev ? 1 : 0, s);
+        case 1: return launch_attn<1>(qkv, B, ntok, heads, out, cattn, ncon, compact, rev ? 1 : 0, head_major, s);
+        case 2: return launch_attn<2>(qkv, B, ntok, heads, out, cattn, ncon, compact, rev ? 1 : 0, head_major, s);
+        case 3: return launch_attn<3>(qkv, B, ntok, heads, out, cattn, ncon, compact, rev ? 1 : 0, head_major, s);
+        case 4: return launch_attn<4>(qkv, B, ntok, heads, out, cattn, ncon, compact, rev ? 1 : 0, head_major, s);
+        case 5: return launch_attn<5>(qkv, B, ntok, heads, out, cattn, ncon, compact, rev ? 1 : 0, head_major, s);
+        case 6: return launch_attn<6>(qkv, B, ntok, heads, out, cattn, ncon, compact, rev ? 1 : 0, head_major, s);
+        case 7: return launch_attn<7>(qkv, B, ntok, heads, out, cattn, ncon, compact, rev ? 1 : 0, head_major, s);
+        case 8: return launch_attn<8>(qkv, B, ntok, heads, out, cattn, ncon, compact, rev ? 1 : 0, head_major, s);
+        case 9: return launch_attn<9>(qkv, B, ntok, heads, out, cattn, ncon, compact, rev ? 1 : 0, head_major, s);
     }
     ch_set_error("attention: the LDS-resident kernel holds at most 288 tokens per image");
     return 2;
diff --git a/concepthash_amd/csrc/debug_taps.hip b/concepthash_amd/csrc/debug_taps.hip
--- a/concepthash_amd/csrc/debug_taps.hip
+++ b/concepthash_amd/csrc/debug_taps.hip
@@ -99,6 +99,17 @@
     p.resid = resid; p.ldr = ldr; p.pos = pos; p.tokens_per_img = tokens_per_img; p.patches_per_img = patches_per_img;
     return debug_gemm_launch_checked(p, EPI_PATCH, stream, variant, "debug_gemm_patch");
 }
+extern "C" int ch_debug_gemm_head_major(int32_t variant, const void *X, int64_t X_rows_alloc, const void *W, const float *bias, int32_t M,
+                                        int32_t N, int32_t K, void *out_bf16, int32_t tokens, int32_t heads, int32_t images, int32_t nt_out,
+                                        void *stream) {
+    CH_REQUIRE(X && W && bias && out_bf16, "debug_gemm_head_major: null operand");
+    CH_REQUIRE(variant == 1 || variant == 2 || variant == 7, "debug_gemm_head_major: variant must be 1 (128x128), 2 (256x256) or 7 (ring)");
+    CH_REQUIRE(!nt_out || variant == 2, "debug_gemm_head_major: only the 256x256 kernel has a non-temporal output instance");
+    GemmParams p = debug_gemm_params(X, X_rows_alloc, W, bias, M, N, K, out_bf16, N, nullptr);
+    p.head_major = 1; p.hm_tokens = tokens; p.hm_heads = heads; p.hm_images = images; p.nt_out = nt_out != 0;
+    CH_REQUIRE(ch_gemm_head_major_ok(p, EPI_BIAS), "debug_gemm_head_major: needs N == 3 * heads * 64, tokens >= 8, M <= images * tokens");
+    return debug_gemm_launch_checked(p, EPI_BIAS, stream, variant, "debug_gemm_head_major");
+}
 extern "C" int32_t ch_debug_experiments_built(void) {
 #ifdef CH_EXPERIMENTS
     return 1;
diff --git a/concepthash_amd/csrc/gemm_bf16.hip b/concepthash_amd/csrc/gemm_bf16.hip
--- a/concepthash_amd/csrc/gemm_bf16.hip
+++ b/concepthash_amd/csrc/gemm_bf16.hip
@@ -20,7 +20,7 @@
     return base + local;
 }
 
-template <int EPI, bool NT = false>
+template <int EPI, bool NT = false, bool HM = false>
 __global__ __launch_bounds__(NTHREADS, 2) void gemm_bf16_kernel(GemmParams p) {
     extern __shared__ __attribute__((aligned(16))) char smem[];
     const int tid = threadIdx.x;
@@ -102,7 +102,7 @@
         cur ^= 1;
     }
 
-    ch_epi::store_tile<EPI, 4, PREF, NT>(p, acc, smem + wid * 16384, m0 + wm * 64, n0 + wn * 64, lane,
+    ch_epi::store_tile<EPI, 4, PREF, NT, false, HM>(p, acc, smem + wid * 16384, m0 + wm * 64, n0 + wn * 64, lane,
                                          (const float *)(smem + 2 * STAGE_BYTES) + 2 * (wm * 64), &rp);
 }
 
@@ -122,6 +122,19 @@
             CH_LAUNCH_CHECK();
             ch_gemm_count_nt_launch(0);
             return 0;
+        }
+    }
+    if (p.head_major) {
+        if constexpr (EPI == EPI_BIAS || EPI == EPI_FOLD_BIAS) {
+            CH_REQUIRE(ch_gemm_head_major_ok(p, EPI), "gemm: head-major output needs N == 3 * heads * 64, >= 8 tokens per image, M <= images * tokens");
+            static ch_once_per_device lds_once_hm;
+            if (int e = ch_func_max_lds((const void *)gemm_bf16_kernel<EPI, false, true>, lds, lds_once_hm)) return e;
+            CH_LAUNCH((gemm_bf16_kernel<EPI, false, true>), dim3(tiles), dim3(NTHREADS), lds, s, p);
+            CH_LAUNCH_CHECK();
+            return 0;
+        } else {
+            ch_set_error("gemm: head-major output exists for EPI_BIAS / EPI_FOLD_BIAS only");
+            return 2;
         }
     }
     CH_LAUNCH(gemm_bf16_kernel<EPI>, dim3(tiles), dim3(NTHREADS), lds, s, p);
@@ -192,6 +205,7 @@
     return std::max<int64_t>(p.M, p.footprint_rows) * p.N * 2 >= (128ll << 20);
 }
 int ch_gemm_launch_variant(int variant, const GemmParams &p, int epi, hipStream_t s) {
+    CH_REQUIRE(!p.head_major || variant == 1 || variant == 2 || variant == 7, "gemm: head-major output exists in the 128x128, 256x256 and ring kernels only");
     switch (variant) {
         case 1: return ch_gemm_bf16_v1(p, epi, s);
         case 2: return ch_gemm_bf16_pp(p, epi, s);
@@ -217,6 +231,9 @@
     GemmParams p = p0;
     p.nt_resid = resid_nt_choice(p, epi);
     p.nt_out = out_nt_choice(p, epi);
+    if (p.head_major)
+        CH_REQUIRE(ch_gemm_head_major_ok(p, epi) && p.pp_sched == 0,
+                   "gemm: head-major output needs EPI_BIAS / EPI_FOLD_BIAS, N == 3 * heads * 64, >= 8 tokens per image, M <= images * tokens");
     if (epi == EPI_BIAS_DACT_QUICK || epi == EPI_BIAS_DACT_GELU) CH_REQUIRE(p.aux != nullptr, "gemm: derivative epilogue needs aux (the pre-activation)");
     if (epi == EPI_FOLD_ACT2_QUICK || epi == EPI_FOLD_ACT2_GELU) CH_REQUIRE(p.hb_out != nullptr, "gemm: two-output epilogue needs hb_out");
     if (epi == EPI_FOLD_BIAS || epi == EPI_FOLD_QUICKGELU || epi == EPI_FOLD_GELU || epi == EPI_FOLD_ACT2_QUICK || epi == EPI_FOLD_ACT2_GELU)
@@ -228,11 +245,11 @@
     const int min_k = p.pp_min_k > 0 ? p.pp_min_k : 512;
     const int64_t tiles_pp = ceil_div64(p.M, 256) * (p.N / 256);
     const bool pp = ch_gemm_pp_supported(p) && p.K >= min_k && (p.pp_min_k > 0 || tiles_pp >= 128);
-    const bool wide = !pp && p.wide_opt > 0 && ch_gemm_wide_supported(p, epi);
+    const bool wide = !pp && !p.head_major && p.wide_opt > 0 && ch_gemm_wide_supported(p, epi);
     g_dispatch_count[pp ? 1 : wide ? 4 : 0].fetch_add(1, std::memory_order_relaxed);
     if (pp) return ch_gemm_bf16_pp(p, epi, s);
     if (wide) return ch_gemm_bf16_wide(p, epi, s);
-    if (p.rows_opt && p.small_kernel == 0 && p.M >= 128 * 128 && ch_gemm_rows_supported(p, epi)) return ch_gemm_bf16_rows(p, epi, s);
+    if (p.rows_opt && !p.head_major && p.small_kernel == 0 && p.M >= 128 * 128 && ch_gemm_rows_supported(p, epi)) return ch_gemm_bf16_rows(p, epi, s);
     const bool ring = (p.small_kernel == 2 || variant == 7 || (p.small_kernel == 0 && variant == 0 && p.M <= CH_RING_MAX_ROWS && !p.nt_resid)) &&
                       ch_gemm_r4_supported(p, epi);
     return ring ? ch_gemm_bf16_r4(p, epi, s) : ch_gemm_bf16_v1(p, epi, s);
diff --git a/concepthash_amd/csrc/gemm_epilogue.h b/concepthash_amd/csrc/gemm_epilogue.h
--- a/concepthash_amd/csrc/gemm_epilogue.h
+++ b/concepthash_amd/csrc/gemm_epilogue.h
@@ -127,10 +127,11 @@
     }
 }
 
-template <int EPI, int MT, bool PREF = false, bool NT = false, bool NTOUT = false>
+template <int EPI, int MT, bool PREF = false, bool NT = false, bool NTOUT = false, bool HM = false>
 __device__ __forceinline__ void store_tile(const GemmParams &p, f32x4 (&acc)[4][MT], char *wave_lds, int m_base, int n_base,
                                            int lane, const float *row_ms = nullptr, const ResidPrefetch *pf = nullptr) {
     static_assert(!PREF || (MT == 4 && traits<EPI>::scale_resid), "prefetched residual: 64-row wave tiles, scale+residual epilogues");
+    static_assert(!HM || EPI == EPI_BIAS || EPI == EPI_FOLD_BIAS, "head-major output: the qkv projection's epilogues");
     const int fr = lane & 15, fq = lane >> 4;
     using T = traits<EPI>;
     constexpr bool BF16_ONLY = T::bf16_only;
@@ -187,6 +188,14 @@
         }
         asm volatile("s_waitcnt lgkmcnt(0)" ::: "memory");
         const int lrow = lane >> 3, pos = lane & 7;
+        int hm_img = 0, hm_tok = 0;
+        size_t hm_slice = 0;
+        if constexpr (HM) {
+            const int sl = n_base >> 6, which = sl / p.hm_heads, head = sl - which * p.hm_heads;
+            hm_slice = ((size_t)which * p.hm_images * p.hm_heads + head) * p.hm_tokens * 64;
+            hm_img = (m_base + lrow) / p.hm_tokens;
+            hm_tok = (m_base + lrow) - hm_img * p.hm_tokens;
+        }
 #pragma unroll
         for (int i = 0; i < MT * 2; ++i) {
             const int row = i * 8 + lrow;
@@ -209,9 +218,18 @@
                 v = make_uint4(ow[0], ow[1], ow[2], ow[3]);
             }
             if (m < p.M) {
-                uint4 *dst = (uint4 *)(p.out_bf16 + (size_t)m * p.ldo + n_base + chunk * 8);
+                uint4 *dst;
+                if constexpr (HM) dst = (uint4 *)(p.out_bf16 + hm_slice + ((size_t)hm_img * p.hm_heads * p.hm_tokens + hm_tok) * 64 + chunk * 8);
+                else dst = (uint4 *)(p.out_bf16 + (size_t)m * p.ldo + n_base + chunk * 8);
                 if constexpr (NTOUT) __builtin_nontemporal_store(__builtin_bit_cast(u32x4_nt, v), (u32x4_nt *)dst);
                 else *dst = v;
+            }
+            if constexpr (HM) {
+                hm_tok += 8;
+                if (hm_tok >= p.hm_tokens) {
+                    hm_tok -= p.hm_tokens;
+                    ++hm_img;
+                }
             }
             if constexpr (T::act2) {
                 const uint32_t vw[4] = {v.x, v.y, v.z, v.w};
diff --git a/concepthash_amd/csrc/gemm_pp.hip b/concepthash_amd/csrc/gemm_pp.hip
--- a/concepthash_amd/csrc/gemm_pp.hip
+++ b/concepthash_amd/csrc/gemm_pp.hip
@@ -353,14 +353,14 @@
                 for (int nt = 0; nt < 4; ++nt)
 #pragma unroll
                     for (int mt = 0; mt < 4; ++mt) half[nt][mt] = acc[nt][pass * 4 + mt];
-                ch_epi::store_tile<EPI, 4, false, false, TAG == 2>(p, half, smem + wid * 8192, m0 + wr * 128 + pass * 64, n0 + wc * 64, lane,
+                ch_epi::store_tile<EPI, 4, false, false, TAG == 2 || TAG == 4, (TAG >= 3)>(p, half, smem + wid * 8192, m0 + wr * 128 + pass * 64, n0 + wc * 64, lane,
                                            (const float *)(smem + 2 * BUF_BYTES) + 2 * (wr * 128 + pass * 64));
                 asm volatile("s_waitcnt lgkmcnt(0)" ::: "memory");
             }
             return;
         }
     }
-    ch_epi::store_tile<EPI, 8, false, false, TAG == 2>(p, acc, smem + wid * 16384, m0 + wr * 128, n0 + wc * 64, lane,
+    ch_epi::store_tile<EPI, 8, false, false, TAG == 2 || TAG == 4, (TAG >= 3)>(p, acc, smem + wid * 16384, m0 + wr * 128, n0 + wc * 64, lane,
                                (const float *)(smem + 2 * BUF_BYTES) + 2 * (wr * 128));
     if constexpr (DBG & 8) {
         stamp[4] = __builtin_amdgcn_s_memtime();
@@ -410,6 +410,27 @@
             CH_LAUNCH((gemm_pp_kernel<EPI, 0, SCHED, 1>), grid, dim3(NTHREADS), lds, s, p);
             CH_LAUNCH_CHECK();
             return 0;
+        }
+    }
+    if (p.head_major) {
+        if constexpr ((EPI == EPI_BIAS || EPI == EPI_FOLD_BIAS) && SCHED == 0) {
+            CH_REQUIRE(ch_gemm_head_major_ok(p, EPI), "gemm_pp: head-major output needs N == 3 * heads * 64, >= 8 tokens per image, M <= images * tokens");
+            if (p.nt_out) {
+                static ch_once_per_device lds_once_hn;
+                if (int e = ch_func_max_lds((const void *)gemm_pp_kernel<EPI, 0, SCHED, 4>, lds, lds_once_hn)) return e;
+                CH_LAUNCH((gemm_pp_kernel<EPI, 0, SCHED, 4>), grid, dim3(NTHREADS), lds, s, p);
+                CH_LAUNCH_CHECK();
+                ch_gemm_count_nt_launch(1);
+                return 0;
+            }
+            static ch_once_per_device lds_once_h;
+            if (int e = ch_func_max_lds((const void *)gemm_pp_kernel<EPI, 0, SCHED, 3>, lds, lds_once_h)) return e;
+            CH_LAUNCH((gemm_pp_kernel<EPI, 0, SCHED, 3>), grid, dim3(NTHREADS), lds, s, p);
+            CH_LAUNCH_CHECK();
+            return 0;
+        } else {
+            ch_set_error("gemm_pp: head-major output exists for EPI_BIAS / EPI_FOLD_BIAS on the fine schedule only");
+            return 2;
         }
     }
     if constexpr ((EPI == EPI_BIAS || EPI == EPI_FOLD_BIAS || EPI == EPI_FOLD_QUICKGELU || EPI == EPI_FOLD_GELU || EPI == EPI_FOLD_ACT2_QUICK ||
diff --git a/concepthash_amd/csrc/gemm_r4.hip b/concepthash_amd/csrc/gemm_r4.hip
--- a/concepthash_amd/csrc/gemm_r4.hip
+++ b/concepthash_amd/csrc/gemm_r4.hip
@@ -17,7 +17,7 @@
     return base + local;
 }
 
-template <int EPI, int NSTAGE>
+template <int EPI, int NSTAGE, bool HM = false>
 __global__ __launch_bounds__(NTHREADS, NSTAGE == 2 ? 4 : 2) void gemm_r4_kernel(GemmParams p) {
     extern __shared__ __attribute__((aligned(16))) char smem[];
     const int tid = threadIdx.x;
@@ -112,7 +112,7 @@
     asm volatile("s_waitcnt lgkmcnt(0)" ::: "memory");
     __builtin_amdgcn_s_barrier();
     __builtin_amdgcn_sched_barrier(0);
-    ch_epi::store_tile<EPI, 4, PREF>(p, acc, smem + wid * (NSTAGE == 2 ? 8192 : 16384), m0 + wm * 64, n0 + wn * 64, lane,
+    ch_epi::store_tile<EPI, 4, PREF, false, false, HM>(p, acc, smem + wid * (NSTAGE == 2 ? 8192 : 16384), m0 + wm * 64, n0 + wn * 64, lane,
                                      (const float *)(smem + NSTAGE * STAGE_BYTES) + 2 * (wm * 64), &rp);
 }
 
@@ -124,6 +124,19 @@
     constexpr int lds = NSTAGE * STAGE_BYTES + (ch_epi::traits<EPI>::fold ? CH_FOLD_LDS_BYTES : 0);
     static ch_once_per_device lds_once;
     if (int e = ch_func_max_lds((const void *)gemm_r4_kernel<EPI, NSTAGE>, lds, lds_once)) return e;
+    if (p.head_major) {
+        if constexpr (EPI == EPI_BIAS || EPI == EPI_FOLD_BIAS) {
+            CH_REQUIRE(ch_gemm_head_major_ok(p, EPI), "gemm_r4: head-major output needs N == 3 * heads * 64, >= 8 tokens per image, M <= images * tokens");
+            static ch_once_per_device lds_once_hm;
+            if (int e = ch_func_max_lds((const void *)gemm_r4_kernel<EPI, NSTAGE, true>, lds, lds_once_hm)) return e;
+            hipLaunchKernelGGL((gemm_r4_kernel<EPI, NSTAGE, true>), dim3(tiles), dim3(NTHREADS), lds, s, p);
+            CH_LAUNCH_CHECK();
+            return 0;
+        } else {
+            ch_set_error("gemm_r4: head-major output exists for EPI_BIAS / EPI_FOLD_BIAS only");
+            return 2;
+        }
+    }
     hipLaunchKernelGGL((gemm_r4_kernel<EPI, NSTAGE>), dim3(tiles), dim3(NTHREADS), lds, s, p);
     CH_LAUNCH_CHECK();
     return 0;
diff --git a/concepthash_amd/csrc/kernels.h b/concepthash_amd/csrc/kernels.h
--- a/concepthash_amd/csrc/kernels.h
+++ b/concepthash_amd/csrc/kernels.h
@@ -62,7 +62,13 @@
     int splitk_opt;
     int rows_opt;
     int wide_opt;
-};
+    int head_major;
+    int hm_tokens, hm_heads, hm_images;
+};
+static inline bool ch_gemm_head_major_ok(const GemmParams &p, int epi) {
+    return (epi == EPI_BIAS || epi == EPI_FOLD_BIAS) && p.hm_tokens >= 8 && p.hm_heads >= 1 && p.hm_images >= 1 && p.N == 3 * p.hm_heads * 64 &&
+           (int64_t)p.M <= (int64_t)p.hm_images * p.hm_tokens;
+}
 constexpr size_t CH_SPLITK_WS_BYTES = (size_t)256 * 256 * 256 * 4;
 constexpr size_t CH_SPLITK_CNT_BYTES = 256 * sizeof(unsigned);
 constexpr int CH_FOLD_LDS_BYTES = 2048;
@@ -139,7 +145,7 @@
 int ch_gather_head_rows(const float *H, int B, int ntok, int ncon, int D, float *out, hipStream_t s);
 
 int ch_attention(const bf16_t *qkv, int B, int ntok, int heads, bf16_t *out, hipStream_t s, float *cattn = nullptr,
-                 int ncon = 0, bool compact = false, bool rev = false, int kernel = 0);
+                 int ncon = 0, bool compact = false, bool rev = false, int kernel = 0, bool head_major = false);
 int ch_attention_causal(const bf16_t *qkv, int B, int ntok, int heads, bf16_t *out, hipStream_t s);
 
 constexpr int CH_ATTN_RESIDENT_MAX_TOKENS = 288;
@@ -149,6 +155,9 @@
 int ch_attention_bwd_stream(const bf16_t *qkv, const bf16_t *dO, int B, int ntok, int heads, bf16_t *dqkv, hipStream_t s, const float *dpext,
                             int ncon);
 void ch_attention_count_launch(int which);
+static inline bool ch_attention_resident_runs(int ntok, int kernel) {
+    return kernel != 2 && ntok <= CH_ATTN_RESIDENT_MAX_TOKENS;
+}
 
 struct HeadParams {
     const float *H;
diff --git a/concepthash_amd/csrc/model.hip b/concepthash_amd/csrc/model.hip
--- a/concepthash_amd/csrc/model.hip
+++ b/concepthash_amd/csrc/model.hip
@@ -277,7 +277,7 @@
 }
 
 int run_chain(ch_model *mm, int pi, const void *images_all, int image_dtype, int img0, int B, int nlayers, hipStream_t s,
-              float *concept_attn, bool attn_all_layers, bool prune, int Btot) {
+              float *concept_attn, bool attn_all_layers, bool prune, int Btot, bool head_major_ok) {
     const ch_model_config &c = mm->cfg;
     const int D = c.dim, M = c.ffn, ntok = mm->ntok, np = mm->np;
     const int rows = B * ntok;
@@ -318,6 +318,9 @@
         bf16_t *hb_out = nullptr;
     };
     const bool fold = mm->ln_fold && c.adapter_dim > 0 && !mm->use_fused_adapter;
+    const int attn_kernel = mm->attn_stream ? 2 : 0;
+    const bool head_major = head_major_ok && mm->qkv_head_major && mm->pp_sched == 0 && ntok >= 8 && ch_attention_resident_runs(ntok, attn_kernel);
+    if (head_major) mm->head_major_used = 1;
     int dir = 0;
     auto next_dir = [&]() { return mm->serpentine ? (dir ^= 1) : 0; };
     int cur_rows = rows;
@@ -344,6 +347,7 @@
         p.addend = addend; p.ld_addend = D;
         p.X = X; p.W = W; p.M = cur_rows; p.N = N; p.K = K; p.X_rows_alloc = m->rows_alloc; p.bias = bias;
         p.out_bf16 = out; p.ldo = ldo; p.resid = cur_H; p.ldr = D; p.scale_ptr = scale;
+        if (cat == CH_CAT_GEMM_QKV && head_major) { p.head_major = 1; p.hm_tokens = ntok; p.hm_heads = c.heads; p.hm_images = B; }
         return ch_gemm_bf16(p, epi, s);
     };
     auto adapter = [&](const AdapterW &aw, bool emit_h) -> int {
@@ -398,7 +402,7 @@
         float *cattn = !concept_attn ? nullptr
                        : attn_all_layers ? concept_attn + (size_t)i * Btot * c.heads * c.ncontext * np
                        : i == nlayers - 1 ? concept_attn : nullptr;
-        if (int e = ch_attention(m->QKV, B, ntok, c.heads, m->AO, s, cattn, c.ncontext, pruned, next_dir() != 0, mm->attn_stream ? 2 : 0))
+        if (int e = ch_attention(m->QKV, B, ntok, c.heads, m->AO, s, cattn, c.ncontext, pruned, next_dir() != 0, attn_kernel, head_major))
             return e;
         if (pruned) {
             cur_rows = B * nq;
@@ -427,20 +431,21 @@
 }
 
 int run_encoder(ch_model *m, const void *images, int image_dtype, int B, int nlayers, hipStream_t s,
-                float *concept_attn = nullptr, bool attn_all_layers = false, bool prune = false) {
+                float *concept_attn = nullptr, bool attn_all_layers = false, bool prune = false, bool head_major_ok = false) {
     int ns = std::min(m->nstreams, B);
+    m->head_major_used = 0;
     if (ns == 2 && m->chain_auto) {
         const int64_t rows = (int64_t)B * m->ntok;
         if (rows < 5600) ns = 1;
     }
     m->last_chains = ns;
-    if (ns < 2) return run_chain(m, 0, images, image_dtype, 0, B, nlayers, s, concept_attn, attn_all_layers, prune, B);
+    if (ns < 2) return run_chain(m, 0, images, image_dtype, 0, B, nlayers, s, concept_attn, attn_all_layers, prune, B, head_major_ok);
     CH_CHECK_HIP(hipEventRecord(m->ev_fork, s));
     for (int i = 0; i < ns; ++i) {
         const int b0 = (int)((int64_t)B * i / ns), b1 = (int)((int64_t)B * (i + 1) / ns);
         hipStream_t si = i == 0 ? s : m->aux_stream[i - 1];
         if (i > 0) CH_CHECK_HIP(hipStreamWaitEvent(si, m->ev_fork, 0));
-        if (int e = run_chain(m, i, images, image_dtype, b0, b1 - b0, nlayers, si, concept_attn, attn_all_layers, prune, B)) return e;
+        if (int e = run_chain(m, i, images, image_dtype, b0, b1 - b0, nlayers, si, concept_attn, attn_all_layers, prune, B, head_major_ok)) return e;
         if (i > 0) {
             CH_CHECK_HIP(hipEventRecord(m->ev_join[i - 1], si));
             CH_CHECK_HIP(hipStreamWaitEvent(s, m->ev_join[i - 1], 0));
@@ -552,6 +557,7 @@
     {"prune_last", 1, CH_OPT_FIELD(prune_last), 0, 1},
     {"pp_min_k", 0, CH_OPT_FIELD(pp_min_k), 0, 1 << 20},
     {"attn_stream", 0, CH_OPT_FIELD(attn_stream), 0, 1},
+    {"qkv_head_major", 1, CH_OPT_FIELD(qkv_head_major), 0, 1},
     {"small_kernel", 0, CH_OPT_FIELD(small_kernel), 0, 2},
     {"serpentine", 1, CH_OPT_FIELD(serpentine), 0, 1},
     {"pp_sched", 0, CH_OPT_FIELD(pp_sched), 0, 2},
@@ -621,6 +627,7 @@
     if (key && std::string(key) == "graph_replays") { *value = m->graph_replays; return 0; }
     if (key && std::string(key) == "last_chains") { *value = m->last_chains; return 0; }
     if (key && std::string(key) == "graph_captures") { *value = m->graph_captures; return 0; }
+    if (key && std::string(key) == "qkv_head_major_used") { *value = m->head_major_used; return 0; }
     const OptionRef *o = find_option(key);
     if (!o) {
         ch_set_error(std::string("invalid argument: get_option: unknown key '") + (key ? key : "(null)") + "'");
@@ -650,7 +657,7 @@
 int encode_impl(ch_model *m, const void *images, int image_dtype, int B, float *out_codes, uint64_t *out_packed, float *out_logits_cont,
                 float *out_logits_bin, float *out_logits_concept, float *out_hash_features, float *out_image_features,
                 float *out_concept_attn, bool all_layers, hipStream_t s) {
-    if (int e = run_encoder(m, images, image_dtype, B, m->cfg.layers, s, out_concept_attn, all_layers, true)) return e;
+    if (int e = run_encoder(m, images, image_dtype, B, m->cfg.layers, s, out_concept_attn, all_layers, true, true)) return e;
     const ch_model_config &c = m->cfg;
     const bool pruned = m->prune_last && m->ln_fold && c.adapter_dim > 0 && !m->use_fused_adapter;
     HeadParams p{};
diff --git a/concepthash_amd/csrc/model_internal.h b/concepthash_amd/csrc/model_internal.h
--- a/concepthash_amd/csrc/model_internal.h
+++ b/concepthash_amd/csrc/model_internal.h
@@ -60,6 +60,8 @@
     int small_kernel = 0;
     int pp_min_k = 0;
     int attn_stream = 0;
+    bool qkv_head_major = false;
+    int head_major_used = 0;
     int resid_nt = 0, nt_out = 0;
     int group_n = 0;
     int splitk = 0;
diff --git a/include/concepthash_hip_debug.h b/include/concepthash_hip_debug.h
--- a/include/concepthash_hip_debug.h
+++ b/include/concepthash_hip_debug.h
@@ -19,6 +19,8 @@
                         const float *stats_in, const float *fold_c, float ln_eps, void *hb_out, int32_t ld_hb, void *stream);
 int ch_debug_gemm_patch(int32_t variant, const void *X, int64_t X_rows_alloc, const void *W, int32_t M, int32_t N, int32_t K, float *resid,
                         int32_t ldr, const float *pos, int32_t tokens_per_img, int32_t patches_per_img, void *stream);
+int ch_debug_gemm_head_major(int32_t variant, const void *X, int64_t X_rows_alloc, const void *W, const float *bias, int32_t M, int32_t N,
+                             int32_t K, void *out_bf16, int32_t tokens, int32_t heads, int32_t images, int32_t nt_out, void *stream);
 int32_t ch_debug_experiments_built(void);
 int64_t ch_debug_gemm_dispatch_count(int32_t which);
 int ch_debug_copy_buffer(ch_model *m, int32_t which, void *out, int64_t nbytes, void *stream);
@@ -31,6 +33,7 @@
                           int32_t kernel, void *stream);
 int ch_debug_attention_causal(const void *qkv, int32_t B, int32_t ntok, int32_t heads, void *out, void *stream);
 int64_t ch_debug_attention_dispatch_count(int32_t which);
+int64_t ch_debug_attention_head_major_count(void);
 
 void ch_debug_set_hamming_scalar_loads(int32_t on);
 
```

After: 21330 images/s (median of 3 runs). About the same (+0.0%).
